# oss0430/SRFRD

Measured on NVIDIA B200. Metric: training seqs/sec; full-catalogue top-10 users/sec, higher is better.
Workload: dtype bf16

## Files before the change

### include/srfrd_b200.h

```cpp
#ifndef SRFRD_B200_H
#define SRFRD_B200_H

#include <stddef.h>
#include <stdint.h>

#ifdef __cplusplus
extern "C" {
#endif

#define SRFRD_ABI_VERSION 10
#if defined(__GNUC__)
#define SRFRD_API __attribute__((visibility("default")))
#else
#define SRFRD_API
#endif

SRFRD_API const char* srfrd_last_error(void);
SRFRD_API int srfrd_abi_version(void);
SRFRD_API int srfrd_device_check(void);

SRFRD_API int srfrd_embed_ln_fwd(const float* item_table, int64_t n_rows, int D, const float* pos_table,
                       const float* aux_table, int64_t n_aux, int F, int mode, const int64_t* seq,
                       const int64_t* aux_ids, int64_t B, int L, float item_scale, const float* ln_w,
                       const float* ln_b, float eps, void* x0_bf16, float* x0_f32, void* q_bf16, float* stats,
                       int ldx, float drop_p, uint64_t drop_seed, uint32_t drop_stream, const float* drop_step,
                       void* stream);

SRFRD_API int srfrd_srfu_labels(const int64_t* fake_ids, int64_t B, int L, int kind, int64_t* labels, void* stream);

SRFRD_API int srfrd_embed_bwd(const void* dx0_bf16, int ldx, const int64_t* seq, const int64_t* aux_ids, int64_t B, int L,
                    int D, int F, int mode, float item_scale, float* d_item, float* d_aux, void* stream);

SRFRD_API int srfrd_layernorm_fwd(const void* x_bf16, int ldx, const float* w, const float* b, float eps, void* y_bf16,
                        float* y_f32, int ldy, float* stats, int64_t T, int H, int64_t row_stride,
                        int64_t row_offset, void* stream);
SRFRD_API int srfrd_layernorm_bwd(const void* dy_bf16, const float* dy_f32, int lddy, const void* x_bf16, int ldx,
                        const float* stats, const float* w, const void* add_bf16, int ldadd,
                        const int64_t* row_ids, void* dx_bf16, int lddx, float* dw, float* db, int64_t T, int H,
                        void* stream);

typedef struct {
  const float* bias;
  const void* residual;
  const void* gate;
  const int64_t* row_ids;
  void* out_bf16;
  float* out_f32;
  int ldr, ldg, ldc;
  int relu;
  float drop_p;
  uint32_t drop_stream;
  uint64_t drop_seed;
  const float* drop_step;
  void* ln_out_bf16;
  const float* ln_w;
  const float* ln_b;
  float* ln_stats;
  int ld_ln;
  float ln_eps;
} srfrd_gemm_epilogue_t;

SRFRD_API int srfrd_gemm_tn(const void* A_bf16, int lda, const void* B_bf16, int ldb, int M, int N, int K,
                  const srfrd_gemm_epilogue_t* ep, void* stream);
SRFRD_API int srfrd_gemm_tn_plan(int M, int N, int K, int has_aux, int bf16_out, int fused_ln, int* out);
SRFRD_API int srfrd_gemm_debug_read(long long* host_dst);
SRFRD_API int srfrd_attn_debug_read(long long* host_dst);

SRFRD_API int srfrd_gemm_wgrad(const void* dY_bf16, int lda, const void* X_bf16, int ldb, int64_t T, int Mo, int No,
                     float* dW, int ldw, float* dbias, void* stream);
SRFRD_API int srfrd_gemm_ref(const void* A, int lda, const void* B, int ldb, float* C, int ldc, int M, int N, int K,
                   int a_mn_major, int b_mn_major, void* stream);

SRFRD_API int srfrd_colsum(const void* X_bf16, int64_t M, int N, int64_t ld, float* out, void* stream);
SRFRD_API int srfrd_add_segments(float* in, int64_t n, int seg_in, int seg_out, float* out, void* stream);

SRFRD_API int srfrd_dropout_apply(const void* x_bf16, int ldx, void* out_bf16, int ldo, int64_t M, int N, float drop_p,
                        uint64_t seed, uint32_t stream_id, const float* drop_step, void* stream);

typedef struct {
  const float* src; int src_ld;
  void* dst; int dst_ld;
  void* dst_t; int dst_t_ld;
  int rows, cols;
  int dst_is_f32;
} srfrd_cast_desc_t;
SRFRD_API int srfrd_cast_weights(const srfrd_cast_desc_t* descs_dev, int n, void* stream);
SRFRD_API int srfrd_f32_to_bf16_split(const float* src, int64_t src_ld, const int64_t* row_index, void* hi, void* lo,
                            int64_t rows, int cols, int dst_ld, void* stream);

SRFRD_API int srfrd_attention_fwd(const void* q, int ldq, const void* k, const void* v, int ldkv, void* o, int ldo,
                        float* stats, int64_t B, int L, int H, int heads, float drop_p, uint64_t seed, uint32_t stream_id,
                        const float* drop_step, void* stream);
SRFRD_API int srfrd_attention_bwd(const void* dout, int lddo, const void* q, int ldq, const void* k, const void* v, int ldkv,
                        const void* o, int ldo, float* stats, void* dq, int lddq, void* dk, void* dv, int lddkv, int64_t B,
                        int L, int H, int heads, float drop_p, uint64_t seed, uint32_t stream_id, const float* drop_step,
                        void* stream);

SRFRD_API int srfrd_score_fwd(const float* h, int ldh, const float* item_table, const float* fake_table, const int64_t* pos,
                    const int64_t* neg, const int64_t* prs, const int64_t* nrs, int64_t T, int D, int F, float* zp,
                    float* zn, void* stream);
SRFRD_API int srfrd_score_bwd(const float* h, int ldh, const float* item_table, const float* fake_table, const int64_t* pos,
                    const int64_t* neg, const int64_t* prs, const int64_t* nrs, const float* dzp, const float* dzn,
                    int64_t T, int D, int F, float* dh, int lddh, float* d_item, float* d_fake, void* stream);
SRFRD_API int srfrd_score_loss_fused(const float* h, int ldh, const float* item_table, const float* fake_table,
                           const int64_t* pos, const int64_t* neg, const int64_t* prs, const int64_t* nrs,
                           const float* w_pos, const float* w_neg, const float* norm, int64_t T, int D, int F,
                           float* zp, float* zn, float* loss_acc, float* dh, int lddh, float* d_item, float* d_fake,
                           void* stream);
SRFRD_API int srfrd_weight_sums(const int64_t* pos, const float* w_pos, const float* w_neg, int64_t T, float* out2,
                      void* stream);
SRFRD_API int srfrd_loss_finalize(float* acc2, const float* norm2, float* loss, void* stream);

SRFRD_API int srfrd_adam_tick(float* state3, float beta1, float beta2, void* stream);
SRFRD_API int srfrd_adam_step(float* p, float* g, float* m, float* v, int64_t n, float lr, float beta1, float beta2, float eps,
                    const float* state3, int zero_grad, void* stream);

SRFRD_API int srfrd_adam_step_fused(float* p, float* g, float* m, float* v, int64_t n, float lr, float beta1, float beta2,
                          float eps, float* state8, int zero_grad, float* acc2, const float* norm2, float* loss,
                          void* stream, const int64_t* l2_seg, int l2_n_seg, const float* l2_coef, const float* l2_reg);

SRFRD_API int srfrd_param_l2_plan(const int64_t* seg_host, int n_seg, int64_t* n_chunks);
SRFRD_API int srfrd_param_l2(const float* p, const int64_t* seg, int n_seg, int64_t n_chunks, float l2, float* coef,
                   float* reg, double* ws, void* stream);

#define SRFRD_TOPK_KMAX 64
SRFRD_API int srfrd_catalogue_topk_plan(int64_t U, int64_t n_rows, int64_t row_lo, int D, int n_split, int* chunks_out,
                                        int k);
SRFRD_API int srfrd_catalogue_topk_kmax(int D, int n_split, int* kmax_out);
SRFRD_API int srfrd_catalogue_topk(const void* feats_bf16, int64_t U, int64_t u_pad, int n_split, const void* table_bf16,
                         int64_t n_rows, int64_t row_lo, int64_t id_base, int D, int ld_feats, int ld_table,
                         int chunks, float* part_scores, int* part_ids, float* packed_out, void* stream, int k);
SRFRD_API int srfrd_merge_topk(const float* scores, const int* ids, int64_t U, int nlists, int k, float* out_scores,
                     int64_t* out_ids, void* stream);
SRFRD_API int srfrd_merge_topk_packed(const float* packed, int64_t U, int nlists, int k, float* out_scores,
                            int64_t* out_ids, void* stream);
SRFRD_API int srfrd_catalogue_rank(const void* feats_bf16, int64_t U, int64_t u_pad, int n_split,
                                   const void* table_bf16, int64_t n_rows, int64_t row_lo, int64_t id_base,
                                   int D, int ld_feats, int ld_table,
                                   const void* target_rows_bf16, int ld_target, const int64_t* target_ids,
                                   float* target_scores, int* rank_out, void* stream);

SRFRD_API int srfrd_catalogue_ce_plan(int Dp, int64_t* smem_bytes, int* ring_stages, int* tmem_cols);
SRFRD_API int srfrd_catalogue_ce_fwd(const void* h_bf16, int ldh, const void* table_bf16, int ldt, int64_t n_items, int Dp,
                                     const int64_t* pos, const float* w_pos, const int* row_tok, const int* rows_dev,
                                     int64_t cap_rows, float* lse, float* loss_acc, void* stream);
SRFRD_API int srfrd_catalogue_ce_bwd(const void* h_bf16, int ldh, const void* table_bf16, int ldt, int64_t n_items, int Dp,
                                     int D, const int64_t* pos, const float* w_pos, const float* norm, const int* row_tok,
                                     const int* rows_dev, int64_t cap_rows, const float* lse, float* dh, int lddh,
                                     float* d_item, int ldd, void* stream);

SRFRD_API int srfrd_sample_batch(const int64_t* offsets, const int* items, const int8_t* labels, const float* p_fake,
                       const int* eligible, int n_eligible, int itemnum, int B, int L, int policy, uint64_t seed,
                       const float* step, int64_t* users, int64_t* seq, int64_t* rsq, int64_t* pos, int64_t* prs,
                       int64_t* neg, int64_t* nrs, float* w_pos, void* stream);

SRFRD_API int srfrd_sample_candidates(const int64_t* offsets, const int* items, const int* users0, const int* target,
                            int64_t U, int itemnum, int C, uint64_t seed, int64_t* cand, void* stream);
SRFRD_API int srfrd_candidate_rank(const float* feats, int ldf, const float* item_table, int64_t n_rows, int D,
                         const int64_t* cand, int64_t U, int C, const float* fake_table, int F,
                         const int64_t* user_label, float* logits, int ldl, int* rank, int* err_flag, void* stream);
SRFRD_API int srfrd_add_user_term(float* logits, int ldl, int64_t U, int I, const float* feats_tail, int ldf,
                        const float* fake_table, const int64_t* label, int F, void* stream);

typedef struct {
  int* rows;
  int* cnt;
  int* seq_first;
  int* tok_row;
  int* row_tok;
  int64_t* row_ids;
  int* row_info;
  int* tile_row0;
  int* last_row;
  int64_t cap;
} srfrd_pack_t;
SRFRD_API int srfrd_pack_plan(const int64_t* seq, const int64_t* keep, int64_t B, int L, const srfrd_pack_t* pk, void* stream);
SRFRD_API int srfrd_set_row_limit(const int* rows_dev);
SRFRD_API int srfrd_embed_ln_fwd_packed(const float* item_table, int64_t n_rows, int D, const float* pos_table,
                              const float* aux_table, int64_t n_aux, int F, int mode, const int64_t* seq,
                              const int64_t* aux_ids, int64_t B, int L, float item_scale, const float* ln_w,
                              const float* ln_b, float eps, void* x0_bf16, void* q_bf16, float* stats, int ldx,
                              float drop_p, uint64_t drop_seed, uint32_t drop_stream, const float* drop_step,
                              const int* row_tok, const int* rows_dev, int64_t cap_rows, void* stream);
SRFRD_API int srfrd_layernorm_fwd_rows(const void* x_bf16, int ldx, const float* w, const float* b, float eps, float* y_f32,
                             int ldy, const int* row_index, int64_t n, int H, void* stream);
SRFRD_API int srfrd_attention_packed_supported(int L, int H, int heads);
SRFRD_API int srfrd_attention_packed_oproj_supported(int L, int H, int heads);
SRFRD_API int srfrd_attention_fwd_packed(const void* q, int ldq, const void* k, const void* v, int ldkv, void* o, int ldo,
                               const srfrd_pack_t* pk, int L, int H, int heads, float drop_p, uint64_t seed,
                               uint32_t stream_id, const float* drop_step, void* stream, const void* wo, int ldw,
                               const float* bo, const void* res, int ldres, const float* ln_w, const float* ln_b,
                               float ln_eps, float* ln_stats, void* r, int ldr, void* y, int ldy);
SRFRD_API int srfrd_attention_bwd_packed(const void* dout, int lddo, const void* q, int ldq, const void* k, const void* v,
                               int ldkv, void* dq, int lddq, void* dk, void* dv, int lddkv, const srfrd_pack_t* pk,
                               int L, int H, int heads, float drop_p, uint64_t seed, uint32_t stream_id,
                               const float* drop_step, void* stream, const void* dr, int lddr, const void* woT, int ldw);
SRFRD_API int srfrd_score_loss_fused_packed(const float* h, int ldh, const float* item_table, const float* fake_table,
                                  const int64_t* pos, const int64_t* neg, const int64_t* prs, const int64_t* nrs,
                                  const float* w_pos, const float* w_neg, const float* norm, int D, int F,
                                  float* loss_acc, float* dh, int lddh, float* d_item, float* d_fake,
                                  const int* row_tok, const int* rows_dev, int64_t cap_rows, void* stream);
SRFRD_API int srfrd_embed_bwd_packed(const void* dx0_bf16, int ldx, const int64_t* seq, const int64_t* aux_ids,
                           const int* row_tok, const int* rows_dev, int64_t cap_rows, int L, int D, int F, int mode,
                           float item_scale, float* d_item, float* d_aux, float* d_pos, void* stream);

typedef struct {
  const float* bias1; const float* bias2;
  const void* gate; int ldg;
  int relu1;
  float drop1_p, drop2_p; uint32_t drop1_stream, drop2_stream; uint64_t drop_seed; const float* drop_step;
  const void* residual; int ldr;
  int residual_is_a;
  const int64_t* row_ids;
  void* mid_out; int ldm;
  void* out; int ldc;
  void* ln_out; int ld_ln; const float* ln_w; const float* ln_b; float* ln_stats; float ln_eps;
} srfrd_mlp2_t;
SRFRD_API int srfrd_mlp2_tn(const void* A_bf16, int lda, const void* W1_bf16, int ldw1, const void* W2_bf16, int ldw2, int M, int N,
                  const srfrd_mlp2_t* ep, void* stream);

SRFRD_API int srfrd_attention_live_items(const int* tok_row, int64_t B, int L, int heads, int* q_lo, int* items, int* n_live,
                               void* stream);
SRFRD_API int srfrd_set_attention_live(const int* q_lo, const int* items, const int* n_live, const int* tok_row);

typedef struct {
  const void* src; int ld_s;
  void* dst; int ld_d;
  int W;
  int mode;
} srfrd_repack_part_t;
SRFRD_API int srfrd_unpack_rows(const srfrd_repack_part_t* parts, int n_parts, const srfrd_pack_t* pk, int64_t B, int L,
                      void* stream);
SRFRD_API int srfrd_pack_rows(const srfrd_repack_part_t* parts, int n_parts, const srfrd_pack_t* pk, int64_t B, int L,
                    void* stream);

SRFRD_API int srfrd_dp_adam_step(float* const* grad_ptrs_dev, float* const* param_ptrs_dev, uint32_t* const* signal_ptrs_dev,
                       int rank, int world, int64_t n, float* m, float* v, float lr, float beta1, float beta2, float eps,
                       float* state8, const float* norm2, uint32_t* local4, void* stream, const int64_t* l2_seg,
                       int l2_n_seg, const float* l2_coef, const float* l2_reg);

#ifdef __cplusplus
}
#endif
#endif
```

### srfrd_b200/_lib.py

```python
from __future__ import annotations

import ctypes as C
import os

_HERE = os.path.dirname(os.path.abspath(__file__))
LIB_PATH = os.environ.get("SRFRD_B200_LIB") or os.path.join(_HERE, "lib", "libsrfrd_b200.so")

vp, i32, i64, f32, u32, u64 = C.c_void_p, C.c_int, C.c_int64, C.c_float, C.c_uint32, C.c_uint64


class GemmEpilogue(C.Structure):
    _fields_ = [("bias", vp), ("residual", vp), ("gate", vp), ("row_ids", vp), ("out_bf16", vp), ("out_f32", vp),
                ("ldr", i32), ("ldg", i32), ("ldc", i32), ("relu", i32), ("drop_p", f32), ("drop_stream", u32),
                ("drop_seed", u64), ("drop_step", vp),
                ("ln_out_bf16", vp), ("ln_w", vp), ("ln_b", vp), ("ln_stats", vp), ("ld_ln", i32), ("ln_eps", f32)]


class CastDesc(C.Structure):
    _fields_ = [("src", vp), ("src_ld", i32), ("dst", vp), ("dst_ld", i32), ("dst_t", vp), ("dst_t_ld", i32),
                ("rows", i32), ("cols", i32), ("dst_is_f32", i32)]


class Mlp2Epilogue(C.Structure):
    _fields_ = [("bias1", vp), ("bias2", vp), ("gate", vp), ("ldg", i32), ("relu1", i32), ("drop1_p", f32), ("drop2_p", f32),
                ("drop1_stream", u32), ("drop2_stream", u32), ("drop_seed", u64), ("drop_step", vp), ("residual", vp), ("ldr", i32),
                ("residual_is_a", i32), ("row_ids", vp), ("mid_out", vp), ("ldm", i32), ("out", vp), ("ldc", i32),
                ("ln_out", vp), ("ld_ln", i32), ("ln_w", vp), ("ln_b", vp), ("ln_stats", vp), ("ln_eps", f32)]


class PackDesc(C.Structure):
    _fields_ = [("rows", vp), ("cnt", vp), ("seq_first", vp), ("tok_row", vp), ("row_tok", vp), ("row_ids", vp),
                ("row_info", vp), ("tile_row0", vp), ("last_row", vp), ("cap", i64)]


class RepackPart(C.Structure):
    _fields_ = [("src", vp), ("ld_s", i32), ("dst", vp), ("ld_d", i32), ("W", i32), ("mode", i32)]


SIGNATURES = {
    "srfrd_abi_version": [],
    "srfrd_device_check": [],
    "srfrd_embed_ln_fwd": [vp, i64, i32, vp, vp, i64, i32, i32, vp, vp, i64, i32, f32, vp, vp, f32, vp, vp, vp, vp, i32,
                           f32, u64, u32, vp, vp],
    "srfrd_srfu_labels": [vp, i64, i32, i32, vp, vp],
    "srfrd_embed_bwd": [vp, i32, vp, vp, i64, i32, i32, i32, i32, f32, vp, vp, vp],
    "srfrd_layernorm_fwd": [vp, i32, vp, vp, f32, vp, vp, i32, vp, i64, i32, i64, i64, vp],
    "srfrd_layernorm_bwd": [vp, vp, i32, vp, i32, vp, vp, vp, i32, vp, vp, i32, vp, vp, i64, i32, vp],
    "srfrd_gemm_tn": [vp, i32, vp, i32, i32, i32, i32, C.POINTER(GemmEpilogue), vp],
    "srfrd_mlp2_tn": [vp, i32, vp, i32, vp, i32, i32, i32, C.POINTER(Mlp2Epilogue), vp],
    "srfrd_gemm_tn_plan": [i32, i32, i32, i32, i32, i32, vp],
    "srfrd_gemm_debug_read": [vp],
    "srfrd_attn_debug_read": [vp],
    "srfrd_gemm_wgrad": [vp, i32, vp, i32, i64, i32, i32, vp, i32, vp, vp],
    "srfrd_gemm_ref": [vp, i32, vp, i32, vp, i32, i32, i32, i32, i32, i32, vp],
    "srfrd_colsum": [vp, i64, i32, i64, vp, vp],
    "srfrd_add_segments": [vp, i64, i32, i32, vp, vp],
    "srfrd_dropout_apply": [vp, i32, vp, i32, i64, i32, f32, u64, u32, vp, vp],
    "srfrd_cast_weights": [vp, i32, vp],
    "srfrd_f32_to_bf16_split": [vp, i64, vp, vp, vp, i64, i32, i32, vp],
    "srfrd_attention_fwd": [vp, i32, vp, vp, i32, vp, i32, vp, i64, i32, i32, i32, f32, u64, u32, vp, vp],
    "srfrd_attention_bwd": [vp, i32, vp, i32, vp, vp, i32, vp, i32, vp, vp, i32, vp, vp, i32, i64, i32, i32, i32, f32, u64,
                            u32, vp, vp],
    "srfrd_score_fwd": [vp, i32, vp, vp, vp, vp, vp, vp, i64, i32, i32, vp, vp, vp],
    "srfrd_score_bwd": [vp, i32, vp, vp, vp, vp, vp, vp, vp, vp, i64, i32, i32, vp, i32, vp, vp, vp],
    "srfrd_score_loss_fused": [vp, i32, vp, vp, vp, vp, vp, vp, vp, vp, vp, i64, i32, i32, vp, vp, vp, vp, i32, vp, vp, vp],
    "srfrd_weight_sums": [vp, vp, vp, i64, vp, vp],
    "srfrd_loss_finalize": [vp, vp, vp, vp],
    "srfrd_adam_tick": [vp, f32, f32, vp],
    "srfrd_adam_step": [vp, vp, vp, vp, i64, f32, f32, f32, f32, vp, i32, vp],
    "srfrd_adam_step_fused": [vp, vp, vp, vp, i64, f32, f32, f32, f32, vp, i32, vp, vp, vp, vp, vp, i32, vp, vp],
    "srfrd_param_l2_plan": [C.POINTER(i64), i32, C.POINTER(i64)],
    "srfrd_param_l2": [vp, vp, i32, i64, f32, vp, vp, vp, vp],
    "srfrd_catalogue_topk_plan": [i64, i64, i64, i32, i32, C.POINTER(i32), i32],
    "srfrd_catalogue_topk_kmax": [i32, i32, C.POINTER(i32)],
    "srfrd_catalogue_topk": [vp, i64, i64, i32, vp, i64, i64, i64, i32, i32, i32, i32, vp, vp, vp, vp, i32],
    "srfrd_merge_topk_packed": [vp, i64, i32, i32, vp, vp, vp],
    "srfrd_catalogue_rank": [vp, i64, i64, i32, vp, i64, i64, i64, i32, i32, i32, vp, i32, vp, vp, vp, vp],
    "srfrd_catalogue_ce_plan": [i32, C.POINTER(i64), C.POINTER(i32), C.POINTER(i32)],
    "srfrd_catalogue_ce_fwd": [vp, i32, vp, i32, i64, i32, vp, vp, vp, vp, i64, vp, vp, vp],
    "srfrd_catalogue_ce_bwd": [vp, i32, vp, i32, i64, i32, i32, vp, vp, vp, vp, vp, i64, vp, vp, i32, vp, i32, vp],
    "srfrd_attention_live_items": [vp, i64, i32, i32, vp, vp, vp, vp],
    "srfrd_set_attention_live": [vp, vp, vp, vp],
    "srfrd_merge_topk": [vp, vp, i64, i32, i32, vp, vp, vp],
    "srfrd_unpack_rows": [C.POINTER(RepackPart), i32, C.POINTER(PackDesc), i64, i32, vp],
    "srfrd_pack_rows": [C.POINTER(RepackPart), i32, C.POINTER(PackDesc), i64, i32, vp],
    "srfrd_dp_adam_step": [vp, vp, vp, i32, i32, i64, vp, vp, f32, f32, f32, f32, vp, vp, vp, vp, vp, i32, vp, vp],
    "srfrd_pack_plan": [vp, vp, i64, i32, C.POINTER(PackDesc), vp],
    "srfrd_set_row_limit": [vp],
    "srfrd_embed_ln_fwd_packed": [vp, i64, i32, vp, vp, i64, i32, i32, vp, vp, i64, i32, f32, vp, vp, f32, vp, vp, vp, i32,
                                  f32, u64, u32, vp, vp, vp, i64, vp],
    "srfrd_layernorm_fwd_rows": [vp, i32, vp, vp, f32, vp, i32, vp, i64, i32, vp],
    "srfrd_attention_packed_supported": [i32, i32, i32],
    "srfrd_attention_packed_oproj_supported": [i32, i32, i32],
    "srfrd_attention_fwd_packed": [vp, i32, vp, vp, i32, vp, i32, C.POINTER(PackDesc), i32, i32, i32, f32, u64, u32, vp, vp,
                                   vp, i32, vp, vp, i32, vp, vp, f32, vp, vp, i32, vp, i32],
    "srfrd_attention_bwd_packed": [vp, i32, vp, i32, vp, vp, i32, vp, i32, vp, vp, i32, C.POINTER(PackDesc), i32, i32, i32,
                                   f32, u64, u32, vp, vp, vp, i32, vp, i32],
    "srfrd_score_loss_fused_packed": [vp, i32, vp, vp, vp, vp, vp, vp, vp, vp, vp, i32, i32, vp, vp, i32, vp, vp, vp, vp,
                                      i64, vp],
    "srfrd_embed_bwd_packed": [vp, i32, vp, vp, vp, vp, i64, i32, i32, i32, i32, f32, vp, vp, vp, vp],
    "srfrd_sample_candidates": [vp, vp, vp, vp, i64, i32, i32, u64, vp, vp],
    "srfrd_candidate_rank": [vp, i32, vp, i64, i32, vp, i64, i32, vp, i32, vp, vp, i32, vp, vp, vp],
    "srfrd_add_user_term": [vp, i32, i64, i32, vp, i32, vp, vp, i32, vp],
    "srfrd_sample_batch": [vp, vp, vp, vp, vp, i32, i32, i32, i32, i32, u64, vp, vp, vp, vp, vp, vp, vp, vp, vp, vp],
}

_lib = None
_device_ok = False
launch_count = 0


def load() -> C.CDLL:
    global _lib
    if _lib is not None:
        return _lib
    if not os.path.exists(LIB_PATH):
        raise RuntimeError(
            f"srfrd_b200: {LIB_PATH} is not built. Run `make -C srfrd_b200/csrc` (needs nvcc, sm_100a). "
            "There is no CPU fallback.")
    lib = C.CDLL(LIB_PATH)
    lib.srfrd_last_error.restype = C.c_char_p
    lib.srfrd_last_error.argtypes = []
    for name, argtypes in SIGNATURES.items():
        fn = getattr(lib, name)
        fn.argtypes = argtypes
        fn.restype = C.c_int
    if lib.srfrd_abi_version() != 10:
        raise RuntimeError("srfrd_b200: ABI version mismatch between _lib.py and the built library")
    _lib = lib
    return lib


def require_device() -> None:
    global _device_ok
    if _device_ok:
        return
    lib = load()
    if lib.srfrd_device_check() != 0:
        raise RuntimeError("srfrd_b200: " + lib.srfrd_last_error().decode())
    _device_ok = True


_profile = None


def set_profile(records) -> None:
    global _profile
    _profile = records


def call(name: str, *args) -> None:
    global launch_count
    lib = _lib or load()
    if _profile is not None:
        import torch
        e0, e1 = torch.cuda.Event(enable_timing=True), torch.cuda.Event(enable_timing=True)
        e0.record()
        rc = getattr(lib, name)(*args)
        e1.record()
        _profile.append((name, args, e0, e1))
    else:
        rc = getattr(lib, name)(*args)
    if rc != 0:
        raise RuntimeError(f"{name}: {lib.srfrd_last_error().decode()}")
    launch_count += 1
```

### srfrd_b200/csrc/pack.cu

```cuda
#include "common.cuh"
#include "srfrd_b200.h"

namespace srfrd {

static constexpr int PACK_TILE = 128;
static constexpr int SCAN_THREADS = 1024;

__global__ void __launch_bounds__(256) pack_count_kernel(const int64_t* seq, const int64_t* keep, int64_t B, int L, int* cnt) {
  const int lane = threadIdx.x & 31;
  const int64_t b = (int64_t)blockIdx.x * (blockDim.x >> 5) + (threadIdx.x >> 5);
  if (b >= B) return;
  int n = 0;
  for (int l0 = 0; l0 < L; l0 += 32) {
    const int l = l0 + lane;
    bool k = false;
    if (l < L) k = (__ldg(seq + b * L + l) != 0) || (keep && __ldg(keep + b * L + l) != 0);
    n += __popc(__ballot_sync(0xffffffffu, k));
  }
  if (lane == 0) cnt[b] = n;
}

__device__ __forceinline__ int pack_bound(const int* first, int B, int Tp, int i) { return i <= B ? first[min(i, B)] + 0 : Tp + (i - B); }

__global__ void __launch_bounds__(SCAN_THREADS) pack_scan_kernel(srfrd_pack_t pk, int64_t B, int plan_tiles) {
  extern __shared__ int sm[];
  __shared__ int wsum[32];
  __shared__ int s_total;
  const int tid = threadIdx.x, lane = tid & 31, warp = tid >> 5;
  int* first = sm;
  const int per = (int)((B + SCAN_THREADS - 1) / SCAN_THREADS);
  const int64_t b0 = (int64_t)tid * per, b1 = min(B, b0 + per);
  int local = 0;
  for (int64_t b = b0; b < b1; ++b) local += pk.cnt[b] + 1;
  int incl = local;
#pragma unroll
  for (int o = 1; o < 32; o <<= 1) { const int v = __shfl_up_sync(0xffffffffu, incl, o); if (lane >= o) incl += v; }
  if (lane == 31) wsum[warp] = incl;
  __syncthreads();
  if (warp == 0) {
    int v = wsum[lane];
#pragma unroll
    for (int o = 1; o < 32; o <<= 1) { const int u = __shfl_up_sync(0xffffffffu, v, o); if (lane >= o) v += u; }
    wsum[lane] = v;
    if (lane == 31) s_total = v;
  }
  __syncthreads();
  int run = incl - local + (warp ? wsum[warp - 1] : 0);
  for (int64_t b = b0; b < b1; ++b) { first[b] = run; pk.seq_first[b] = run; run += pk.cnt[b] + 1; }
  const int Tp = s_total;
  const int M = (Tp + PACK_TILE - 1) / PACK_TILE * PACK_TILE;
  if (tid == 0) { first[B] = Tp; pk.seq_first[B] = Tp; pk.rows[0] = M; pk.rows[1] = Tp; }
  __syncthreads();
  for (int r = Tp + tid; r < M; r += SCAN_THREADS) {
    pk.row_tok[r] = -1;
    pk.row_ids[r] = 0;
    reinterpret_cast<int4*>(pk.row_info)[r] = make_int4(r, r + 1, __float_as_int(1.f), 0);
  }
  if (!plan_tiles) {
    if (tid == 0) { pk.rows[2] = 0; pk.rows[3] = 0; pk.tile_row0[0] = M; }
    return;
  }
  const int NB = (int)B + (M - Tp);
  int* nxt = sm + B + 1;
  for (int i = tid; i < NB; i += SCAN_THREADS) {
    const int lim = pack_bound(first, (int)B, Tp, i) + PACK_TILE;
    int lo = i + 1, hi = NB;
    while (lo < hi) {
      const int mid = (lo + hi + 1) >> 1;
      if (pack_bound(first, (int)B, Tp, mid) <= lim) lo = mid; else hi = mid - 1;
    }
    nxt[i] = lo;
  }
  __syncthreads();
  __shared__ int s_ntiles;
  if (tid == 0) {
    int k = 0;
    for (int i = 0; i < NB;) { const int j = nxt[i]; nxt[k++] = i; i = j; }
    s_ntiles = k;
    pk.rows[2] = k;
    pk.rows[3] = 0;
  }
  __syncthreads();
  const int nt = s_ntiles;
  for (int k = tid; k < nt; k += SCAN_THREADS) pk.tile_row0[k] = pack_bound(first, (int)B, Tp, nxt[k]);
  if (tid == 0) pk.tile_row0[nt] = M;
}

__global__ void __launch_bounds__(256) pack_fill_kernel(const int64_t* seq, const int64_t* keep, int64_t B, int L, srfrd_pack_t pk) {
  const int lane = threadIdx.x & 31;
  const int64_t b = (int64_t)blockIdx.x * (blockDim.x >> 5) + (threadIdx.x >> 5);
  if (b >= B) return;
  const int row0 = pk.seq_first[b], end = pk.seq_first[b + 1];
  int4* info = reinterpret_cast<int4*>(pk.row_info);
  if (lane == 0) {
    pk.row_tok[row0] = -1;
    pk.row_ids[row0] = 0;
    info[row0] = make_int4(row0, end, __float_as_int(1.f), 0);
  }
  int base = 0;
  int last = row0;
  for (int l0 = 0; l0 < L; l0 += 32) {
    const int l = l0 + lane;
    int64_t id = 0;
    bool k = false;
    if (l < L) {
      id = __ldg(seq + b * L + l);
      k = (id != 0) || (keep && __ldg(keep + b * L + l) != 0);
    }
    const unsigned m = __ballot_sync(0xffffffffu, k);
    const int before = base + __popc(m & ((1u << lane) - 1u));
    const int row = row0 + 1 + before;
    if (l < L) {
      pk.tok_row[b * L + l] = k ? row : -1;
      if (k) {
        pk.row_tok[row] = (int)(b * L + l);
        pk.row_ids[row] = id;
        info[row] = make_int4(row0, end, __float_as_int((float)(l - before)), l);
        if (l == L - 1) last = row;
      }
    }
    base += __popc(m);
  }
  last = __shfl_sync(0xffffffffu, last, (L - 1) & 31);
  if (lane == 0) pk.last_row[b] = last;
}

}

using namespace srfrd;

extern "C" int srfrd_pack_plan(const int64_t* seq, const int64_t* keep, int64_t B, int L, const srfrd_pack_t* pk_host,
                               void* stream_) {
  cudaStream_t stream = (cudaStream_t)stream_;
  SRFRD_REQUIRE(seq && pk_host, "pack_plan: null pointer");
  const srfrd_pack_t pk = *pk_host;
  SRFRD_REQUIRE(pk.rows && pk.cnt && pk.seq_first && pk.tok_row && pk.row_tok && pk.row_ids && pk.row_info && pk.tile_row0 &&
                pk.last_row, "pack_plan: null output");
  SRFRD_REQUIRE(B >= 1 && L >= 1 && L <= 4096, "pack_plan: bad shape (B=%lld L=%d)", (long long)B, L);
  SRFRD_REQUIRE(B <= 16384, "pack_plan: at most 16384 sequences per call (B=%lld)", (long long)B);
  const int64_t need = (B * (L + 1) + PACK_TILE - 1) / PACK_TILE * PACK_TILE;
  SRFRD_REQUIRE(pk.cap >= need, "pack_plan: capacity %lld rows < %lld", (long long)pk.cap, (long long)need);
  SRFRD_REQUIRE(((uintptr_t)pk.row_info & 15) == 0, "pack_plan: row_info must be 16-byte aligned");
  pack_count_kernel<<<(unsigned)((B + 7) / 8), 256, 0, stream>>>(seq, keep, B, L, pk.cnt);
  SRFRD_LAUNCH_CHECK();
  const size_t smem = (size_t)(2 * B + 2 + PACK_TILE + 2) * sizeof(int);
  static bool attr = false;
  if (!attr) {
    SRFRD_CUDA(cudaFuncSetAttribute(pack_scan_kernel, cudaFuncAttributeMaxDynamicSharedMemorySize, 160 * 1024));
    attr = true;
  }
  pack_scan_kernel<<<1, SCAN_THREADS, smem, stream>>>(pk, B, L + 1 <= PACK_TILE ? 1 : 0);
  SRFRD_LAUNCH_CHECK();
  pack_fill_kernel<<<(unsigned)((B + 7) / 8), 256, 0, stream>>>(seq, keep, B, L, pk);
  SRFRD_LAUNCH_CHECK();
  return 0;
}
```

### srfrd_b200/csrc/rowwise.cu

```cuda
#include <stdlib.h>

#include "common.cuh"
#include "srfrd_b200.h"

namespace srfrd {

static constexpr int MAXW = 512;

template <int LPR>
__device__ __forceinline__ float group_sum(float v) {
#pragma unroll
  for (int o = LPR / 2; o > 0; o >>= 1) v += __shfl_xor_sync(0xffffffffu, v, o);
  return v;
}

__device__ __forceinline__ void unpack8(const uint4& u, float* f) {
  const uint32_t w[4] = {u.x, u.y, u.z, u.w};
#pragma unroll
  for (int i = 0; i < 4; ++i) {
    const float2 t = __bfloat1622float2(*reinterpret_cast<const __nv_bfloat162*>(&w[i]));
    f[2 * i] = t.x; f[2 * i + 1] = t.y;
  }
}
__device__ __forceinline__ uint4 pack8(const float* f) {
  return make_uint4(pack_bf16x2(f[0], f[1]), pack_bf16x2(f[2], f[3]), pack_bf16x2(f[4], f[5]), pack_bf16x2(f[6], f[7]));
}
__device__ __forceinline__ void load8_f32(const float* p, float* f) {
  const float4 a = __ldg(reinterpret_cast<const float4*>(p)), b = __ldg(reinterpret_cast<const float4*>(p) + 1);
  f[0] = a.x; f[1] = a.y; f[2] = a.z; f[3] = a.w; f[4] = b.x; f[5] = b.y; f[6] = b.z; f[7] = b.w;
}
__device__ __forceinline__ void load8_f32_stream(const float* p, float* f) {
  float4 a, b;
  asm volatile("ld.global.nc.L1::no_allocate.L2::256B.v4.f32 {%0,%1,%2,%3}, [%4];"
               : "=f"(a.x), "=f"(a.y), "=f"(a.z), "=f"(a.w) : "l"(p));
  asm volatile("ld.global.nc.L1::no_allocate.L2::256B.v4.f32 {%0,%1,%2,%3}, [%4];"
               : "=f"(b.x), "=f"(b.y), "=f"(b.z), "=f"(b.w) : "l"(p + 4));
  f[0] = a.x; f[1] = a.y; f[2] = a.z; f[3] = a.w; f[4] = b.x; f[5] = b.y; f[6] = b.z; f[7] = b.w;
}
__device__ __forceinline__ void store8_f32(float* p, const float* f) {
  reinterpret_cast<float4*>(p)[0] = make_float4(f[0], f[1], f[2], f[3]);
  reinterpret_cast<float4*>(p)[1] = make_float4(f[4], f[5], f[6], f[7]);
}

struct EmbedParams {
  const float* item_table;
  const float* pos_table;
  const float* aux_table;
  const int64_t* seq;
  const int64_t* aux_ids;
  const int* row_tok;
  const int* rows_dev;
  int64_t T;
  int L, D, F, mode;
  float item_scale;
  const float* ln_w;
  const float* ln_b;
  float eps;
  bf16* x0;
  float* x0_f32;
  bf16* q;
  float* stats;
  int ldx;
  uint64_t drop_seed; uint32_t drop_thresh, drop_stream; float drop_scale; const float* drop_step;
};

template <int LPR, int CH, bool VEC>
__global__ void __launch_bounds__(256, 4) embed_ln_kernel(EmbedParams p) {
  pdl_prologue_done();
  if (p.drop_thresh) p.drop_seed = mix_seed(p.drop_seed, p.drop_step);
  constexpr int RPW = 32 / LPR;
  const int lane = threadIdx.x & 31, sub = lane % LPR, grp = lane / LPR;
  const int H = p.D + (p.mode == 1 ? p.F : 0);
  const int Hc = (H + 7) & ~7;
  const int64_t warp = (int64_t)blockIdx.x * (blockDim.x >> 5) + (threadIdx.x >> 5);
  const int64_t nwarps = (int64_t)gridDim.x * (blockDim.x >> 5);
  for (int64_t t0 = warp * RPW; t0 < p.T; t0 += nwarps * RPW) {
    const int64_t t = t0 + grp;
    const bool row_ok = t < p.T;
    int64_t id = 0, aid = 0;
    int l = 0;
    if (row_ok) {
      l = (int)(t % p.L);
      id = __ldg(p.seq + t);
      if (p.mode == 1) aid = p.aux_ids ? __ldg(p.aux_ids + t) : 0;
      if (p.mode == 2) aid = __ldg(p.aux_ids + t / p.L);
    }
    const bool valid = row_ok && id != 0;
    float v[CH][8];
    float sum = 0.f;
#pragma unroll
    for (int ch = 0; ch < CH; ++ch) {
      const int c = (ch * LPR + sub) * 8;
#pragma unroll
      for (int j = 0; j < 8; ++j) v[ch][j] = 0.f;
      if (!VEC) {
        if (valid && c < Hc) {
#pragma unroll
          for (int j = 0; j < 8; ++j) {
            const int col = c + j;
            float x = 0.f;
            if (col < p.D) {
              x = __ldg(p.item_table + id * p.D + col);
              if (p.item_scale != 1.f) x = __fmul_rn(x, p.item_scale);
              x = __fadd_rn(x, __ldg(p.pos_table + (int64_t)l * p.D + col));
              if (p.mode == 2) x = __fadd_rn(x, __ldg(p.aux_table + aid * p.D + col));
            } else if (col < H) {
              x = __ldg(p.aux_table + aid * p.F + (col - p.D));
            }
            if (p.drop_thresh && col < H)
              x = dropout_keep(p.drop_seed, p.drop_stream, (uint64_t)t * H + col, p.drop_thresh) ? x * p.drop_scale : 0.f;
            v[ch][j] = x;
          }
        }
      } else if (valid && c < H) {
        if (c < p.D) {
          float e[8], pp[8];
          load8_f32_stream(p.item_table + id * p.D + c, e);
          load8_f32(p.pos_table + (int64_t)l * p.D + c, pp);
#pragma unroll
          for (int j = 0; j < 8; ++j) {
            float x = e[j];
            if (p.item_scale != 1.f) x = __fmul_rn(x, p.item_scale);
            v[ch][j] = __fadd_rn(x, pp[j]);
          }
          if (p.mode == 2) {
            float u[8];
            load8_f32(p.aux_table + aid * p.D + c, u);
#pragma unroll
            for (int j = 0; j < 8; ++j) v[ch][j] = __fadd_rn(v[ch][j], u[j]);
          }
        } else {
          load8_f32(p.aux_table + aid * p.F + (c - p.D), v[ch]);
        }
        if (p.drop_thresh) {
#pragma unroll
          for (int j = 0; j < 8; ++j)
            v[ch][j] = dropout_keep(p.drop_seed, p.drop_stream, (uint64_t)t * H + c + j, p.drop_thresh)
                           ? v[ch][j] * p.drop_scale : 0.f;
        }
      }
#pragma unroll
      for (int j = 0; j < 8; ++j) sum += v[ch][j];
    }
    float mean = 0.f, rstd = 0.f;
    if (p.ln_w) {
      mean = group_sum<LPR>(sum) / H;
      float sq = 0.f;
#pragma unroll
      for (int ch = 0; ch < CH; ++ch) {
        const int c = (ch * LPR + sub) * 8;
        if (c < Hc) {
#pragma unroll
          for (int j = 0; j < 8; ++j) { const float d = v[ch][j] - mean; sq += (VEC || c + j < H) ? d * d : 0.f; }
        }
      }
      rstd = rsqrtf(group_sum<LPR>(sq) / H + p.eps);
    }
    if (!row_ok) continue;
#pragma unroll
    for (int ch = 0; ch < CH; ++ch) {
      const int c = (ch * LPR + sub) * 8;
      if (c >= Hc) continue;
      if (p.x0_f32) {
        if (VEC) store8_f32(p.x0_f32 + t * H + c, v[ch]);
        else {
#pragma unroll
          for (int j = 0; j < 8; ++j) if (c + j < H) p.x0_f32[t * H + c + j] = v[ch][j];
        }
      }
      if (p.x0) *reinterpret_cast<uint4*>(p.x0 + t * p.ldx + c) = pack8(v[ch]);
      if (p.ln_w) {
        float w[8], b[8], y[8];
        if (VEC) { load8_f32(p.ln_w + c, w); load8_f32(p.ln_b + c, b); }
        else {
#pragma unroll
          for (int j = 0; j < 8; ++j) { w[j] = c + j < H ? __ldg(p.ln_w + c + j) : 0.f; b[j] = c + j < H ? __ldg(p.ln_b + c + j) : 0.f; }
        }
#pragma unroll
        for (int j = 0; j < 8; ++j) y[j] = (VEC || c + j < H) ? (v[ch][j] - mean) * rstd * w[j] + b[j] : 0.f;
        *reinterpret_cast<uint4*>(p.q + t * p.ldx + c) = pack8(y);
      }
    }
    if (p.ln_w && p.stats && sub == 0) *reinterpret_cast<float2*>(p.stats + 2 * t) = make_float2(mean, rstd);
  }
}

template <int LPR, int CH, int MODE, bool DROP>
__global__ void __launch_bounds__(256, 4) embed_ln_vec_kernel(EmbedParams p) {
  pdl_prologue_done();
  if (DROP) p.drop_seed = mix_seed(p.drop_seed, p.drop_step);
  constexpr int RPW = 32 / LPR;
  const int lane = threadIdx.x & 31, sub = lane % LPR, grp = lane / LPR;
  const int H = p.D + (MODE == 1 ? p.F : 0);
  const float invH = 1.f / (float)H;
  const int64_t warp = (int64_t)blockIdx.x * (blockDim.x >> 5) + (threadIdx.x >> 5);
  const int64_t stride = (int64_t)gridDim.x * (blockDim.x >> 5) * RPW;
  const int lstep = (int)(stride % p.L);
  int64_t t = warp * RPW + grp;
  int l = (int)(t % p.L);
  const bool has_ln = p.ln_w != nullptr;
  if (p.rows_dev) p.T = min(p.T, (int64_t)__ldg(p.rows_dev));
  for (; t - grp < p.T; t += stride, l = (l + lstep >= p.L) ? l + lstep - p.L : l + lstep) {
    const bool row_ok = t < p.T;
    int64_t id = 0, aid = 0;
    if (p.row_tok) {
      const int src = row_ok ? __ldg(p.row_tok + t) : -1;
      if (src >= 0) {
        l = src % p.L;
        id = __ldg(p.seq + src);
        if (MODE == 1) aid = p.aux_ids ? __ldg(p.aux_ids + src) : 0;
        if (MODE == 2) aid = __ldg(p.aux_ids + src / p.L);
      }
    } else if (row_ok) {
      id = __ldg(p.seq + t);
      if (MODE == 1) aid = p.aux_ids ? __ldg(p.aux_ids + t) : 0;
      if (MODE == 2) aid = __ldg(p.aux_ids + t / p.L);
    }
    const bool valid = row_ok && id != 0;
    const float* erow = p.item_table + id * p.D;
    const float* prow = p.pos_table + (int64_t)l * p.D;
    const float* arow = p.aux_table + aid * (MODE == 1 ? p.F : p.D);
    float v[CH][8];
    float e[CH][8];
#pragma unroll
    for (int ch = 0; ch < CH; ++ch) {
      const int c = (ch * LPR + sub) * 8;
#pragma unroll
      for (int j = 0; j < 8; ++j) e[ch][j] = 0.f;
      if (valid && c < H) {
        if (MODE != 1 || c < p.D) load8_f32_stream(erow + c, e[ch]);
        else load8_f32(arow + (c - p.D), e[ch]);
      }
    }
    float sum = 0.f;
#pragma unroll
    for (int ch = 0; ch < CH; ++ch) {
      const int c = (ch * LPR + sub) * 8;
#pragma unroll
      for (int j = 0; j < 8; ++j) v[ch][j] = e[ch][j];
      if (valid && c < p.D) {
        float pp[8];
        load8_f32(prow + c, pp);
#pragma unroll
        for (int j = 0; j < 8; ++j) {
          float x = e[ch][j];
          if (p.item_scale != 1.f) x = __fmul_rn(x, p.item_scale);
          v[ch][j] = __fadd_rn(x, pp[j]);
        }
        if (MODE == 2) {
          float u[8];
          load8_f32(arow + c, u);
#pragma unroll
          for (int j = 0; j < 8; ++j) v[ch][j] = __fadd_rn(v[ch][j], u[j]);
        }
      }
      if (DROP) {
        if (valid && c < H) {
#pragma unroll
          for (int j = 0; j < 8; ++j)
            v[ch][j] = dropout_keep(p.drop_seed, p.drop_stream, (uint64_t)t * H + c + j, p.drop_thresh)
                           ? v[ch][j] * p.drop_scale : 0.f;
        }
      }
      sum += ((v[ch][0] + v[ch][1]) + (v[ch][2] + v[ch][3])) + ((v[ch][4] + v[ch][5]) + (v[ch][6] + v[ch][7]));
    }
    float a = 0.f, nb = 0.f, mean = 0.f;
    if (has_ln) {
      mean = group_sum<LPR>(sum) * invH;
      float sq = 0.f;
#pragma unroll
      for (int ch = 0; ch < CH; ++ch) {
        if ((ch * LPR + sub) * 8 < H) {
          float d[8];
#pragma unroll
          for (int j = 0; j < 8; ++j) d[j] = v[ch][j] - mean;
          sq += ((d[0] * d[0] + d[1] * d[1]) + (d[2] * d[2] + d[3] * d[3])) + ((d[4] * d[4] + d[5] * d[5]) + (d[6] * d[6] + d[7] * d[7]));
        }
      }
      a = rsqrtf(group_sum<LPR>(sq) * invH + p.eps);
      nb = -mean * a;
    }
    if (!row_ok) continue;
#pragma unroll
    for (int ch = 0; ch < CH; ++ch) {
      const int c = (ch * LPR + sub) * 8;
      if (c >= H) continue;
      if (p.x0_f32) store8_f32(p.x0_f32 + t * H + c, v[ch]);
      if (p.x0) *reinterpret_cast<uint4*>(p.x0 + t * p.ldx + c) = pack8(v[ch]);
      if (has_ln) {
        float w[8], b[8], y[8];
        load8_f32(p.ln_w + c, w);
        load8_f32(p.ln_b + c, b);
#pragma unroll
        for (int j = 0; j < 8; ++j) y[j] = fmaf(fmaf(v[ch][j], a, nb), w[j], b[j]);
        *reinterpret_cast<uint4*>(p.q + t * p.ldx + c) = pack8(y);
      }
    }
    if (has_ln && p.stats && sub == 0) *reinterpret_cast<float2*>(p.stats + 2 * t) = make_float2(mean, a);
  }
}

struct LnFwdParams {
  const bf16* x; int ldx;
  const float* w; const float* b; float eps;
  bf16* y_bf16; float* y_f32; int ldy;
  float* stats;
  int64_t T; int H;
  int64_t row_stride;
  int64_t row_offset;
  const int* row_index;
  const int* rows_dev;
};

template <int LPR, int CH, bool RAGGED>
__global__ void __launch_bounds__(256) ln_fwd_kernel(LnFwdParams p) {
  constexpr int RPW = 32 / LPR, UN = 2;
  const int lane = threadIdx.x & 31, sub = lane % LPR, grp = lane / LPR;
  const int Hc = (p.H + 7) & ~7;
  constexpr bool ragged = RAGGED;
  pdl_prologue_done();
  if (p.rows_dev) p.T = min(p.T, (int64_t)__ldg(p.rows_dev));
  const int64_t warp = (int64_t)blockIdx.x * (blockDim.x >> 5) + (threadIdx.x >> 5);
  const int64_t nwarps = (int64_t)gridDim.x * (blockDim.x >> 5);
  for (int64_t t0 = warp * RPW * UN; t0 < p.T; t0 += nwarps * RPW * UN) {
    uint4 raw[UN][CH];
#pragma unroll
    for (int u = 0; u < UN; ++u) {
      const int64_t t = t0 + u * RPW + grp;
#pragma unroll
      for (int ch = 0; ch < CH; ++ch) {
        const int c = (ch * LPR + sub) * 8;
        raw[u][ch] = make_uint4(0, 0, 0, 0);
        if (t < p.T && c < Hc)
          raw[u][ch] = __ldg(reinterpret_cast<const uint4*>(
              p.x + (p.row_index ? (int64_t)__ldg(p.row_index + t) : t * p.row_stride + p.row_offset) * p.ldx + c));
      }
    }
#pragma unroll
    for (int u = 0; u < UN; ++u) {
      const int64_t t = t0 + u * RPW + grp;
      float v[CH][8];
      float sum = 0.f;
#pragma unroll
      for (int ch = 0; ch < CH; ++ch) {
        unpack8(raw[u][ch], v[ch]);
        const int c = (ch * LPR + sub) * 8;
#pragma unroll
        for (int j = 0; j < 8; ++j) {
          if (ragged && c + j >= p.H) v[ch][j] = 0.f;
          sum += v[ch][j];
        }
      }
      const float mean = group_sum<LPR>(sum) / p.H;
      float sq = 0.f;
#pragma unroll
      for (int ch = 0; ch < CH; ++ch) {
        const int c = (ch * LPR + sub) * 8;
        if (c < Hc) {
#pragma unroll
          for (int j = 0; j < 8; ++j) { const float d = v[ch][j] - mean; sq += (!ragged || c + j < p.H) ? d * d : 0.f; }
        }
      }
      const float rstd = rsqrtf(group_sum<LPR>(sq) / p.H + p.eps);
      if (t >= p.T) continue;
#pragma unroll
      for (int ch = 0; ch < CH; ++ch) {
        const int c = (ch * LPR + sub) * 8;
        if (c >= Hc) continue;
        float y[8], w[8], b[8];
        if (!ragged) { load8_f32(p.w + c, w); load8_f32(p.b + c, b); }
        else {
#pragma unroll
          for (int j = 0; j < 8; ++j) { w[j] = c + j < p.H ? __ldg(p.w + c + j) : 0.f; b[j] = c + j < p.H ? __ldg(p.b + c + j) : 0.f; }
        }
#pragma unroll
        for (int j = 0; j < 8; ++j) y[j] = (!ragged || c + j < p.H) ? (v[ch][j] - mean) * rstd * w[j] + b[j] : 0.f;
        if (p.y_bf16) *reinterpret_cast<uint4*>(p.y_bf16 + t * p.ldy + c) = pack8(y);
        if (p.y_f32) store8_f32(p.y_f32 + t * p.ldy + c, y);
      }
      if (p.stats && sub == 0) *reinterpret_cast<float2*>(p.stats + 2 * t) = make_float2(mean, rstd);
    }
  }
}

struct LnBwdParams {
  const bf16* dy_bf16; const float* dy_f32; int lddy;
  const bf16* x; int ldx;
  const float* stats;
  const float* w;
  const bf16* add; int ldadd;
  const int64_t* row_ids;
  bf16* dx; int lddx;
  float* dw; float* db;
  int64_t T; int H;
  const int* rows_dev;
};

template <int LPR, int CH, bool F32DY, bool RAGGED>
__global__ void __launch_bounds__(256, 2) ln_bwd_kernel(LnBwdParams p) {
  __shared__ float sdw[MAXW], sdb[MAXW];
  __shared__ __align__(16) float sw[MAXW];
  constexpr int RPW = 32 / LPR;
  const int lane = threadIdx.x & 31, sub = lane % LPR, grp = lane / LPR;
  const int Hc = (p.H + 7) & ~7;
  constexpr bool ragged = RAGGED;
  const int64_t warp = (int64_t)blockIdx.x * (blockDim.x >> 5) + (threadIdx.x >> 5);
  const int64_t nwarps = (int64_t)gridDim.x * (blockDim.x >> 5);
  pdl_prologue_done();
  if (p.rows_dev) p.T = min(p.T, (int64_t)__ldg(p.rows_dev));
  for (int i = threadIdx.x; i < MAXW; i += blockDim.x) { sdw[i] = sdb[i] = 0.f; sw[i] = i < p.H ? __ldg(p.w + i) : 0.f; }
  __syncthreads();
  float adw[CH][8], adb[CH][8];
#pragma unroll
  for (int ch = 0; ch < CH; ++ch)
#pragma unroll
    for (int j = 0; j < 8; ++j) adw[ch][j] = adb[ch][j] = 0.f;
  const float invH = 1.f / p.H;
  for (int64_t t0 = warp * RPW; t0 < p.T; t0 += nwarps * RPW) {
    const int64_t t = t0 + grp;
    const bool ok = t < p.T;
    uint4 xr[CH], ar[CH], dr[CH];
    float df[F32DY ? CH : 1][8];
    const float2 st = ok ? __ldg(reinterpret_cast<const float2*>(p.stats + 2 * t)) : make_float2(0.f, 0.f);
    const float msk = (ok && p.row_ids) ? ((__ldg(p.row_ids + t) != 0) ? 1.f : 0.f) : 1.f;
#pragma unroll
    for (int ch = 0; ch < CH; ++ch) {
      const int c = (ch * LPR + sub) * 8;
      xr[ch] = ar[ch] = dr[ch] = make_uint4(0, 0, 0, 0);
      if (F32DY) {
#pragma unroll
        for (int j = 0; j < 8; ++j) df[ch][j] = 0.f;
      }
      if (ok && c < Hc) {
        if (F32DY) load8_f32(p.dy_f32 + t * p.lddy + c, df[ch]);
        else dr[ch] = __ldg(reinterpret_cast<const uint4*>(p.dy_bf16 + t * p.lddy + c));
        xr[ch] = __ldg(reinterpret_cast<const uint4*>(p.x + t * p.ldx + c));
        if (p.add) ar[ch] = __ldg(reinterpret_cast<const uint4*>(p.add + t * p.ldadd + c));
      }
    }
    const float mean = st.x, rstd = st.y;
    float sg = 0.f, sgx = 0.f;
#pragma unroll
    for (int ch = 0; ch < CH; ++ch) {
      const int c = (ch * LPR + sub) * 8;
      const bool cok = c < Hc && ok;
      float xv[8], dv[8];
      unpack8(xr[ch], xv);
      if (F32DY) {
#pragma unroll
        for (int j = 0; j < 8; ++j) dv[j] = df[ch][j];
      } else {
        unpack8(dr[ch], dv);
      }
      const float4 w0 = *reinterpret_cast<const float4*>(sw + (cok ? c : 0)), w1 = *reinterpret_cast<const float4*>(sw + (cok ? c : 0) + 4);
      const float wv[8] = {w0.x, w0.y, w0.z, w0.w, w1.x, w1.y, w1.z, w1.w};
#pragma unroll
      for (int j = 0; j < 8; ++j) {
        const float xh = (cok && (!ragged || c + j < p.H)) ? (xv[j] - mean) * rstd : 0.f;
        if (ragged && c + j >= p.H) dv[j] = 0.f;
        const float g = dv[j] * wv[j];
        adw[ch][j] = fmaf(dv[j], xh, adw[ch][j]);
        adb[ch][j] += dv[j];
        sg += g;
        sgx = fmaf(g, xh, sgx);
      }
    }
    sg = group_sum<LPR>(sg) * invH;
    sgx = group_sum<LPR>(sgx) * invH;
    if (!ok) continue;
#pragma unroll
    for (int ch = 0; ch < CH; ++ch) {
      const int c = (ch * LPR + sub) * 8;
      if (c >= Hc) continue;
      float xv[8], dv[8], av[8], o[8];
      unpack8(xr[ch], xv);
      unpack8(ar[ch], av);
      if (F32DY) {
#pragma unroll
        for (int j = 0; j < 8; ++j) dv[j] = df[ch][j];
      } else {
        unpack8(dr[ch], dv);
      }
      const float4 w0 = *reinterpret_cast<const float4*>(sw + c), w1 = *reinterpret_cast<const float4*>(sw + c + 4);
      const float wv[8] = {w0.x, w0.y, w0.z, w0.w, w1.x, w1.y, w1.z, w1.w};
#pragma unroll
      for (int j = 0; j < 8; ++j) {
        const float xh = (xv[j] - mean) * rstd;
        o[j] = (rstd * (dv[j] * wv[j] - sg - xh * sgx) + av[j]) * msk;
        if (ragged && c + j >= p.H) o[j] = 0.f;
      }
      *reinterpret_cast<uint4*>(p.dx + t * p.lddx + c) = pack8(o);
    }
  }
#pragma unroll
  for (int ch = 0; ch < CH; ++ch) {
#pragma unroll
    for (int j = 0; j < 8; ++j) {
#pragma unroll
      for (int o = LPR; o < 32; o <<= 1) {
        adw[ch][j] += __shfl_xor_sync(0xffffffffu, adw[ch][j], o);
        adb[ch][j] += __shfl_xor_sync(0xffffffffu, adb[ch][j], o);
      }
    }
    const int c = (ch * LPR + sub) * 8;
    if (grp == 0 && c < Hc) {
#pragma unroll
      for (int j = 0; j < 8; ++j) { atomicAdd(&sdw[c + j], adw[ch][j]); atomicAdd(&sdb[c + j], adb[ch][j]); }
    }
  }
  __syncthreads();
  for (int i = threadIdx.x; i < p.H; i += blockDim.x) { red_add_f32(p.dw + i, sdw[i]); red_add_f32(p.db + i, sdb[i]); }
}

template <int LPR, int CH>
__global__ void __launch_bounds__(256, 4) ln_fwd_vec_kernel(LnFwdParams p) {
  constexpr int RPW = 32 / LPR, LAST = CH - 1;
  const int lane = threadIdx.x & 31, sub = lane % LPR, grp = lane / LPR;
  pdl_prologue_done();
  const float invH = 1.f / (float)p.H;
  const bool last_ok = (LAST * LPR + sub) * 8 < p.H;
  int col[CH];
#pragma unroll
  for (int ch = 0; ch < CH; ++ch) col[ch] = (ch * LPR + sub) * 8;
  if (!last_ok) col[LAST] = 0;
  const int64_t stride = (int64_t)gridDim.x * (blockDim.x >> 5) * RPW;
  if (p.rows_dev) p.T = min(p.T, (int64_t)__ldg(p.rows_dev));
  for (int64_t t = ((int64_t)blockIdx.x * (blockDim.x >> 5) + (threadIdx.x >> 5)) * RPW + grp; t - grp < p.T; t += stride) {
    const bool ok = t < p.T;
    const int64_t tt = ok ? t : p.T - 1;
    const bf16* xrow = p.x + (p.row_index ? (int64_t)__ldg(p.row_index + tt) : tt * p.row_stride + p.row_offset) * p.ldx;
    uint4 raw[CH];
#pragma unroll
    for (int ch = 0; ch < CH; ++ch) raw[ch] = __ldg(reinterpret_cast<const uint4*>(xrow + col[ch]));
    if (!last_ok) raw[LAST] = make_uint4(0, 0, 0, 0);
    float v[CH][8];
    float sum = 0.f;
#pragma unroll
    for (int ch = 0; ch < CH; ++ch) {
      unpack8(raw[ch], v[ch]);
      sum += ((v[ch][0] + v[ch][1]) + (v[ch][2] + v[ch][3])) + ((v[ch][4] + v[ch][5]) + (v[ch][6] + v[ch][7]));
    }
    const float mean = group_sum<LPR>(sum) * invH;
    float sq = 0.f;
#pragma unroll
    for (int ch = 0; ch < CH; ++ch) {
      float d[8];
#pragma unroll
      for (int j = 0; j < 8; ++j) d[j] = v[ch][j] - mean;
      const float s8 = ((d[0] * d[0] + d[1] * d[1]) + (d[2] * d[2] + d[3] * d[3])) + ((d[4] * d[4] + d[5] * d[5]) + (d[6] * d[6] + d[7] * d[7]));
      sq += (ch == LAST && !last_ok) ? 0.f : s8;
    }
    const float a = rsqrtf(group_sum<LPR>(sq) * invH + p.eps), nb = -mean * a;
#pragma unroll
    for (int ch = 0; ch < CH; ++ch) {
      float y[8], w[8], b[8];
      load8_f32(p.w + col[ch], w);
      load8_f32(p.b + col[ch], b);
#pragma unroll
      for (int j = 0; j < 8; ++j) y[j] = fmaf(fmaf(v[ch][j], a, nb), w[j], b[j]);
      const bool st = ok && (ch != LAST || last_ok);
      if (p.y_bf16 && st) *reinterpret_cast<uint4*>(p.y_bf16 + t * p.ldy + col[ch]) = pack8(y);
      if (p.y_f32 && st) store8_f32(p.y_f32 + t * p.ldy + col[ch], y);
    }
    if (p.stats && sub == 0 && ok) *reinterpret_cast<float2*>(p.stats + 2 * t) = make_float2(mean, a);
  }
}

template <int LPR, int CH, bool F32DY, bool HAS_ADD, int TPB, int BPS>
__global__ void __launch_bounds__(TPB, BPS) ln_bwd_vec_kernel(LnBwdParams p) {
  __shared__ float sdw[MAXW], sdb[MAXW];
  __shared__ __align__(16) float sw[MAXW];
  constexpr int RPW = 32 / LPR, LAST = CH - 1;
  const int lane = threadIdx.x & 31, sub = lane % LPR, grp = lane / LPR;
  pdl_prologue_done();
  if (p.rows_dev) p.T = min(p.T, (int64_t)__ldg(p.rows_dev));
  for (int i = threadIdx.x; i < MAXW; i += blockDim.x) { sdw[i] = sdb[i] = 0.f; sw[i] = i < p.H ? __ldg(p.w + i) : 0.f; }
  __syncthreads();
  float adw[CH][8], adb[CH][8];
#pragma unroll
  for (int ch = 0; ch < CH; ++ch)
#pragma unroll
    for (int j = 0; j < 8; ++j) adw[ch][j] = adb[ch][j] = 0.f;
  const float invH = 1.f / (float)p.H;
  const bool last_ok = (LAST * LPR + sub) * 8 < p.H;
  int col[CH];
#pragma unroll
  for (int ch = 0; ch < CH; ++ch) col[ch] = (ch * LPR + sub) * 8;
  if (!last_ok) col[LAST] = 0;
  const int64_t stride = (int64_t)gridDim.x * (blockDim.x >> 5) * RPW;
  for (int64_t t = ((int64_t)blockIdx.x * (blockDim.x >> 5) + (threadIdx.x >> 5)) * RPW + grp; t - grp < p.T; t += stride) {
    const bool ok = t < p.T;
    const int64_t tt = ok ? t : p.T - 1;
    uint4 xr[CH], ar[HAS_ADD ? CH : 1], dr[F32DY ? 1 : CH];
    float df[F32DY ? CH : 1][8];
    const float2 st = __ldg(reinterpret_cast<const float2*>(p.stats + 2 * tt));
    const bool keep = p.row_ids ? (__ldg(p.row_ids + tt) != 0) : true;
#pragma unroll
    for (int ch = 0; ch < CH; ++ch) {
      const bool cok = ok && (ch != LAST || last_ok);
      if (F32DY) {
        load8_f32(p.dy_f32 + tt * p.lddy + col[ch], df[ch]);
        if (!cok) {
#pragma unroll
          for (int j = 0; j < 8; ++j) df[ch][j] = 0.f;
        }
      } else {
        dr[ch] = __ldg(reinterpret_cast<const uint4*>(p.dy_bf16 + tt * p.lddy + col[ch]));
        if (!cok) dr[ch] = make_uint4(0, 0, 0, 0);
      }
      xr[ch] = __ldg(reinterpret_cast<const uint4*>(p.x + tt * p.ldx + col[ch]));
      if (HAS_ADD) ar[ch] = __ldg(reinterpret_cast<const uint4*>(p.add + tt * p.ldadd + col[ch]));
    }
    const float rstd = st.y, nb = -st.x * st.y;
    float sg = 0.f, sgx = 0.f;
#pragma unroll
    for (int ch = 0; ch < CH; ++ch) {
      float xv[8], dv[8];
      unpack8(xr[ch], xv);
      if (F32DY) {
#pragma unroll
        for (int j = 0; j < 8; ++j) dv[j] = df[ch][j];
      } else {
        unpack8(dr[ch], dv);
      }
      const float4 w0 = *reinterpret_cast<const float4*>(sw + col[ch]), w1 = *reinterpret_cast<const float4*>(sw + col[ch] + 4);
      const float wv[8] = {w0.x, w0.y, w0.z, w0.w, w1.x, w1.y, w1.z, w1.w};
#pragma unroll
      for (int j = 0; j < 8; ++j) {
        const float xh = fmaf(xv[j], rstd, nb);
        const float g = dv[j] * wv[j];
        adw[ch][j] = fmaf(dv[j], xh, adw[ch][j]);
        adb[ch][j] += dv[j];
        sg += g;
        sgx = fmaf(g, xh, sgx);
      }
    }
    sg = group_sum<LPR>(sg) * invH;
    sgx = group_sum<LPR>(sgx) * invH;
#pragma unroll
    for (int ch = 0; ch < CH; ++ch) {
      float xv[8], dv[8], av[8], o[8];
      unpack8(xr[ch], xv);
      if (HAS_ADD) unpack8(ar[ch], av);
      if (F32DY) {
#pragma unroll
        for (int j = 0; j < 8; ++j) dv[j] = df[ch][j];
      } else {
        unpack8(dr[ch], dv);
      }
      const float4 w0 = *reinterpret_cast<const float4*>(sw + col[ch]), w1 = *reinterpret_cast<const float4*>(sw + col[ch] + 4);
      const float wv[8] = {w0.x, w0.y, w0.z, w0.w, w1.x, w1.y, w1.z, w1.w};
#pragma unroll
      for (int j = 0; j < 8; ++j) {
        const float xh = fmaf(xv[j], rstd, nb);
        const float u = fmaf(-sgx, xh, fmaf(dv[j], wv[j], -sg));
        o[j] = HAS_ADD ? fmaf(rstd, u, av[j]) : rstd * u;
      }
      uint4 pk = pack8(o);
      if (!keep) pk = make_uint4(0, 0, 0, 0);
      if (ok && (ch != LAST || last_ok)) *reinterpret_cast<uint4*>(p.dx + t * p.lddx + col[ch]) = pk;
    }
  }
#pragma unroll
  for (int ch = 0; ch < CH; ++ch) {
#pragma unroll
    for (int j = 0; j < 8; ++j) {
#pragma unroll
      for (int o = LPR; o < 32; o <<= 1) {
        adw[ch][j] += __shfl_xor_sync(0xffffffffu, adw[ch][j], o);
        adb[ch][j] += __shfl_xor_sync(0xffffffffu, adb[ch][j], o);
      }
    }
    if (grp == 0 && (ch != LAST || last_ok)) {
#pragma unroll
      for (int j = 0; j < 8; ++j) { atomicAdd(&sdw[col[ch] + j], adw[ch][j]); atomicAdd(&sdb[col[ch] + j], adb[ch][j]); }
    }
  }
  __syncthreads();
  for (int i = threadIdx.x; i < p.H; i += blockDim.x) { red_add_f32(p.dw + i, sdw[i]); red_add_f32(p.db + i, sdb[i]); }
}

#define SRFRD_ROW_DISPATCH_BWD(H, CALL)                  \
  do {                                                   \
    if ((H) <= 64) { CALL(8, 1); }                       \
    else if ((H) <= 128) { CALL(16, 1); }                \
    else if ((H) <= 256) { CALL(32, 1); }                \
    else { CALL(32, 2); }                                \
  } while (0)
#define SRFRD_ROW_DISPATCH(H, CALL)                      \
  do {                                                   \
    if ((H) <= 32) { CALL(4, 1); }                       \
    else if ((H) <= 64) { CALL(8, 1); }                  \
    else if ((H) <= 96) { CALL(4, 3); }                  \
    else if ((H) <= 128) { CALL(16, 1); }                \
    else if ((H) <= 192) { CALL(8, 3); }                 \
    else if ((H) <= 256) { CALL(32, 1); }                \
    else if ((H) <= 384) { CALL(16, 3); }                \
    else { CALL(32, 2); }                                \
  } while (0)

__global__ void __launch_bounds__(256) colsum_kernel(const bf16* X, int64_t M, int N, int64_t ld, float* out,
                                                     int rows_per_block) {
  extern __shared__ float sm[];
  pdl_prologue_done();
  const int TX = blockDim.x, TY = blockDim.y;
  const int64_t r0 = (int64_t)blockIdx.x * rows_per_block;
  const int64_t r1 = min(M, r0 + rows_per_block);
  for (int c0 = blockIdx.y * TX * 2; c0 < N; c0 += gridDim.y * TX * 2) {
    const int c = c0 + threadIdx.x * 2;
    float a0 = 0.f, a1 = 0.f;
    if (c < N) {
      for (int64_t r = r0 + threadIdx.y; r < r1; r += TY) {
        const __nv_bfloat162 v = *reinterpret_cast<const __nv_bfloat162*>(X + r * ld + c);
        a0 += __low2float(v);
        a1 += __high2float(v);
      }
    }
    sm[(threadIdx.y * TX + threadIdx.x) * 2] = a0;
    sm[(threadIdx.y * TX + threadIdx.x) * 2 + 1] = a1;
    __syncthreads();
    if (threadIdx.y == 0 && c < N) {
      for (int y = 1; y < TY; ++y) { a0 += sm[(y * TX + threadIdx.x) * 2]; a1 += sm[(y * TX + threadIdx.x) * 2 + 1]; }
      red_add_f32(out + c, a0);
      red_add_f32(out + c + 1, a1);
    }
    __syncthreads();
  }
}

__global__ void cast_weights_kernel(const srfrd_cast_desc_t* descs, int n) {
  pdl_prologue_done();
  const srfrd_cast_desc_t d = descs[blockIdx.x];
  const int total = d.rows * d.cols;
  for (int i = blockIdx.y * blockDim.x + threadIdx.x; i < total; i += gridDim.y * blockDim.x) {
    const int r = i / d.cols, c = i % d.cols;
    if (d.dst_is_f32) {
      reinterpret_cast<float*>(d.dst)[(size_t)r * d.dst_ld + c] = d.src[(size_t)r * d.src_ld + c];
      continue;
    }
    const bf16 v = f2bf(d.src[(size_t)r * d.src_ld + c]);
    if (d.dst) reinterpret_cast<bf16*>(d.dst)[(size_t)r * d.dst_ld + c] = v;
    if (d.dst_t) reinterpret_cast<bf16*>(d.dst_t)[(size_t)c * d.dst_t_ld + r] = v;
  }
}

__global__ void srfu_labels_kernel(const int64_t* fake_ids, int64_t B, int L, int kind, int64_t* labels) {
  const int lane = threadIdx.x & 31;
  const int64_t b = (int64_t)blockIdx.x * (blockDim.x >> 5) + (threadIdx.x >> 5);
  if (b >= B) return;
  int nf = 0, nr = 0;
  for (int l = lane; l < L; l += 32) {
    const int64_t f = fake_ids[b * L + l];
    nf += f == 1;
    nr += f == 2;
  }
  for (int o = 16; o > 0; o >>= 1) { nf += __shfl_xor_sync(0xffffffffu, nf, o); nr += __shfl_xor_sync(0xffffffffu, nr, o); }
  if (lane == 0) {
    int64_t lab;
    if (kind == 0) lab = nf < nr ? 1 : 2;
    else if (kind == 3) lab = nf > nr ? 2 : 1;
    else if (kind == 1) lab = nf;
    else {
      const float r = __fmul_rn(__fdiv_rn((float)nf, (float)(nf + nr)), 10.f);
      lab = (nf + nr) == 0 ? 0 : (int64_t)floorf(r);
    }
    labels[b] = lab;
  }
}

__global__ void f32_to_bf16_rows_kernel(const float* src, int64_t src_ld, const int64_t* row_index, bf16* hi, bf16* lo,
                                        int64_t rows, int cols, int dst_ld) {
  const int64_t i = (int64_t)blockIdx.x * blockDim.x + threadIdx.x;
  if (i >= rows * cols) return;
  const int64_t r = i / cols; const int c = (int)(i % cols);
  const int64_t sr = row_index ? row_index[r] : r;
  const float v = src[sr * src_ld + c];
  const bf16 h = f2bf(v);
  hi[r * dst_ld + c] = h;
  if (lo) lo[r * dst_ld + c] = f2bf(v - bf2f(h));
}

__global__ void dropout_apply_kernel(const bf16* x, int ldx, bf16* out, int ldo, int64_t M, int N, uint64_t seed,
                                     uint32_t thresh, uint32_t stream_id, float scale, const float* step,
                                     const int* rows_dev) {
  pdl_prologue_done();
  if (rows_dev) M = min(M, (int64_t)__ldg(rows_dev));
  seed = mix_seed(seed, step);
  const int64_t n2 = M * (N / 2);
  for (int64_t i = (int64_t)blockIdx.x * blockDim.x + threadIdx.x; i < n2; i += (int64_t)gridDim.x * blockDim.x) {
    const int64_t r = i / (N / 2); const int c = (int)(i % (N / 2)) * 2;
    const float2 v = __bfloat1622float2(*reinterpret_cast<const __nv_bfloat162*>(x + r * ldx + c));
    const float a = dropout_keep(seed, stream_id, (uint64_t)r * N + c, thresh) ? v.x * scale : 0.f;
    const float b = dropout_keep(seed, stream_id, (uint64_t)r * N + c + 1, thresh) ? v.y * scale : 0.f;
    *reinterpret_cast<uint32_t*>(out + r * ldo + c) = pack_bf16x2(a, b);
  }
}

static int grid_for_rows(int64_t T, int rows_per_block, int max_blocks_per_sm) {
  int64_t blocks = (T + rows_per_block - 1) / rows_per_block;
  const int64_t cap = (int64_t)num_sms() * max_blocks_per_sm;
  return (int)(blocks < cap ? (blocks > 0 ? blocks : 1) : cap);
}

}

using namespace srfrd;

static int embed_ln_fwd_impl(const float* item_table, int64_t n_rows, int D, const float* pos_table,
                             const float* aux_table, int64_t n_aux, int F, int mode, const int64_t* seq,
                             const int64_t* aux_ids, int64_t B, int L, float item_scale, const float* ln_w,
                             const float* ln_b, float eps, void* x0_bf16, float* x0_f32, void* q_bf16,
                             float* stats, int ldx, float drop_p, uint64_t drop_seed, uint32_t drop_stream,
                             const float* drop_step, const int* row_tok, const int* rows_dev, int64_t cap_rows,
                             void* stream) {
  SRFRD_REQUIRE(item_table && pos_table && seq, "embed_ln_fwd: null input");
  SRFRD_REQUIRE(drop_p >= 0.f && drop_p < 1.f, "embed_ln_fwd: dropout p must be in [0, 1)");
  SRFRD_REQUIRE(mode >= 0 && mode <= 2, "embed_ln_fwd: mode must be 0 (none), 1 (concat fake) or 2 (add user label)");
  SRFRD_REQUIRE(mode == 0 || aux_table, "embed_ln_fwd: aux_table required for mode %d", mode);
  SRFRD_REQUIRE(mode != 2 || aux_ids, "embed_ln_fwd: per-sequence labels required for mode 2");
  const int H = D + (mode == 1 ? F : 0);
  SRFRD_REQUIRE(H <= MAXW, "embed_ln_fwd: width %d > %d unsupported", H, MAXW);
  const bool vec = D % 8 == 0 && H % 8 == 0;
  SRFRD_REQUIRE(!ln_w || (ln_b && q_bf16), "embed_ln_fwd: LN needs weight, bias and an output");
  SRFRD_REQUIRE((!x0_bf16 && !q_bf16) || (ldx >= ((H + 7) & ~7) && ldx % 8 == 0), "embed_ln_fwd: bad ldx %d", ldx);
  (void)n_rows; (void)n_aux;
  if (B * L == 0) return 0;
  SRFRD_REQUIRE(!row_tok || (vec && rows_dev && cap_rows > 0 && !x0_f32),
                "embed_ln_fwd_packed: needs widths that are multiples of 8, the device row count and a capacity");
  EmbedParams p;
  p.item_table = item_table; p.pos_table = pos_table; p.aux_table = aux_table; p.seq = seq; p.aux_ids = aux_ids;
  p.row_tok = row_tok; p.rows_dev = rows_dev;
  p.T = row_tok ? cap_rows : B * L; p.L = L; p.D = D; p.F = F; p.mode = mode; p.item_scale = item_scale;
  p.ln_w = ln_w; p.ln_b = ln_b; p.eps = eps; p.x0 = (bf16*)x0_bf16; p.x0_f32 = x0_f32; p.q = (bf16*)q_bf16;
  p.stats = stats; p.ldx = ldx;
  p.drop_seed = drop_seed; p.drop_stream = drop_stream; p.drop_step = drop_step;
  p.drop_thresh = drop_p > 0.f ? (uint32_t)((double)drop_p * 4294967296.0) : 0;
  p.drop_scale = drop_p > 0.f ? 1.f / (1.f - drop_p) : 1.f;
#define CALL(LPR, CH)                                                                                       \
  do {                                                                                                      \
    const int grid = grid_for_rows(p.T, 8 * (32 / LPR), 8);                                                 \
    if (vec) {                                                                                              \
      auto* kern = !p.drop_thresh ? (p.mode == 0 ? embed_ln_vec_kernel<LPR, CH, 0, false>                   \
                                    : p.mode == 1 ? embed_ln_vec_kernel<LPR, CH, 1, false>                  \
                                                  : embed_ln_vec_kernel<LPR, CH, 2, false>)                 \
                                  : (p.mode == 0 ? embed_ln_vec_kernel<LPR, CH, 0, true>                    \
                                    : p.mode == 1 ? embed_ln_vec_kernel<LPR, CH, 1, true>                   \
                                                  : embed_ln_vec_kernel<LPR, CH, 2, true>);                 \
      SRFRD_CUDA(launch_pdl(kern, dim3(grid), dim3(256), 0, (cudaStream_t)stream, p));                      \
    }                                                                                                       \
    else SRFRD_CUDA(launch_pdl(embed_ln_kernel<LPR, CH, false>, dim3(grid), dim3(256), 0, (cudaStream_t)stream, p));    \
  } while (0)
  SRFRD_ROW_DISPATCH(H, CALL);
#undef CALL
  SRFRD_LAUNCH_CHECK();
  return 0;
}

extern "C" int srfrd_embed_ln_fwd(const float* item_table, int64_t n_rows, int D, const float* pos_table,
                                  const float* aux_table, int64_t n_aux, int F, int mode, const int64_t* seq,
                                  const int64_t* aux_ids, int64_t B, int L, float item_scale, const float* ln_w,
                                  const float* ln_b, float eps, void* x0_bf16, float* x0_f32, void* q_bf16,
                                  float* stats, int ldx, float drop_p, uint64_t drop_seed, uint32_t drop_stream,
                                  const float* drop_step, void* stream) {
  return embed_ln_fwd_impl(item_table, n_rows, D, pos_table, aux_table, n_aux, F, mode, seq, aux_ids, B, L, item_scale, ln_w,
                           ln_b, eps, x0_bf16, x0_f32, q_bf16, stats, ldx, drop_p, drop_seed, drop_stream, drop_step, nullptr,
                           nullptr, 0, stream);
}

extern "C" int srfrd_embed_ln_fwd_packed(const float* item_table, int64_t n_rows, int D, const float* pos_table,
                                         const float* aux_table, int64_t n_aux, int F, int mode, const int64_t* seq,
                                         const int64_t* aux_ids, int64_t B, int L, float item_scale, const float* ln_w,
                                         const float* ln_b, float eps, void* x0_bf16, void* q_bf16, float* stats, int ldx,
                                         float drop_p, uint64_t drop_seed, uint32_t drop_stream, const float* drop_step,
                                         const int* row_tok, const int* rows_dev, int64_t cap_rows, void* stream) {
  SRFRD_REQUIRE(row_tok && rows_dev, "embed_ln_fwd_packed: null row map");
  return embed_ln_fwd_impl(item_table, n_rows, D, pos_table, aux_table, n_aux, F, mode, seq, aux_ids, B, L, item_scale, ln_w,
                           ln_b, eps, x0_bf16, nullptr, q_bf16, stats, ldx, drop_p, drop_seed, drop_stream, drop_step, row_tok,
                           rows_dev, cap_rows, stream);
}

static int layernorm_fwd_impl(const void* x, int ldx, const float* w, const float* b, float eps, void* y_bf16,
                              float* y_f32, int ldy, float* stats, int64_t T, int H, int64_t row_stride,
                              int64_t row_offset, const int* row_index, const int* rows_dev, void* stream) {
  SRFRD_REQUIRE(x && w && b && (y_bf16 || y_f32), "layernorm_fwd: null pointer");
  SRFRD_REQUIRE(H <= MAXW && ldx % 8 == 0 && ldy % 8 == 0 && ldx >= ((H + 7) & ~7) && ldy >= ((H + 7) & ~7),
                "layernorm_fwd: width %d / ld (%d, %d) unsupported (rows are padded to a multiple of 8 columns)", H, ldx, ldy);
  if (T == 0) return 0;
  LnFwdParams p;
  p.x = (const bf16*)x; p.ldx = ldx; p.w = w; p.b = b; p.eps = eps; p.y_bf16 = (bf16*)y_bf16; p.y_f32 = y_f32;
  p.ldy = ldy; p.stats = stats; p.T = T; p.H = H; p.row_stride = row_stride; p.row_offset = row_offset;
  p.row_index = row_index; p.rows_dev = rows_dev;
#define CALL(LPR, CH)                                                                                                   \
  do {                                                                                                                  \
    const dim3 grid(grid_for_rows(T, 16 * (32 / LPR), 8));                                                              \
    if (H % 8) SRFRD_CUDA(launch_pdl(ln_fwd_kernel<LPR, CH, true>, grid, dim3(256), 0, (cudaStream_t)stream, p));       \
    else SRFRD_CUDA(launch_pdl(ln_fwd_vec_kernel<LPR, CH>, dim3(grid_for_rows(T, 8 * (32 / LPR), 4)), dim3(256), 0,     \
                               (cudaStream_t)stream, p));                                                               \
  } while (0)
  SRFRD_ROW_DISPATCH(H, CALL);
#undef CALL
  SRFRD_LAUNCH_CHECK();
  return 0;
}

extern "C" int srfrd_layernorm_fwd(const void* x, int ldx, const float* w, const float* b, float eps, void* y_bf16,
                                   float* y_f32, int ldy, float* stats, int64_t T, int H, int64_t row_stride,
                                   int64_t row_offset, void* stream) {
  return layernorm_fwd_impl(x, ldx, w, b, eps, y_bf16, y_f32, ldy, stats, T, H, row_stride, row_offset, nullptr, row_limit(),
                            stream);
}

extern "C" int srfrd_layernorm_fwd_rows(const void* x, int ldx, const float* w, const float* b, float eps, float* y_f32,
                                        int ldy, const int* row_index, int64_t n, int H, void* stream) {
  SRFRD_REQUIRE(row_index, "layernorm_fwd_rows: null row index");
  return layernorm_fwd_impl(x, ldx, w, b, eps, nullptr, y_f32, ldy, nullptr, n, H, 1, 0, row_index, nullptr, stream);
}

extern "C" int srfrd_layernorm_bwd(const void* dy_bf16, const float* dy_f32, int lddy, const void* x, int ldx,
                                   const float* stats, const float* w, const void* add, int ldadd,
                                   const int64_t* row_ids, void* dx, int lddx, float* dw, float* db, int64_t T, int H,
                                   void* stream) {
  SRFRD_REQUIRE((dy_bf16 || dy_f32) && x && stats && w && dx && dw && db, "layernorm_bwd: null pointer");
  const int Hc8 = (H + 7) & ~7;
  SRFRD_REQUIRE(H <= MAXW - 8 && ldx % 8 == 0 && lddx % 8 == 0 && lddy % 8 == 0 && (!add || ldadd % 8 == 0) &&
                    ldx >= Hc8 && lddx >= Hc8 && lddy >= Hc8 && (!add || ldadd >= Hc8),
                "layernorm_bwd: width %d / ld unsupported (rows are padded to a multiple of 8 columns)", H);
  if (T == 0) return 0;
  LnBwdParams p;
  p.dy_bf16 = (const bf16*)dy_bf16; p.dy_f32 = dy_f32; p.lddy = lddy; p.x = (const bf16*)x; p.ldx = ldx;
  p.stats = stats; p.w = w; p.add = (const bf16*)add; p.ldadd = ldadd; p.row_ids = row_ids; p.dx = (bf16*)dx;
  p.lddx = lddx; p.dw = dw; p.db = db; p.T = T; p.H = H; p.rows_dev = row_limit();
#define CALL(LPR, CH)                                                                                             \
  do {                                                                                                            \
    const int grid = grid_for_rows(T, 8 * (32 / LPR) * 8, 2);                                                     \
    if (dy_f32 && (H % 8)) SRFRD_CUDA(launch_pdl(ln_bwd_kernel<LPR, CH, true, true>, dim3(grid), dim3(256), 0, (cudaStream_t)stream, p));        \
    else if (H % 8) SRFRD_CUDA(launch_pdl(ln_bwd_kernel<LPR, CH, false, true>, dim3(grid), dim3(256), 0, (cudaStream_t)stream, p));        \
    else {                                                                                                        \
        \
      const int g3 = grid_for_rows(T, 4 * (32 / LPR) * 8, 3);                                                     \
      if (dy_f32 && add) SRFRD_CUDA(launch_pdl(ln_bwd_vec_kernel<LPR, CH, true, true, 128, 3>, dim3(g3), dim3(128), 0, (cudaStream_t)stream, p));   \
      else if (dy_f32) SRFRD_CUDA(launch_pdl(ln_bwd_vec_kernel<LPR, CH, true, false, 128, 3>, dim3(g3), dim3(128), 0, (cudaStream_t)stream, p));  \
      else if (add) SRFRD_CUDA(launch_pdl(ln_bwd_vec_kernel<LPR, CH, false, true, 128, 3>, dim3(g3), dim3(128), 0, (cudaStream_t)stream, p));     \
      else SRFRD_CUDA(launch_pdl(ln_bwd_vec_kernel<LPR, CH, false, false, 128, 3>, dim3(g3), dim3(128), 0, (cudaStream_t)stream, p));             \
    }                                                                                                             \
  } while (0)
  SRFRD_ROW_DISPATCH(H, CALL);
#undef CALL
  SRFRD_LAUNCH_CHECK();
  return 0;
}

extern "C" int srfrd_colsum(const void* X, int64_t M, int N, int64_t ld, float* out, void* stream) {
  SRFRD_REQUIRE(X && out, "colsum: null pointer");
  SRFRD_REQUIRE(N % 2 == 0 && ld % 2 == 0, "colsum: N and ld must be even");
  if (M == 0 || N == 0) return 0;
  int tx = 32;
  while (tx * 2 < N && tx < 128) tx *= 2;
  const int ty = 256 / tx;
  const int gy = (N + tx * 2 - 1) / (tx * 2);
  int64_t gx = (int64_t)num_sms() * 8 / gy;
  if (gx < 1) gx = 1;
  int64_t rows_per_block = (M + gx - 1) / gx;
  if (rows_per_block < ty * 4) rows_per_block = ty * 4;
  gx = (M + rows_per_block - 1) / rows_per_block;
  dim3 grid((unsigned)gx, (unsigned)gy), block(tx, ty);
  SRFRD_CUDA(launch_pdl(colsum_kernel, grid, block, 256 * 2 * sizeof(float), (cudaStream_t)stream, (const bf16*)X, M, N, ld, out,
                        (int)rows_per_block));
  SRFRD_LAUNCH_CHECK();
  return 0;
}

extern "C" int srfrd_cast_weights(const srfrd_cast_desc_t* descs_dev, int n, void* stream) {
  SRFRD_REQUIRE(descs_dev || n == 0, "cast_weights: null table");
  if (n == 0) return 0;
  SRFRD_CUDA(launch_pdl(cast_weights_kernel, dim3(n, 8), dim3(256), 0, (cudaStream_t)stream, descs_dev, n));
  SRFRD_LAUNCH_CHECK();
  return 0;
}

extern "C" int srfrd_srfu_labels(const int64_t* fake_ids, int64_t B, int L, int kind, int64_t* labels, void* stream) {
  SRFRD_REQUIRE(fake_ids && labels, "srfu_labels: null pointer");
  SRFRD_REQUIRE(kind >= 0 && kind <= 3, "srfu_labels: kind must be 0 (B), 1 (F), 2 (R) or 3 (SRFRN.predict)");
  if (B == 0) return 0;
  srfu_labels_kernel<<<(unsigned)((B + 7) / 8), 256, 0, (cudaStream_t)stream>>>(fake_ids, B, L, kind, labels);
  SRFRD_LAUNCH_CHECK();
  return 0;
}

extern "C" int srfrd_f32_to_bf16_split(const float* src, int64_t src_ld, const int64_t* row_index, void* hi, void* lo,
                                       int64_t rows, int cols, int dst_ld, void* stream) {
  SRFRD_REQUIRE(src && hi, "f32_to_bf16_split: null pointer");
  if (rows * cols == 0) return 0;
  const int64_t n = rows * cols;
  f32_to_bf16_rows_kernel<<<(unsigned)((n + 255) / 256), 256, 0, (cudaStream_t)stream>>>(
      src, src_ld, row_index, (bf16*)hi, (bf16*)lo, rows, cols, dst_ld);
  SRFRD_LAUNCH_CHECK();
  return 0;
}

extern "C" int srfrd_dropout_apply(const void* x, int ldx, void* out, int ldo, int64_t M, int N, float drop_p,
                                   uint64_t seed, uint32_t stream_id, const float* drop_step, void* stream) {
  SRFRD_REQUIRE(x && out, "dropout_apply: null pointer");
  SRFRD_REQUIRE(N % 2 == 0 && ldx % 2 == 0 && ldo % 2 == 0, "dropout_apply: widths must be even");
  SRFRD_REQUIRE(drop_p > 0.f && drop_p < 1.f, "dropout_apply: p must be in (0, 1)");
  if (M == 0) return 0;
  int64_t blocks = (M * (N / 2) + 255) / 256;
  if (blocks > num_sms() * 16) blocks = num_sms() * 16;
  SRFRD_CUDA(launch_pdl(dropout_apply_kernel, dim3((unsigned)blocks), dim3(256), 0, (cudaStream_t)stream, (const bf16*)x, ldx,
                        (bf16*)out, ldo, M, N, seed, (uint32_t)((double)drop_p * 4294967296.0), stream_id,
                        1.f / (1.f - drop_p), drop_step, row_limit()));
  SRFRD_LAUNCH_CHECK();
  return 0;
}
```

### srfrd_b200/engine.py

```python
from __future__ import annotations

import math
import os
from contextlib import contextmanager, nullcontext
from dataclasses import dataclass
from typing import Dict, List, Optional, Tuple

import torch

from . import ops

bf16 = torch.bfloat16
LN_EPS = 1e-8

KINDS = ("SRFR", "SRFRN", "SRFU_B", "SRFU_F", "SRFU_R", "SASRec")


@dataclass
class ModelSpec:
    kind: str
    item_number: int
    max_len: int
    D: int
    F: int = 0
    n_labels: int = 0
    num_blocks: int = 2
    num_heads: int = 1
    dropout: float = 0.0

    def __post_init__(self):
        if self.kind not in KINDS:
            raise ValueError(f"unknown model kind {self.kind}")
        if self.H % self.num_heads:
            raise ValueError("hidden size must be divisible by num_heads")
        if (self.H // self.num_heads) % 2:
            raise ValueError(f"srfrd_b200: head width {self.H // self.num_heads} must be even (bf16 pairs)")

    @property
    def H(self) -> int:
        return self.D + self.F if self.kind in ("SRFR", "SRFRN") else self.D

    @property
    def Dout(self) -> int:
        return self.H if self.kind == "SRFRN" else self.D

    @property
    def Hp(self) -> int:
        return (self.H + 15) // 16 * 16

    @property
    def Dp(self) -> int:
        return (self.D + 15) // 16 * 16

    @property
    def Doutp(self) -> int:
        return self.Hp if self.kind == "SRFRN" else self.Dp

    @property
    def padded(self) -> bool:
        return self.Hp != self.H or self.Dp != self.D

    @property
    def mode(self) -> int:
        return 1 if self.kind in ("SRFR", "SRFRN") else (2 if self.kind.startswith("SRFU") else 0)

    @property
    def item_scale(self) -> float:
        return float(self.D ** 0.5) if self.kind == "SASRec" else 1.0

    @property
    def item_key(self) -> str:
        return "item_emb.weight" if self.kind == "SASRec" else "embedding_layer.item_embed.weight"

    @property
    def pos_key(self) -> str:
        return "pos_emb.weight" if self.kind == "SASRec" else "embedding_layer.pos_embed.weight"

    @property
    def aux_key(self) -> Optional[str]:
        if self.mode == 1:
            return "embedding_layer.fake_embed.weight"
        if self.mode == 2:
            return "embedding_layer.user_label_embed.weight"
        return None

    def param_shapes(self) -> List[Tuple[str, Tuple[int, ...]]]:
        H, D, L, N = self.H, self.D, self.max_len, self.item_number
        out: List[Tuple[str, Tuple[int, ...]]] = []
        if self.kind == "SASRec":
            out += [("item_emb.weight", (N + 1, D)), ("pos_emb.weight", (L, D))]
        elif self.mode == 1:
            out += [("embedding_layer.item_embed.weight", (N + 1, D)),
                    ("embedding_layer.fake_embed.weight", (3, self.F)),
                    ("embedding_layer.pos_embed.weight", (L, D))]
        else:
            out += [("embedding_layer.item_embed.weight", (N + 1, D)),
                    ("embedding_layer.user_label_embed.weight", (self.n_labels, D)),
                    ("embedding_layer.pos_embed.weight", (L, D))]
        for i in range(self.num_blocks):
            out += [(f"attention_layernorms.{i}.weight", (H,)), (f"attention_layernorms.{i}.bias", (H,))]
        for i in range(self.num_blocks):
            out += [(f"attention_layers.{i}.in_proj_weight", (3 * H, H)), (f"attention_layers.{i}.in_proj_bias", (3 * H,)),
                    (f"attention_layers.{i}.out_proj.weight", (H, H)), (f"attention_layers.{i}.out_proj.bias", (H,))]
        for i in range(self.num_blocks):
            out += [(f"forward_layernorms.{i}.weight", (H,)), (f"forward_layernorms.{i}.bias", (H,))]
        for i in range(self.num_blocks):
            out += [(f"forward_layers.{i}.conv1.weight", (H, H, 1)), (f"forward_layers.{i}.conv1.bias", (H,)),
                    (f"forward_layers.{i}.conv2.weight", (H, H, 1)), (f"forward_layers.{i}.conv2.bias", (H,))]
        if self.kind == "SRFR":
            out += [("last_conv.weight", (D, H, 1)), ("last_conv.bias", (D,))]
        out += [("last_layernorm.weight", (self.Dout,)), ("last_layernorm.bias", (self.Dout,))]
        return out


class FlatParams:

    def __init__(self, spec: ModelSpec, device, alloc=None):
        self.spec = spec
        self.offsets: Dict[str, Tuple[int, Tuple[int, ...]]] = {}
        off = 0
        for name, shape in spec.param_shapes():
            n = int(math.prod(shape))
            self.offsets[name] = (off, shape)
            off += (n + 3) // 4 * 4
        self.numel = off
        zeros = (lambda n: alloc(n).zero_()) if alloc is not None else (lambda n: torch.zeros(n, dtype=torch.float32, device=device))
        self.data_ext = zeros(off + 4)
        self.data = self.data_ext[:off]
        self.data_tail = self.data_ext[off:]
        self.grad_bucket = zeros(off + 4)
        self.grad = self.grad_bucket[:off]
        self.grad_tail = self.grad_bucket[off:]

    def segments(self) -> List[Tuple[int, int]]:
        return [(off, int(math.prod(shape))) for off, shape in self.offsets.values()]

    def view(self, name: str, grad: bool = False) -> torch.Tensor:
        off, shape = self.offsets[name]
        buf = self.grad if grad else self.data
        return buf[off:off + int(math.prod(shape))].view(shape)

    def mat(self, name: str, grad: bool = False) -> torch.Tensor:
        v = self.view(name, grad)
        return v.view(v.shape[0], -1)


@dataclass
class _Saved:
    seq: torch.Tensor
    aux_ids: Optional[torch.Tensor]
    B: int
    L: int
    T: int
    row_ids: torch.Tensor
    plan: Optional[ops.PackedPlan]
    hyb: Optional[Dict[str, torch.Tensor]]
    live: Optional[ops.LiveTiles]
    p_drop: float
    seed: int
    step: Optional[torch.Tensor]
    fuse_ln: bool
    oproj: int
    mlp2: bool
    version: int

    def __getitem__(self, key: str):
        return getattr(self, key)


class HotPath:

    def __init__(self, spec: ModelSpec, params: FlatParams):
        self.spec, self.P = spec, params
        self.device = params.data.device
        self._ws_tokens = 0
        self._ws: Dict[str, torch.Tensor] = {}
        self.ws_generation = 0
        self.fwd_version = 0
        self.host_drop_counter = 0
        self._build_shadows()
        self.step_state = torch.zeros(8, dtype=torch.float32, device=self.device)
        self.side = torch.cuda.Stream(device=self.device)
        self.side2 = torch.cuda.Stream(device=self.device)
        self.overlap = os.environ.get("SRFRD_OVERLAP", "1") != "0"
        self.drop_seed = 0x5EED5EED
        self.saved: Optional[_Saved] = None
        self._plans: Dict[Tuple[int, int], ops.PackedPlan] = {}
        self._lives: Dict[Tuple[int, int], ops.LiveTiles] = {}
        self.packed_default = os.environ.get("SRFRD_PACKED", "1") != "0"
        self.fuse_ffn = os.environ.get("SRFRD_FUSE_FFN", "1") != "0"
        self.fuse_ln = os.environ.get("SRFRD_FUSE_LN", "1") != "0"
        self.hybrid = os.environ.get("SRFRD_HYBRID", "1") != "0"
        self.live_tiles = os.environ.get("SRFRD_LIVE_TILES", "1") != "0"

    def _build_shadows(self):
        s, P, dev = self.spec, self.P, self.device
        H, D, Hp, Dp = s.H, s.D, s.Hp, s.Dp
        self.sh: Dict[str, torch.Tensor] = {}
        self.vsh: Dict[str, torch.Tensor] = {}
        entries = []
        zb = lambda r, c: torch.zeros(r, c, dtype=bf16, device=dev)

        def vec(name, src, n_pad, dst_off=0, dst=None):
            if not s.padded:
                return
            if dst is None:
                dst = self.vsh.setdefault(name, torch.zeros(n_pad, dtype=torch.float32, device=dev))
            entries.append((src.view(1, -1), dst[dst_off:dst_off + src.numel()].view(1, -1), None))

        for i in range(s.num_blocks):
            win = P.mat(f"attention_layers.{i}.in_proj_weight")
            bin_ = P.view(f"attention_layers.{i}.in_proj_bias")
            self.sh[f"wq{i}"] = zb(Hp, Hp)
            self.sh[f"wkv{i}"] = zb(2 * Hp, Hp)
            self.sh[f"wqT{i}"] = zb(Hp, Hp)
            self.sh[f"wkvT{i}"] = zb(Hp, 2 * Hp)
            entries.append((win[:H], self.sh[f"wq{i}"][:H, :H], self.sh[f"wqT{i}"][:H, :H]))
            entries.append((win[H:2 * H], self.sh[f"wkv{i}"][:H, :H], self.sh[f"wkvT{i}"][:H, :H]))
            entries.append((win[2 * H:], self.sh[f"wkv{i}"][Hp:Hp + H, :H], self.sh[f"wkvT{i}"][:H, Hp:Hp + H]))
            vec(f"bq{i}", bin_[:H], Hp)
            vec(f"bkv{i}", bin_[H:2 * H], 2 * Hp)
            vec(f"bkv{i}", bin_[2 * H:], 2 * Hp, dst_off=Hp)
            for tag, key in (("wo", f"attention_layers.{i}.out_proj"), ("w1", f"forward_layers.{i}.conv1"),
                             ("w2", f"forward_layers.{i}.conv2")):
                self.sh[f"{tag}{i}"] = zb(Hp, Hp)
                self.sh[f"{tag}T{i}"] = zb(Hp, Hp)
                entries.append((P.mat(key + ".weight"), self.sh[f"{tag}{i}"][:H, :H], self.sh[f"{tag}T{i}"][:H, :H]))
                vec(f"b{tag[1]}{i}", P.view(key + ".bias"), Hp)
        if s.kind == "SRFR":
            self.sh["wc"] = zb(Dp, Hp)
            self.sh["wcT"] = zb(Hp, Dp)
            entries.append((P.mat("last_conv.weight"), self.sh["wc"][:D, :H], self.sh["wcT"][:H, :D]))
            vec("bc", P.view("last_conv.bias"), Dp)
        self._cast_entries = entries
        self._cast_table, self._cast_n = ops.make_cast_table(entries, dev)
        self.shadows_version = -1

    def enable_ce_table(self) -> torch.Tensor:
        if "ce_table" not in self.sh:
            s = self.spec
            E = self.P.view(s.item_key)
            self.sh["ce_table"] = torch.zeros(E.shape[0], s.Dp, dtype=bf16, device=self.device)
            for r0 in range(0, E.shape[0], 4096):
                self._cast_entries.append((E[r0:r0 + 4096], self.sh["ce_table"][r0:r0 + 4096, :s.D], None))
            self._cast_table, self._cast_n = ops.make_cast_table(self._cast_entries, self.device)
            self.refresh_shadows()
        return self.sh["ce_table"]

    def bias(self, tag: str, i: Optional[int] = None) -> torch.Tensor:
        s, P = self.spec, self.P
        if s.padded:
            return self.vsh[tag if i is None else f"{tag}{i}"]
        if tag == "bq":
            return P.view(f"attention_layers.{i}.in_proj_bias")[:s.H]
        if tag == "bkv":
            return P.view(f"attention_layers.{i}.in_proj_bias")[s.H:]
        if tag == "bc":
            return P.view("last_conv.bias")
        key = {"bo": f"attention_layers.{i}.out_proj.bias", "b1": f"forward_layers.{i}.conv1.bias",
               "b2": f"forward_layers.{i}.conv2.bias"}[tag]
        return P.view(key)

    def refresh_shadows(self):
        ops.cast_weights(self._cast_table, self._cast_n)

    @contextmanager
    def _branch(self, second: bool = False):
        if not self.overlap:
            yield
            return
        main = torch.cuda.current_stream()
        st = self.side2 if second else self.side
        st.wait_stream(main)
        with torch.cuda.stream(st):
            yield

    def _join(self, second: bool = False):
        if self.overlap:
            torch.cuda.current_stream().wait_stream(self.side2 if second else self.side)

    def _workspace(self, T: int, L: int) -> Dict[str, torch.Tensor]:
        if T <= self._ws_tokens:
            return self._ws
        s, dev = self.spec, self.device
        Lmax = max(L, s.max_len)
        H, nb = s.Hp, s.num_blocks
        ws: Dict[str, torch.Tensor] = {}

        def act(name, w=H, dtype=bf16):
            ws[name] = torch.zeros(T, w, dtype=dtype, device=dev)

        for i in range(nb + 1):
            act(f"x{i}")
        for i in range(nb):
            for n in ("Q", "q", "o", "r", "y", "h1"):
                act(f"{n}{i}")
            act(f"kv{i}", 2 * H)
            act(f"st1_{i}", 2, torch.float32)
            act(f"st2_{i}", 2, torch.float32)
            if Lmax > 128:
                ws[f"ast{i}"] = torch.zeros(T * s.num_heads, 4, dtype=torch.float32, device=dev)
        if s.kind == "SRFR":
            act("c", s.Dp)
        act("stF", 2, torch.float32)
        act("hfin", s.Doutp, torch.float32)
        act("dh", s.Doutp, torch.float32)
        for n in ("gA", "gC", "gD", "gX"):
            act(n)
        for i in range(nb):
            for n in ("gda1_", "gdr_", "gdq_"):
                act(f"{n}{i}")
            act(f"gdz_{i}")
            act(f"gdkv_{i}", 2 * H)
        if s.kind == "SRFR":
            act("gc", s.Dp)
        if s.dropout > 0:
            for i in range(nb):
                act(f"gE_{i}")
        ws["pos_tmp"] = torch.zeros(Lmax * H, dtype=torch.float32, device=dev)
        self._ws, self._ws_tokens = ws, T
        self.ws_generation += 1
        return ws

    def packed_ok(self, B: int, L: int) -> bool:
        return self.packed_mode(B, L) is not None

    def packed_mode(self, B: int, L: int) -> Optional[str]:
        s = self.spec
        if s.padded or s.H % 16 or s.D % 8 or B > 16384 or B < 1:
            return None
        if ops.attention_packed_supported(L, s.H, s.num_heads):
            return "tile"
        if self.hybrid and L <= 4096:
            return "hybrid"
        return None

    def _hybrid_ws(self, Td: int) -> Dict[str, torch.Tensor]:
        hw = getattr(self, "_hws", None)
        if hw is not None and hw["_rows"] >= Td:
            return hw
        s, dev = self.spec, self.device
        Hp = s.Hp
        hw = {"_rows": Td}
        z = lambda w: torch.zeros(Td, w, dtype=bf16, device=dev)
        for i in range(s.num_blocks):
            hw[f"qd{i}"], hw[f"kvd{i}"], hw[f"od{i}"] = z(Hp), z(2 * Hp), z(Hp)
        hw["dod"], hw["dqd"], hw["dkvd"] = z(Hp), z(Hp), z(2 * Hp)
        self._hws = hw
        self.ws_generation += 1
        return hw

    def _cached(self, cache: dict, key, make):
        if key not in cache:
            if len(cache) >= 4:
                cache.clear()
                self.ws_generation += 1
            cache[key] = make()
        return cache[key]

    def _aux_ids(self, fake_ids: Optional[torch.Tensor], B: int, L: int) -> Optional[torch.Tensor]:
        s = self.spec
        if s.mode == 1:
            return None if fake_ids is None else fake_ids.contiguous()
        if s.mode != 2:
            return None
        aux_ids = torch.empty(B, dtype=torch.int64, device=self.device)
        ops.srfu_labels(fake_ids.contiguous(), {"SRFU_B": 0, "SRFU_F": 1, "SRFU_R": 2}[s.kind], aux_ids)
        need = {"SRFU_B": 3, "SRFU_F": L + 1, "SRFU_R": 11}[s.kind]
        if s.n_labels < need and B > 0 and int(aux_ids.max()) >= s.n_labels:
            raise IndexError(f"index out of range in self: {s.kind} user label {int(aux_ids.max())} needs "
                             f"number_of_labels >= {need}, got {s.n_labels}")
        return aux_ids

    def forward(self, seq: torch.Tensor, fake_ids: Optional[torch.Tensor], training: bool,
                last_only: bool = False, save: Optional[bool] = None, packed: bool = False,
                keep: Optional[torch.Tensor] = None) -> torch.Tensor:
        s, P = self.spec, self.P
        B, L = seq.shape
        if L > s.max_len:
            raise RuntimeError(f"sequence length {L} exceeds max_len {s.max_len} (pos_embed rows, SRFR_model.py:12)")
        H, Hp, nb = s.H, s.Hp, s.num_blocks
        plan = self._cached(self._plans, (B, L), lambda: ops.PackedPlan(B, L, self.device)) if packed else None
        T = plan.cap if packed else B * L
        ws = self._workspace(T, L)
        self.fwd_version += 1
        p_drop = s.dropout if training else 0.0
        step = self.step_state[3:4] if p_drop > 0 else None
        seed = (self.drop_seed + self.host_drop_counter * 0x9E3779B97F4A7C15) & 0xFFFFFFFFFFFFFFFF
        seq = seq.contiguous()
        aux_ids = self._aux_ids(fake_ids, B, L)
        hyb = live = None
        if packed:
            plan.build(seq, None if keep is None else keep.contiguous())
            if self.packed_mode(B, L) == "hybrid":
                hyb = self._hybrid_ws(B * L)
                if self.live_tiles:
                    live = self._cached(self._lives, (B, L), lambda: ops.LiveTiles(B, L, s.num_heads, self.device))
                    live.build(plan)
        fuse_ln = H == Hp and Hp <= 128 and self.fuse_ln
        oproj = 0
        if packed and hyb is None and s.num_heads == 1 and fuse_ln:
            oproj = ops.attention_packed_oproj_supported(L, H, s.num_heads)
        sv = _Saved(seq=seq, aux_ids=aux_ids, B=B, L=L, T=T, row_ids=plan.row_ids if packed else seq.view(-1), plan=plan,
                    hyb=hyb, live=live, p_drop=p_drop, seed=seed, step=step, fuse_ln=fuse_ln, oproj=oproj,
                    mlp2=packed and self.fuse_ffn and Hp <= 128, version=self.fwd_version)
        x = [ws[f"x{i}"][:T] for i in range(nb + 1)]
        with ops.row_limit(plan.rows) if packed else nullcontext():
            emb = (P.view(s.item_key), P.view(s.pos_key), P.view(s.aux_key) if s.aux_key else None, s.mode, seq, aux_ids,
                   s.item_scale, P.view("attention_layernorms.0.weight"), P.view("attention_layernorms.0.bias"), LN_EPS)
            emb_drop = dict(drop_p=p_drop if s.kind == "SASRec" else 0.0, drop_seed=seed, drop_stream=1, drop_step=step)
            if packed:
                ops.embed_ln_fwd_packed(*emb, x[0], ws["Q0"][:T], ws["st1_0"][:T], plan, **emb_drop)
            else:
                ops.embed_ln_fwd(*emb, x0_bf16=x[0], q_bf16=ws["Q0"][:T], stats=ws["st1_0"][:T], **emb_drop)
            for i in range(nb):
                Q, q, kv, o, r, y, h1 = (ws[f"{n}{i}"][:T] for n in ("Q", "q", "kv", "o", "r", "y", "h1"))
                with self._branch():
                    ops.gemm_tn(x[i], self.sh[f"wkv{i}"], out_bf16=kv, bias=self.bias("bkv", i))
                if i > 0 and not fuse_ln:
                    ops.layernorm_fwd(x[i], P.view(f"attention_layernorms.{i}.weight"), P.view(f"attention_layernorms.{i}.bias"),
                                      LN_EPS, y_bf16=Q, stats=ws[f"st1_{i}"][:T], H=H)
                ops.gemm_tn(Q, self.sh[f"wq{i}"], out_bf16=q, bias=self.bias("bq", i))
                self._join()
                ln2 = dict(ln_w=P.view(f"forward_layernorms.{i}.weight"), ln_b=P.view(f"forward_layernorms.{i}.bias"),
                           ln_eps=LN_EPS, ln_stats=ws[f"st2_{i}"][:T])
                fold = dict(wo=self.sh[f"wo{i}"], bias=self.bias("bo", i), residual=Q, r=r, y=y, **ln2) if oproj & 1 else {}
                self._attention_fwd(sv, i, q, kv, o, ws.get(f"ast{i}"), fold)
                if oproj & 1:
                    pass
                elif fuse_ln:
                    ops.gemm_tn(o, self.sh[f"wo{i}"], out_bf16=r, bias=self.bias("bo", i), residual=Q, ln_out=y, **ln2)
                else:
                    ops.gemm_tn(o, self.sh[f"wo{i}"], out_bf16=r, bias=self.bias("bo", i), residual=Q)
                    ops.layernorm_fwd(r, ln2["ln_w"], ln2["ln_b"], LN_EPS, y_bf16=y, stats=ln2["ln_stats"], H=H)
                nxt = {}
                if fuse_ln and i + 1 < nb:
                    nxt = dict(ln_out=ws[f"Q{i + 1}"][:T], ln_w=P.view(f"attention_layernorms.{i + 1}.weight"),
                               ln_b=P.view(f"attention_layernorms.{i + 1}.bias"), ln_eps=LN_EPS,
                               ln_stats=ws[f"st1_{i + 1}"][:T])
                if sv.mlp2:
                    ops.mlp2_tn(y, self.sh[f"w1{i}"], self.sh[f"w2{i}"], h1, x[i + 1], bias1=self.bias("b1", i),
                                bias2=self.bias("b2", i), relu1=True, drop1_p=p_drop, drop2_p=p_drop, drop1_stream=11 + 4 * i,
                                drop2_stream=12 + 4 * i, drop_seed=seed, drop_step=step, residual_is_a=True,
                                row_ids=sv.row_ids, **nxt)
                else:
                    ops.gemm_tn(y, self.sh[f"w1{i}"], out_bf16=h1, bias=self.bias("b1", i), relu=True,
                                drop_p=p_drop, drop_seed=seed, drop_stream=11 + 4 * i, drop_step=step)
                    ops.gemm_tn(h1, self.sh[f"w2{i}"], out_bf16=x[i + 1], bias=self.bias("b2", i), residual=y,
                                row_ids=sv.row_ids, drop_p=p_drop, drop_seed=seed, drop_stream=12 + 4 * i, drop_step=step,
                                **nxt)
            fin_in = x[nb]
            if s.kind == "SRFR":
                ops.gemm_tn(x[nb], self.sh["wc"], out_bf16=ws["c"][:T], bias=self.bias("bc"))
                fin_in = ws["c"][:T]
            if not last_only:
                ops.layernorm_fwd(fin_in, P.view("last_layernorm.weight"), P.view("last_layernorm.bias"), LN_EPS,
                                  y_f32=ws["hfin"][:T], stats=ws["stF"][:T], H=s.Dout)
        if last_only:
            out = ws["hfin"][:B]
            if packed:
                ops.layernorm_fwd_rows(fin_in, P.view("last_layernorm.weight"), P.view("last_layernorm.bias"), LN_EPS, out,
                                       plan.last_row, B, s.Dout)
            else:
                ops.layernorm_fwd(fin_in, P.view("last_layernorm.weight"), P.view("last_layernorm.bias"), LN_EPS, y_f32=out,
                                  T=B, H=s.Dout, row_stride=L, row_offset=L - 1)
            return out[:, :s.Dout]
        if training if save is None else save:
            self.saved = sv
        return ws["hfin"][:T] if packed else ws["hfin"][:T].view(B, L, s.Doutp)[..., :s.Dout]

    def _attention_fwd(self, sv: "_Saved", i: int, q, kv, o, stats, fold: dict) -> None:
        s, Hp = self.spec, self.spec.Hp
        drop = (sv.p_drop, sv.seed, 10 + 4 * i, sv.step)
        if sv.plan is not None and sv.hyb is None:
            ops.attention_fwd_packed(q, kv[:, :Hp], kv[:, Hp:], o, sv.plan, sv.L, s.H, s.num_heads, *drop, **fold)
            return
        qd, kvd, od = q, kv, o
        if sv.hyb is not None:
            Td = sv.B * sv.L
            qd, kvd, od = sv.hyb[f"qd{i}"][:Td], sv.hyb[f"kvd{i}"][:Td], sv.hyb[f"od{i}"][:Td]
            ops.unpack_rows([(q, qd, Hp, 0), (kv, kvd, 2 * Hp, 0)], sv.plan)
        with sv.live.active() if sv.live is not None else nullcontext():
            ops.attention_fwd(qd, kvd[:, :Hp], kvd[:, Hp:], od, sv.B, sv.L, s.H, s.num_heads, *drop, stats=stats)
        if sv.hyb is not None:
            ops.pack_rows([(od, o, Hp, 0)], sv.plan)

    def check_saved(self, version: Optional[int] = None) -> "_Saved":
        sv = self.saved
        if sv is None and version is None:
            raise RuntimeError("backward() without a training forward()")
        if sv is None or sv.version != self.fwd_version or (version is not None and version != sv.version):
            raise RuntimeError("srfrd_b200: backward() of a stale forward -- another forward() (training, validation or "
                               "predict) ran on this model after the one being back-propagated and overwrote the shared "
                               "activation workspace; run backward() before the next forward()")
        return sv

    def backward(self, dh: torch.Tensor, version: Optional[int] = None) -> None:
        s, P = self.spec, self.P
        sv = self.check_saved(version)
        T, H, Hp, nb = sv.T, s.H, s.Hp, s.num_blocks
        ws = self._ws
        row_ids = sv.row_ids
        p_drop, seed, step = sv.p_drop, sv.seed, sv.step
        gA, gC, gD, gX = (ws[n][:T] for n in ("gA", "gC", "gD", "gX"))
        G = lambda name: P.view(name, grad=True)
        GM = lambda name: P.mat(name, grad=True)
        x = [ws[f"x{i}"][:T] for i in range(nb + 1)]
        dz_top = ws[f"gdz_{nb - 1}"][:T]
        with ops.row_limit(sv.plan.rows) if sv.plan is not None else nullcontext():
            if s.kind == "SRFR":
                gc = ws["gc"][:T]
                ops.layernorm_bwd(dh, ws["c"][:T], ws["stF"][:T], P.view("last_layernorm.weight"), gc,
                                  G("last_layernorm.weight"), G("last_layernorm.bias"), H=s.D)
                with self._branch():
                    ops.gemm_wgrad(gc, x[nb], GM("last_conv.weight"), G("last_conv.bias"), Mo=s.D, No=H)
                ops.gemm_tn(gc, self.sh["wcT"], out_bf16=dz_top, row_ids=row_ids)
            else:
                ops.layernorm_bwd(dh, x[nb], ws["stF"][:T], P.view("last_layernorm.weight"), dz_top,
                                  G("last_layernorm.weight"), G("last_layernorm.bias"), row_ids=row_ids, H=s.Dout)

            for i in reversed(range(nb)):
                Q, q, kv, o, r, y, h1 = (ws[f"{n}{i}"][:T] for n in ("Q", "q", "kv", "o", "r", "y", "h1"))
                dz, da1, dr, dq, dkv = (ws[f"{n}{i}"][:T] for n in ("gdz_", "gda1_", "gdr_", "gdq_", "gdkv_"))
                dx_out = ws[f"gdz_{i - 1}"][:T] if i > 0 else gA
                dz2 = dz
                if p_drop > 0:
                    dz2 = ws[f"gE_{i}"][:T]
                    ops.dropout_apply(dz, dz2, Hp, p_drop, seed, 12 + 4 * i, step)
                with self._branch():
                    ops.gemm_wgrad(dz2, h1, GM(f"forward_layers.{i}.conv2.weight"), G(f"forward_layers.{i}.conv2.bias"),
                                   Mo=H, No=H)
                if sv.mlp2:
                    ops.mlp2_tn(dz2, self.sh[f"w2T{i}"], self.sh[f"w1T{i}"], da1, gC, gate=h1, drop1_p=p_drop,
                                drop1_stream=11 + 4 * i, drop_seed=seed, drop_step=step, residual=dz)
                else:
                    ops.gemm_tn(dz2, self.sh[f"w2T{i}"], out_bf16=da1, gate=h1, drop_p=p_drop, drop_seed=seed,
                                drop_stream=11 + 4 * i, drop_step=step)
                with self._branch():
                    ops.gemm_wgrad(da1, y, GM(f"forward_layers.{i}.conv1.weight"), G(f"forward_layers.{i}.conv1.bias"),
                                   Mo=H, No=H)
                if not sv.mlp2:
                    ops.gemm_tn(da1, self.sh[f"w1T{i}"], out_bf16=gC, residual=dz)
                ops.layernorm_bwd(gC, r, ws[f"st2_{i}"][:T], P.view(f"forward_layernorms.{i}.weight"), dr,
                                  G(f"forward_layernorms.{i}.weight"), G(f"forward_layernorms.{i}.bias"), H=H)
                with self._branch():
                    ops.gemm_wgrad(dr, o, GM(f"attention_layers.{i}.out_proj.weight"),
                                   G(f"attention_layers.{i}.out_proj.bias"), Mo=H, No=H)
                if not sv.oproj & 2:
                    ops.gemm_tn(dr, self.sh[f"woT{i}"], out_bf16=gC)
                self._attention_bwd(sv, i, gC, q, kv, o, dq, dkv, dr, ws.get(f"ast{i}"))
                gin = GM(f"attention_layers.{i}.in_proj_weight")
                gbin = G(f"attention_layers.{i}.in_proj_bias")
                with self._branch():
                    ops.gemm_wgrad(dq, Q, gin[:H], gbin[:H], Mo=H, No=H)
                    if Hp == H:
                        ops.gemm_wgrad(dkv, x[i], gin[H:], gbin[H:], Mo=2 * H, No=H)
                    else:
                        ops.gemm_wgrad(dkv[:, :Hp], x[i], gin[H:2 * H], gbin[H:2 * H], Mo=H, No=H)
                        ops.gemm_wgrad(dkv[:, Hp:], x[i], gin[2 * H:], gbin[2 * H:], Mo=H, No=H)
                with self._branch(second=True):
                    ops.gemm_tn(dkv, self.sh[f"wkvT{i}"], out_bf16=gX)
                ops.gemm_tn(dq, self.sh[f"wqT{i}"], out_bf16=gD, residual=dr)
                self._join(second=True)
                ops.layernorm_bwd(gD, x[i], ws[f"st1_{i}"][:T], P.view(f"attention_layernorms.{i}.weight"), dx_out,
                                  G(f"attention_layernorms.{i}.weight"), G(f"attention_layernorms.{i}.bias"),
                                  add=gX, row_ids=row_ids, H=H)
            dx0 = gA
            if s.kind == "SASRec" and p_drop > 0:
                ops.dropout_apply(gA, gC, H, p_drop, seed, 1, step)
                dx0 = gC

        aux_grad = G(s.aux_key) if s.aux_key else None
        F = s.F if s.mode == 1 else 0
        if sv.plan is not None:
            ops.embed_bwd_packed(dx0, sv.seq, sv.aux_ids, sv.plan, s.D, F, s.mode, s.item_scale, G(s.item_key), aux_grad,
                                 G(s.pos_key))
        else:
            ops.embed_bwd(dx0, sv.seq, sv.aux_ids, s.D, F, s.mode, s.item_scale, G(s.item_key), aux_grad)
            LH = sv.L * Hp
            pos_tmp = ws["pos_tmp"][:LH]
            ops.colsum(dx0, pos_tmp, M=sv.B, N=LH, ld=LH)
            ops.add_segments(pos_tmp, LH, Hp, s.D, G(s.pos_key))
        self._join()
        self.saved = None

    def _attention_bwd(self, sv: "_Saved", i: int, do, q, kv, o, dq, dkv, dr, stats) -> None:
        s, Hp = self.spec, self.spec.Hp
        drop = (sv.p_drop, sv.seed, 10 + 4 * i, sv.step)
        if sv.plan is not None and sv.hyb is None:
            fold = dict(dr=dr, woT=self.sh[f"woT{i}"]) if sv.oproj & 2 else {}
            ops.attention_bwd_packed(None if fold else do, q, kv[:, :Hp], kv[:, Hp:], dq, dkv[:, :Hp], dkv[:, Hp:], sv.plan,
                                     sv.L, s.H, s.num_heads, *drop, **fold)
            return
        dqd, dkvd = dq, dkv
        if sv.hyb is not None:
            Td, hyb = sv.B * sv.L, sv.hyb
            q, kv, o = hyb[f"qd{i}"][:Td], hyb[f"kvd{i}"][:Td], hyb[f"od{i}"][:Td]
            dod, dqd, dkvd = hyb["dod"][:Td], hyb["dqd"][:Td], hyb["dkvd"][:Td]
            ops.unpack_rows([(do, dod, Hp, 1)], sv.plan)
            do = dod
        with sv.live.active() if sv.live is not None else nullcontext():
            ops.attention_bwd(do, q, kv[:, :Hp], kv[:, Hp:], dqd, dkvd[:, :Hp], dkvd[:, Hp:], sv.B, sv.L, s.H, s.num_heads,
                              *drop, o=o, stats=stats)
        if sv.hyb is not None:
            ops.pack_rows([(dqd, dq, Hp, 0), (dkvd, dkv, 2 * Hp, 1)], sv.plan)

    def fake_table(self) -> Optional[torch.Tensor]:
        return self.P.view("embedding_layer.fake_embed.weight") if self.spec.kind == "SRFRN" else None

    def fake_table_grad(self) -> Optional[torch.Tensor]:
        return self.P.view("embedding_layer.fake_embed.weight", grad=True) if self.spec.kind == "SRFRN" else None
```

### srfrd_b200/ops.py

```python
from __future__ import annotations

import ctypes as C
from typing import Optional

import torch

from . import _lib
from contextlib import contextmanager

from ._lib import CastDesc, GemmEpilogue, Mlp2Epilogue, PackDesc, RepackPart, call

bf16 = torch.bfloat16


def _p(t: Optional[torch.Tensor]):
    return None if t is None else t.data_ptr()


def _stream():
    return torch.cuda.current_stream().cuda_stream


def _chk(t: torch.Tensor, dtype, name: str):
    if not t.is_cuda:
        raise RuntimeError(f"srfrd_b200: {name} must be a CUDA tensor (there is no CPU fallback)")
    if t.dtype != dtype:
        raise RuntimeError(f"srfrd_b200: {name} must be {dtype}, got {t.dtype}")
    if t.stride(-1) != 1:
        raise RuntimeError(f"srfrd_b200: {name} must be contiguous in its last dimension")


def embed_ln_fwd(item_table, pos_table, aux_table, mode, seq, aux_ids, item_scale, ln_w, ln_b, eps,
                 x0_bf16=None, x0_f32=None, q_bf16=None, stats=None, drop_p=0.0, drop_seed=0, drop_stream=0,
                 drop_step=None):
    _lib.require_device()
    B, L = seq.shape
    D = item_table.shape[1]
    F = aux_table.shape[1] if (aux_table is not None and mode == 1) else 0
    _chk(item_table, torch.float32, "item_table"); _chk(seq, torch.int64, "seq")
    ldx = (x0_bf16 if x0_bf16 is not None else q_bf16).stride(0) if (x0_bf16 is not None or q_bf16 is not None) else D + F
    call("srfrd_embed_ln_fwd", _p(item_table), item_table.shape[0], D, _p(pos_table), _p(aux_table),
         0 if aux_table is None else aux_table.shape[0], F, mode, _p(seq), _p(aux_ids), B, L, float(item_scale),
         _p(ln_w), _p(ln_b), float(eps), _p(x0_bf16), _p(x0_f32), _p(q_bf16), _p(stats), ldx, float(drop_p),
         int(drop_seed), int(drop_stream), _p(drop_step), _stream())


def srfu_labels(fake_ids, kind: int, labels):
    _lib.require_device()
    B, L = fake_ids.shape
    call("srfrd_srfu_labels", _p(fake_ids), B, L, kind, _p(labels), _stream())


def embed_bwd(dx0, seq, aux_ids, D, F, mode, item_scale, d_item, d_aux):
    B, L = seq.shape
    call("srfrd_embed_bwd", _p(dx0), dx0.stride(0), _p(seq), _p(aux_ids), B, L, D, F, mode, float(item_scale),
         _p(d_item), _p(d_aux), _stream())


def layernorm_fwd(x, w, b, eps, y_bf16=None, y_f32=None, stats=None, T=None, H=None, row_stride=1, row_offset=0):
    _lib.require_device()
    T = x.shape[0] if T is None else T
    H = x.shape[1] if H is None else H
    y = y_bf16 if y_bf16 is not None else y_f32
    call("srfrd_layernorm_fwd", _p(x), x.stride(0), _p(w), _p(b), float(eps), _p(y_bf16), _p(y_f32), y.stride(0),
         _p(stats), T, H, row_stride, row_offset, _stream())


def layernorm_bwd(dy, x, stats, w, dx, dw, db, add=None, row_ids=None, H=None):
    T = x.shape[0]
    H = x.shape[1] if H is None else H
    dyb = dy if dy.dtype == bf16 else None
    dyf = dy if dy.dtype == torch.float32 else None
    call("srfrd_layernorm_bwd", _p(dyb), _p(dyf), dy.stride(0), _p(x), x.stride(0), _p(stats), _p(w), _p(add),
         0 if add is None else add.stride(0), _p(row_ids), _p(dx), dx.stride(0), _p(dw), _p(db), T, H, _stream())


def gemm_tn(A, B, out_bf16=None, out_f32=None, bias=None, residual=None, gate=None, row_ids=None, relu=False,
            drop_p=0.0, drop_seed=0, drop_stream=0, drop_step=None, M=None, ln_out=None, ln_w=None, ln_b=None, ln_eps=0.0,
            ln_stats=None):
    _lib.require_device()
    M = A.shape[0] if M is None else M
    K = A.shape[1]
    N = B.shape[0]
    out = out_bf16 if out_bf16 is not None else out_f32
    ep = GemmEpilogue(_p(bias), _p(residual), _p(gate), _p(row_ids), _p(out_bf16), _p(out_f32),
                      0 if residual is None else residual.stride(0), 0 if gate is None else gate.stride(0),
                      out.stride(0), int(relu), float(drop_p), int(drop_stream), int(drop_seed), _p(drop_step),
                      _p(ln_out), _p(ln_w), _p(ln_b), _p(ln_stats), 0 if ln_out is None else ln_out.stride(0), float(ln_eps))
    call("srfrd_gemm_tn", _p(A), A.stride(0), _p(B), B.stride(0), M, N, K, C.byref(ep), _stream())


def gemm_wgrad(dY, X, dW, dbias=None, Mo=None, No=None):
    T = dY.shape[0]
    Mo = dY.shape[1] if Mo is None else Mo
    No = X.shape[1] if No is None else No
    call("srfrd_gemm_wgrad", _p(dY), dY.stride(0), _p(X), X.stride(0), T, Mo, No, _p(dW), dW.stride(0), _p(dbias),
         _stream())


def gemm_ref(A, B, Cout, a_mn_major=False, b_mn_major=False):
    _lib.require_device()
    M, N = Cout.shape
    K = A.shape[0] if a_mn_major else A.shape[1]
    call("srfrd_gemm_ref", _p(A), A.stride(0), _p(B), B.stride(0), _p(Cout), Cout.stride(0), M, N, K,
         int(a_mn_major), int(b_mn_major), _stream())


def colsum(X, out, M=None, N=None, ld=None):
    M = X.shape[0] if M is None else M
    N = X.shape[1] if N is None else N
    ld = X.stride(0) if ld is None else ld
    call("srfrd_colsum", _p(X), M, N, ld, _p(out), _stream())


def add_segments(src, n, seg_in, seg_out, out):
    call("srfrd_add_segments", _p(src), n, seg_in, seg_out, _p(out), _stream())


def dropout_apply(x, out, N, drop_p, seed, stream_id, drop_step=None):
    call("srfrd_dropout_apply", _p(x), x.stride(0), _p(out), out.stride(0), x.shape[0], N, float(drop_p), int(seed),
         int(stream_id), _p(drop_step), _stream())


def cast_weights(descs_dev, n):
    call("srfrd_cast_weights", _p(descs_dev), n, _stream())


def make_cast_table(entries, device):
    arr = (CastDesc * len(entries))()
    for i, (src, dst, dst_t) in enumerate(entries):
        is_f32 = int(dst is not None and dst.dtype == torch.float32)
        arr[i] = CastDesc(src.data_ptr(), src.stride(0), _p(dst), 0 if dst is None else dst.stride(0), _p(dst_t),
                          0 if dst_t is None else dst_t.stride(0), src.shape[0], src.shape[1], is_f32)
    raw = bytes(arr)
    host = torch.frombuffer(bytearray(raw), dtype=torch.uint8)
    return host.to(device), len(entries)


def f32_to_bf16_split(src, hi, lo=None, row_index=None):
    _lib.require_device()
    rows = src.shape[0] if row_index is None else row_index.numel()
    cols = src.shape[1]
    call("srfrd_f32_to_bf16_split", _p(src), src.stride(0), _p(row_index), _p(hi), _p(lo), rows, cols, hi.stride(0),
         _stream())


def attention_fwd(q, k, v, o, B, L, H, heads, drop_p=0.0, seed=0, stream_id=0, drop_step=None, stats=None):
    _lib.require_device()
    call("srfrd_attention_fwd", _p(q), q.stride(0), _p(k), _p(v), k.stride(0), _p(o), o.stride(0), _p(stats), B, L, H, heads,
         float(drop_p), int(seed), int(stream_id), _p(drop_step), _stream())


def attention_bwd(dout, q, k, v, dq, dk, dv, B, L, H, heads, drop_p=0.0, seed=0, stream_id=0, drop_step=None, o=None,
                  stats=None):
    call("srfrd_attention_bwd", _p(dout), dout.stride(0), _p(q), q.stride(0), _p(k), _p(v), k.stride(0), _p(o),
         0 if o is None else o.stride(0), _p(stats), _p(dq), dq.stride(0), _p(dk), _p(dv), dk.stride(0), B, L, H, heads,
         float(drop_p), int(seed), int(stream_id), _p(drop_step), _stream())


def score_fwd(h, item_table, fake_table, pos, neg, prs, nrs, zp, zn):
    _lib.require_device()
    T = pos.numel()
    D = item_table.shape[1]
    F = 0 if fake_table is None else fake_table.shape[1]
    call("srfrd_score_fwd", _p(h), h.stride(0), _p(item_table), _p(fake_table), _p(pos), _p(neg), _p(prs), _p(nrs), T,
         D, F, _p(zp), _p(zn), _stream())


def score_bwd(h, item_table, fake_table, pos, neg, prs, nrs, dzp, dzn, dh, d_item, d_fake):
    T = pos.numel()
    D = item_table.shape[1]
    F = 0 if fake_table is None else fake_table.shape[1]
    call("srfrd_score_bwd", _p(h), h.stride(0), _p(item_table), _p(fake_table), _p(pos), _p(neg), _p(prs), _p(nrs),
         _p(dzp), _p(dzn), T, D, F, _p(dh), dh.stride(0), _p(d_item), _p(d_fake), _stream())


def score_loss_fused(h, item_table, fake_table, pos, neg, prs, nrs, w_pos, w_neg, norm, loss_acc, dh, d_item, d_fake,
                     zp=None, zn=None):
    T = pos.numel()
    D = item_table.shape[1]
    F = 0 if fake_table is None else fake_table.shape[1]
    call("srfrd_score_loss_fused", _p(h), h.stride(0), _p(item_table), _p(fake_table), _p(pos), _p(neg), _p(prs),
         _p(nrs), _p(w_pos), _p(w_neg), _p(norm), T, D, F, _p(zp), _p(zn), _p(loss_acc), _p(dh),
         0 if dh is None else dh.stride(0), _p(d_item), _p(d_fake), _stream())


def weight_sums(pos, w_pos, w_neg, out2):
    _lib.require_device()
    call("srfrd_weight_sums", _p(pos), _p(w_pos), _p(w_neg), pos.numel(), _p(out2), _stream())


def loss_finalize(acc2, norm2, loss):
    call("srfrd_loss_finalize", _p(acc2), _p(norm2), _p(loss), _stream())


def adam_tick(state3, beta1, beta2):
    call("srfrd_adam_tick", _p(state3), float(beta1), float(beta2), _stream())


def adam_step(p, g, m, v, lr, beta1, beta2, eps, state3, zero_grad=True):
    _lib.require_device()
    call("srfrd_adam_step", _p(p), _p(g), _p(m), _p(v), p.numel(), float(lr), float(beta1), float(beta2), float(eps),
         _p(state3), int(zero_grad), _stream())


def adam_step_fused(p, g, m, v, lr, beta1, beta2, eps, state8, zero_grad=True, acc2=None, norm2=None, loss=None,
                    l2: Optional["ParamL2"] = None):
    _lib.require_device()
    call("srfrd_adam_step_fused", _p(p), _p(g), _p(m), _p(v), p.numel(), float(lr), float(beta1), float(beta2), float(eps),
         _p(state8), int(zero_grad), _p(acc2), _p(norm2), _p(loss), _stream(), *_l2_args(l2))


class ParamL2:

    def __init__(self, segments, l2: float, device):
        host = (C.c_int64 * (2 * len(segments)))(*[int(x) for s in segments for x in s])
        n_chunks = C.c_int64(0)
        call("srfrd_param_l2_plan", host, len(segments), C.byref(n_chunks))
        self.n_seg, self.n_chunks, self.l2 = len(segments), int(n_chunks.value), float(l2)
        self.seg = torch.tensor([int(x) for s in segments for x in s], dtype=torch.int64).to(device)
        self.coef = torch.zeros(self.n_seg, dtype=torch.float32, device=device)
        self.reg = torch.zeros(1, dtype=torch.float32, device=device)
        self.ws = torch.zeros(self.n_chunks + 1, dtype=torch.float64, device=device)

    def launch(self, p: torch.Tensor):
        _lib.require_device()
        _chk(p, torch.float32, "p")
        call("srfrd_param_l2", _p(p), _p(self.seg), self.n_seg, self.n_chunks, self.l2, _p(self.coef), _p(self.reg),
             _p(self.ws), _stream())


def _l2_args(l2: Optional[ParamL2]):
    return (None, 0, None, None) if l2 is None else (_p(l2.seg), l2.n_seg, _p(l2.coef), _p(l2.reg))


def catalogue_topk_plan(U, n_rows, row_lo, D, n_split, k=10) -> int:
    out = C.c_int(0)
    call("srfrd_catalogue_topk_plan", U, n_rows, row_lo, D, n_split, C.byref(out), int(k))
    return out.value


def catalogue_topk_kmax(D, n_split) -> int:
    out = C.c_int(0)
    call("srfrd_catalogue_topk_kmax", D, n_split, C.byref(out))
    return out.value


def catalogue_topk(feats, U, u_pad, n_split, table, row_lo, id_base, chunks, part_scores, part_ids, packed=None, k=10):
    _lib.require_device()
    D = table.shape[1]
    call("srfrd_catalogue_topk", _p(feats), U, u_pad, n_split, _p(table), table.shape[0], row_lo, id_base, D,
         feats.stride(0), table.stride(0), chunks, _p(part_scores), _p(part_ids), _p(packed), _stream(), int(k))


def catalogue_rank(feats, U, u_pad, n_split, table, row_lo, id_base, target_rows, target_ids, rank_out,
                   target_scores=None):
    _lib.require_device()
    D = table.shape[1]
    call("srfrd_catalogue_rank", _p(feats), U, u_pad, n_split, _p(table), table.shape[0], row_lo, id_base, D,
         feats.stride(0), table.stride(0), _p(target_rows), target_rows.stride(0), _p(target_ids), _p(target_scores),
         _p(rank_out), _stream())


def merge_topk_packed(packed, U, nlists, k, out_scores, out_ids):
    _lib.require_device()
    call("srfrd_merge_topk_packed", _p(packed), U, nlists, k, _p(out_scores), _p(out_ids), _stream())


def merge_topk(scores, ids, U, nlists, k, out_scores, out_ids):
    _lib.require_device()
    call("srfrd_merge_topk", _p(scores), _p(ids), U, nlists, k, _p(out_scores), _p(out_ids), _stream())


def sample_batch(offsets, items, labels, p_fake, eligible, itemnum, B, L, policy, seed, step, out, w_pos=None):
    _lib.require_device()
    call("srfrd_sample_batch", _p(offsets), _p(items), _p(labels), _p(p_fake), _p(eligible), eligible.numel(), int(itemnum),
         B, L, int(policy), int(seed), _p(step), _p(out.get("users")), _p(out["seq"]), _p(out["rsq"]), _p(out["pos"]),
         _p(out["prs"]), _p(out["neg"]), _p(out["nrs"]), _p(w_pos), _stream())


def sample_candidates(offsets, items, users0, target, itemnum, C, seed, cand):
    _lib.require_device()
    call("srfrd_sample_candidates", _p(offsets), _p(items), _p(users0), _p(target), users0.numel(), int(itemnum), int(C),
         int(seed), _p(cand), _stream())


def candidate_rank(feats, item_table, cand, D, fake_table=None, user_label=None, logits=None, rank=None, err_flag=None):
    _lib.require_device()
    _chk(feats, torch.float32, "feats"); _chk(item_table, torch.float32, "item_table"); _chk(cand, torch.int64, "cand")
    U, Cn = cand.shape
    F = 0 if fake_table is None else fake_table.shape[1]
    call("srfrd_candidate_rank", _p(feats), feats.stride(0), _p(item_table), item_table.shape[0], int(D), _p(cand), U, Cn,
         _p(fake_table), F, _p(user_label), _p(logits), 0 if logits is None else logits.stride(0), _p(rank), _p(err_flag),
         _stream())


def add_user_term(logits, feats_tail, fake_table, label):
    _lib.require_device()
    U, I = logits.shape
    call("srfrd_add_user_term", _p(logits), logits.stride(0), U, I, _p(feats_tail), feats_tail.stride(0), _p(fake_table),
         _p(label), fake_table.shape[1], _stream())


class PackedPlan:

    def __init__(self, B: int, L: int, device):
        self.B, self.L = B, L
        self.cap = (B * (L + 1) + 127) // 128 * 128
        i32 = lambda n: torch.zeros(n, dtype=torch.int32, device=device)
        self.rows, self.cnt, self.seq_first = i32(4), i32(B), i32(B + 1)
        self.tok_row, self.row_tok = i32(B * L), i32(self.cap)
        self.row_ids = torch.zeros(self.cap, dtype=torch.int64, device=device)
        self.row_info = i32(4 * self.cap)
        self.tile_row0, self.last_row = i32(B + 130), i32(B)
        self.desc = PackDesc(_p(self.rows), _p(self.cnt), _p(self.seq_first), _p(self.tok_row), _p(self.row_tok),
                             _p(self.row_ids), _p(self.row_info), _p(self.tile_row0), _p(self.last_row), self.cap)

    def build(self, seq, keep=None):
        _lib.require_device()
        B, L = seq.shape
        assert (B, L) == (self.B, self.L)
        _chk(seq, torch.int64, "seq")
        call("srfrd_pack_plan", _p(seq), _p(keep), B, L, C.byref(self.desc), _stream())


@contextmanager
def row_limit(rows_dev):
    call("srfrd_set_row_limit", _p(rows_dev))
    try:
        yield
    finally:
        call("srfrd_set_row_limit", None)


class LiveTiles:

    def __init__(self, B: int, L: int, heads: int, device):
        nq = (L + 127) // 128
        self.B, self.L, self.heads = B, L, heads
        self.q_lo = torch.zeros(B, dtype=torch.int32, device=device)
        self.items = torch.zeros(B * heads * nq, dtype=torch.int32, device=device)
        self.n_live = torch.zeros(1, dtype=torch.int32, device=device)

    def build(self, plan: "PackedPlan"):
        _lib.require_device()
        assert (plan.B, plan.L) == (self.B, self.L)
        self.tok_row = plan.tok_row
        call("srfrd_attention_live_items", _p(plan.tok_row), self.B, self.L, self.heads, _p(self.q_lo), _p(self.items),
             _p(self.n_live), _stream())

    @contextmanager
    def active(self):
        call("srfrd_set_attention_live", _p(self.q_lo), _p(self.items), _p(self.n_live), _p(self.tok_row))
        try:
            yield
        finally:
            call("srfrd_set_attention_live", None, None, None, None)


def attention_packed_supported(L: int, H: int, heads: int) -> bool:
    return bool(_lib.load().srfrd_attention_packed_supported(int(L), int(H), int(heads)))


def embed_ln_fwd_packed(item_table, pos_table, aux_table, mode, seq, aux_ids, item_scale, ln_w, ln_b, eps, x0_bf16, q_bf16,
                        stats, plan: PackedPlan, drop_p=0.0, drop_seed=0, drop_stream=0, drop_step=None):
    _lib.require_device()
    B, L = seq.shape
    D = item_table.shape[1]
    F = aux_table.shape[1] if (aux_table is not None and mode == 1) else 0
    call("srfrd_embed_ln_fwd_packed", _p(item_table), item_table.shape[0], D, _p(pos_table), _p(aux_table),
         0 if aux_table is None else aux_table.shape[0], F, mode, _p(seq), _p(aux_ids), B, L, float(item_scale), _p(ln_w),
         _p(ln_b), float(eps), _p(x0_bf16), _p(q_bf16), _p(stats), x0_bf16.stride(0), float(drop_p), int(drop_seed),
         int(drop_stream), _p(drop_step), _p(plan.row_tok), _p(plan.rows), plan.cap, _stream())


def layernorm_fwd_rows(x, w, b, eps, y_f32, row_index, n, H):
    _lib.require_device()
    call("srfrd_layernorm_fwd_rows", _p(x), x.stride(0), _p(w), _p(b), float(eps), _p(y_f32), y_f32.stride(0), _p(row_index),
         n, H, _stream())


def attention_packed_oproj_supported(L: int, H: int, heads: int) -> int:
    return int(_lib.load().srfrd_attention_packed_oproj_supported(int(L), int(H), int(heads)))


def attention_fwd_packed(q, k, v, o, plan: PackedPlan, L, H, heads, drop_p=0.0, seed=0, stream_id=0, drop_step=None,
                         wo=None, bias=None, residual=None, r=None, y=None, ln_w=None, ln_b=None, ln_eps=0.0, ln_stats=None):
    _lib.require_device()
    st = lambda t: 0 if t is None else t.stride(0)
    call("srfrd_attention_fwd_packed", _p(q), q.stride(0), _p(k), _p(v), k.stride(0), _p(o), o.stride(0), C.byref(plan.desc),
         L, H, heads, float(drop_p), int(seed), int(stream_id), _p(drop_step), _stream(), _p(wo), st(wo), _p(bias),
         _p(residual), st(residual), _p(ln_w), _p(ln_b), float(ln_eps), _p(ln_stats), _p(r), st(r), _p(y), st(y))


def attention_bwd_packed(dout, q, k, v, dq, dk, dv, plan: PackedPlan, L, H, heads, drop_p=0.0, seed=0, stream_id=0,
                         drop_step=None, dr=None, woT=None):
    st = lambda t: 0 if t is None else t.stride(0)
    call("srfrd_attention_bwd_packed", _p(dout), st(dout), _p(q), q.stride(0), _p(k), _p(v), k.stride(0), _p(dq),
         dq.stride(0), _p(dk), _p(dv), dk.stride(0), C.byref(plan.desc), L, H, heads, float(drop_p), int(seed),
         int(stream_id), _p(drop_step), _stream(), _p(dr), st(dr), _p(woT), st(woT))


def score_loss_fused_packed(h, item_table, fake_table, pos, neg, prs, nrs, w_pos, w_neg, norm, loss_acc, dh, d_item, d_fake,
                            plan: PackedPlan):
    D = item_table.shape[1]
    F = 0 if fake_table is None else fake_table.shape[1]
    call("srfrd_score_loss_fused_packed", _p(h), h.stride(0), _p(item_table), _p(fake_table), _p(pos), _p(neg), _p(prs),
         _p(nrs), _p(w_pos), _p(w_neg), _p(norm), D, F, _p(loss_acc), _p(dh), dh.stride(0), _p(d_item), _p(d_fake),
         _p(plan.row_tok), _p(plan.rows), plan.cap, _stream())


def embed_bwd_packed(dx0, seq, aux_ids, plan: PackedPlan, D, F, mode, item_scale, d_item, d_aux, d_pos):
    B, L = seq.shape
    call("srfrd_embed_bwd_packed", _p(dx0), dx0.stride(0), _p(seq), _p(aux_ids), _p(plan.row_tok), _p(plan.rows), plan.cap,
         L, D, F, mode, float(item_scale), _p(d_item), _p(d_aux), _p(d_pos), _stream())


def dp_adam_step(grad_ptrs_dev: int, param_ptrs_dev: int, signal_ptrs_dev: int, rank, world, n, m, v, lr, beta1, beta2, eps,
                 state8, norm2, local4, l2: Optional[ParamL2] = None):
    _lib.require_device()
    call("srfrd_dp_adam_step", grad_ptrs_dev, param_ptrs_dev, signal_ptrs_dev, int(rank), int(world), int(n), _p(m), _p(v),
         float(lr), float(beta1), float(beta2), float(eps), _p(state8), _p(norm2), _p(local4), _stream(), *_l2_args(l2))


def _parts(parts):
    arr = (RepackPart * len(parts))()
    for i, (src, dst, W, mode) in enumerate(parts):
        arr[i] = RepackPart(_p(src), src.stride(0), _p(dst), dst.stride(0), int(W), int(mode))
    return arr


def unpack_rows(parts, plan: PackedPlan):
    _lib.require_device()
    arr = _parts(parts)
    call("srfrd_unpack_rows", arr, len(parts), C.byref(plan.desc), plan.B, plan.L, _stream())


def pack_rows(parts, plan: PackedPlan):
    _lib.require_device()
    arr = _parts(parts)
    call("srfrd_pack_rows", arr, len(parts), C.byref(plan.desc), plan.B, plan.L, _stream())


def mlp2_tn(A, W1, W2, mid_out, out, bias1=None, bias2=None, gate=None, relu1=False, drop1_p=0.0, drop2_p=0.0, drop1_stream=0,
            drop2_stream=0, drop_seed=0, drop_step=None, residual=None, residual_is_a=False, row_ids=None, ln_out=None,
            ln_w=None, ln_b=None, ln_stats=None, ln_eps=0.0, M=None):
    _lib.require_device()
    M = A.shape[0] if M is None else M
    N = W1.shape[0]
    ep = Mlp2Epilogue(_p(bias1), _p(bias2), _p(gate), 0 if gate is None else gate.stride(0), int(relu1), float(drop1_p),
                      float(drop2_p), int(drop1_stream), int(drop2_stream), int(drop_seed), _p(drop_step), _p(residual),
                      0 if residual is None else residual.stride(0), int(residual_is_a), _p(row_ids), _p(mid_out),
                      mid_out.stride(0), _p(out), out.stride(0), _p(ln_out), 0 if ln_out is None else ln_out.stride(0),
                      _p(ln_w), _p(ln_b), _p(ln_stats), float(ln_eps))
    call("srfrd_mlp2_tn", _p(A), A.stride(0), _p(W1), W1.stride(0), _p(W2), W2.stride(0), M, N, C.byref(ep), _stream())


def catalogue_ce_plan(Dp: int):
    smem, stages, tmem = C.c_int64(0), C.c_int(0), C.c_int(0)
    call("srfrd_catalogue_ce_plan", int(Dp), C.byref(smem), C.byref(stages), C.byref(tmem))
    return int(smem.value), int(stages.value), int(tmem.value)


def _ce_rows(h, plan):
    return (None, None, h.shape[0]) if plan is None else (plan.row_tok, plan.rows, plan.cap)


def catalogue_ce_fwd(h, table, pos, w_pos, lse, loss_acc, plan: Optional[PackedPlan] = None):
    _lib.require_device()
    _chk(h, bf16, "h"); _chk(table, bf16, "table"); _chk(pos, torch.int64, "pos")
    row_tok, rows, cap = _ce_rows(h, plan)
    call("srfrd_catalogue_ce_fwd", _p(h), h.stride(0), _p(table), table.stride(0), table.shape[0] - 1, table.shape[1],
         _p(pos), _p(w_pos), _p(row_tok), _p(rows), cap, _p(lse), _p(loss_acc), _stream())


def catalogue_ce_bwd(h, table, pos, w_pos, norm, lse, dh, d_item, D, plan: Optional[PackedPlan] = None):
    _lib.require_device()
    _chk(h, bf16, "h"); _chk(table, bf16, "table"); _chk(pos, torch.int64, "pos")
    row_tok, rows, cap = _ce_rows(h, plan)
    call("srfrd_catalogue_ce_bwd", _p(h), h.stride(0), _p(table), table.stride(0), table.shape[0] - 1, table.shape[1],
         int(D), _p(pos), _p(w_pos), _p(norm), _p(row_tok), _p(rows), cap, _p(lse), _p(dh),
         0 if dh is None else dh.stride(0), _p(d_item), 0 if d_item is None else d_item.stride(0), _stream())
```

Baseline: 9.834 million.

## Split pack planning and fuse row fill with embedding LayerNorm

Pack planning is split into three steps. The first computes offsets with a multi-block count plus last-block scan, replacing the single-block 1024-thread scan. The second fills the packed rows and computes the embedding and LayerNorm for those rows in the same kernel. The third builds the attention tile plan on a side stream that is joined before the first attention. This removes separate kernel launches and a global round trip, and takes the serial scan off the critical path, at the cost of more complex code and atomic last-block coordination.

```diff
diff --git a/include/srfrd_b200.h b/include/srfrd_b200.h
--- a/include/srfrd_b200.h
+++ b/include/srfrd_b200.h
@@ -8,7 +8,7 @@
 extern "C" {
 #endif
 
-#define SRFRD_ABI_VERSION 10
+#define SRFRD_ABI_VERSION 11
 #if defined(__GNUC__)
 #define SRFRD_API __attribute__((visibility("default")))
 #else
@@ -175,6 +175,15 @@
   int64_t cap;
 } srfrd_pack_t;
 SRFRD_API int srfrd_pack_plan(const int64_t* seq, const int64_t* keep, int64_t B, int L, const srfrd_pack_t* pk, void* stream);
+SRFRD_API int srfrd_pack_offsets(const int64_t* seq, const int64_t* keep, int64_t B, int L, const srfrd_pack_t* pk,
+                                 void* stream);
+SRFRD_API int srfrd_pack_embed_ln_fwd(const int64_t* seq, const int64_t* keep, int64_t B, int L, const srfrd_pack_t* pk,
+                                      const float* item_table, int64_t n_rows, int D, const float* pos_table,
+                                      const float* aux_table, int64_t n_aux, int F, int mode, const int64_t* aux_ids,
+                                      float item_scale, const float* ln_w, const float* ln_b, float eps, void* x0_bf16,
+                                      void* q_bf16, float* stats, int ldx, float drop_p, uint64_t drop_seed,
+                                      uint32_t drop_stream, const float* drop_step, void* stream);
+SRFRD_API int srfrd_pack_tiles(int64_t B, int L, const srfrd_pack_t* pk, void* stream);
 SRFRD_API int srfrd_set_row_limit(const int* rows_dev);
 SRFRD_API int srfrd_embed_ln_fwd_packed(const float* item_table, int64_t n_rows, int D, const float* pos_table,
                               const float* aux_table, int64_t n_aux, int F, int mode, const int64_t* seq,
diff --git a/srfrd_b200/_lib.py b/srfrd_b200/_lib.py
--- a/srfrd_b200/_lib.py
+++ b/srfrd_b200/_lib.py
@@ -86,6 +86,10 @@
     "srfrd_pack_rows": [C.POINTER(RepackPart), i32, C.POINTER(PackDesc), i64, i32, vp],
     "srfrd_dp_adam_step": [vp, vp, vp, i32, i32, i64, vp, vp, f32, f32, f32, f32, vp, vp, vp, vp, vp, i32, vp, vp],
     "srfrd_pack_plan": [vp, vp, i64, i32, C.POINTER(PackDesc), vp],
+    "srfrd_pack_offsets": [vp, vp, i64, i32, C.POINTER(PackDesc), vp],
+    "srfrd_pack_embed_ln_fwd": [vp, vp, i64, i32, C.POINTER(PackDesc), vp, i64, i32, vp, vp, i64, i32, i32, vp, f32, vp, vp,
+                                f32, vp, vp, vp, i32, f32, u64, u32, vp, vp],
+    "srfrd_pack_tiles": [i64, i32, C.POINTER(PackDesc), vp],
     "srfrd_set_row_limit": [vp],
     "srfrd_embed_ln_fwd_packed": [vp, i64, i32, vp, vp, i64, i32, i32, vp, vp, i64, i32, f32, vp, vp, f32, vp, vp, vp, i32,
                                   f32, u64, u32, vp, vp, vp, i64, vp],
@@ -125,7 +129,7 @@
         fn = getattr(lib, name)
         fn.argtypes = argtypes
         fn.restype = C.c_int
-    if lib.srfrd_abi_version() != 10:
+    if lib.srfrd_abi_version() != 11:
         raise RuntimeError("srfrd_b200: ABI version mismatch between _lib.py and the built library")
     _lib = lib
     return lib
diff --git a/srfrd_b200/csrc/embed_row.cuh b/srfrd_b200/csrc/embed_row.cuh
--- /dev/null
+++ b/srfrd_b200/csrc/embed_row.cuh
@@ -0,0 +1,173 @@
+#pragma once
+#include "common.cuh"
+
+namespace srfrd {
+
+static constexpr int MAXW = 512;
+
+template <int LPR>
+__device__ __forceinline__ float group_sum(float v) {
+#pragma unroll
+  for (int o = LPR / 2; o > 0; o >>= 1) v += __shfl_xor_sync(0xffffffffu, v, o);
+  return v;
+}
+
+__device__ __forceinline__ void unpack8(const uint4& u, float* f) {
+  const uint32_t w[4] = {u.x, u.y, u.z, u.w};
+#pragma unroll
+  for (int i = 0; i < 4; ++i) {
+    const float2 t = __bfloat1622float2(*reinterpret_cast<const __nv_bfloat162*>(&w[i]));
+    f[2 * i] = t.x; f[2 * i + 1] = t.y;
+  }
+}
+__device__ __forceinline__ uint4 pack8(const float* f) {
+  return make_uint4(pack_bf16x2(f[0], f[1]), pack_bf16x2(f[2], f[3]), pack_bf16x2(f[4], f[5]), pack_bf16x2(f[6], f[7]));
+}
+__device__ __forceinline__ void load8_f32(const float* p, float* f) {
+  const float4 a = __ldg(reinterpret_cast<const float4*>(p)), b = __ldg(reinterpret_cast<const float4*>(p) + 1);
+  f[0] = a.x; f[1] = a.y; f[2] = a.z; f[3] = a.w; f[4] = b.x; f[5] = b.y; f[6] = b.z; f[7] = b.w;
+}
+__device__ __forceinline__ void load8_f32_stream(const float* p, float* f) {
+  float4 a, b;
+  asm volatile("ld.global.nc.L1::no_allocate.L2::256B.v4.f32 {%0,%1,%2,%3}, [%4];"
+               : "=f"(a.x), "=f"(a.y), "=f"(a.z), "=f"(a.w) : "l"(p));
+  asm volatile("ld.global.nc.L1::no_allocate.L2::256B.v4.f32 {%0,%1,%2,%3}, [%4];"
+               : "=f"(b.x), "=f"(b.y), "=f"(b.z), "=f"(b.w) : "l"(p + 4));
+  f[0] = a.x; f[1] = a.y; f[2] = a.z; f[3] = a.w; f[4] = b.x; f[5] = b.y; f[6] = b.z; f[7] = b.w;
+}
+__device__ __forceinline__ void store8_f32(float* p, const float* f) {
+  reinterpret_cast<float4*>(p)[0] = make_float4(f[0], f[1], f[2], f[3]);
+  reinterpret_cast<float4*>(p)[1] = make_float4(f[4], f[5], f[6], f[7]);
+}
+
+struct EmbedParams {
+  const float* item_table;
+  const float* pos_table;
+  const float* aux_table;
+  const int64_t* seq;
+  const int64_t* aux_ids;
+  const int* row_tok;
+  const int* rows_dev;
+  int64_t T;
+  int L, D, F, mode;
+  float item_scale;
+  const float* ln_w;
+  const float* ln_b;
+  float eps;
+  bf16* x0;
+  float* x0_f32;
+  bf16* q;
+  float* stats;
+  int ldx;
+  uint64_t drop_seed; uint32_t drop_thresh, drop_stream; float drop_scale; const float* drop_step;
+};
+
+template <int LPR, int CH, int MODE, bool DROP>
+__device__ __forceinline__ void embed_ln_row(const EmbedParams& p, int64_t t, bool row_ok, int64_t id, int64_t aid, int l,
+                                             int sub) {
+  const int H = p.D + (MODE == 1 ? p.F : 0);
+  const float invH = 1.f / (float)H;
+  const bool has_ln = p.ln_w != nullptr;
+  const bool valid = row_ok && id != 0;
+  const float* erow = p.item_table + id * p.D;
+  const float* prow = p.pos_table + (int64_t)l * p.D;
+  const float* arow = p.aux_table + aid * (MODE == 1 ? p.F : p.D);
+  float v[CH][8];
+  float e[CH][8];
+#pragma unroll
+  for (int ch = 0; ch < CH; ++ch) {
+    const int c = (ch * LPR + sub) * 8;
+#pragma unroll
+    for (int j = 0; j < 8; ++j) e[ch][j] = 0.f;
+    if (valid && c < H) {
+      if (MODE != 1 || c < p.D) load8_f32_stream(erow + c, e[ch]);
+      else load8_f32(arow + (c - p.D), e[ch]);
+    }
+  }
+  float sum = 0.f;
+#pragma unroll
+  for (int ch = 0; ch < CH; ++ch) {
+    const int c = (ch * LPR + sub) * 8;
+#pragma unroll
+    for (int j = 0; j < 8; ++j) v[ch][j] = e[ch][j];
+    if (valid && c < p.D) {
+      float pp[8];
+      load8_f32(prow + c, pp);
+#pragma unroll
+      for (int j = 0; j < 8; ++j) {
+        float x = e[ch][j];
+        if (p.item_scale != 1.f) x = __fmul_rn(x, p.item_scale);
+        v[ch][j] = __fadd_rn(x, pp[j]);
+      }
+      if (MODE == 2) {
+        float u[8];
+        load8_f32(arow + c, u);
+#pragma unroll
+        for (int j = 0; j < 8; ++j) v[ch][j] = __fadd_rn(v[ch][j], u[j]);
+      }
+    }
+    if (DROP) {
+      if (valid && c < H) {
+#pragma unroll
+        for (int j = 0; j < 8; ++j)
+          v[ch][j] = dropout_keep(p.drop_seed, p.drop_stream, (uint64_t)t * H + c + j, p.drop_thresh)
+                         ? v[ch][j] * p.drop_scale : 0.f;
+      }
+    }
+    sum += ((v[ch][0] + v[ch][1]) + (v[ch][2] + v[ch][3])) + ((v[ch][4] + v[ch][5]) + (v[ch][6] + v[ch][7]));
+  }
+  float a = 0.f, nb = 0.f, mean = 0.f;
+  if (has_ln) {
+    mean = group_sum<LPR>(sum) * invH;
+    float sq = 0.f;
+#pragma unroll
+    for (int ch = 0; ch < CH; ++ch) {
+      if ((ch * LPR + sub) * 8 < H) {
+        float d[8];
+#pragma unroll
+        for (int j = 0; j < 8; ++j) d[j] = v[ch][j] - mean;
+        sq += ((d[0] * d[0] + d[1] * d[1]) + (d[2] * d[2] + d[3] * d[3])) + ((d[4] * d[4] + d[5] * d[5]) + (d[6] * d[6] + d[7] * d[7]));
+      }
+    }
+    a = rsqrtf(group_sum<LPR>(sq) * invH + p.eps);
+    nb = -mean * a;
+  }
+  if (!row_ok) return;
+#pragma unroll
+  for (int ch = 0; ch < CH; ++ch) {
+    const int c = (ch * LPR + sub) * 8;
+    if (c >= H) continue;
+    if (p.x0_f32) store8_f32(p.x0_f32 + t * H + c, v[ch]);
+    if (p.x0) *reinterpret_cast<uint4*>(p.x0 + t * p.ldx + c) = pack8(v[ch]);
+    if (has_ln) {
+      float w[8], b[8], y[8];
+      load8_f32(p.ln_w + c, w);
+      load8_f32(p.ln_b + c, b);
+#pragma unroll
+      for (int j = 0; j < 8; ++j) y[j] = fmaf(fmaf(v[ch][j], a, nb), w[j], b[j]);
+      *reinterpret_cast<uint4*>(p.q + t * p.ldx + c) = pack8(y);
+    }
+  }
+  if (has_ln && p.stats && sub == 0) *reinterpret_cast<float2*>(p.stats + 2 * t) = make_float2(mean, a);
+}
+
+#define SRFRD_ROW_DISPATCH(H, CALL)                      \
+  do {                                                   \
+    if ((H) <= 32) { CALL(4, 1); }                       \
+    else if ((H) <= 64) { CALL(8, 1); }                  \
+    else if ((H) <= 96) { CALL(4, 3); }                  \
+    else if ((H) <= 128) { CALL(16, 1); }                \
+    else if ((H) <= 192) { CALL(8, 3); }                 \
+    else if ((H) <= 256) { CALL(32, 1); }                \
+    else if ((H) <= 384) { CALL(16, 3); }                \
+    else { CALL(32, 2); }                                \
+  } while (0)
+
+
+int embed_params(EmbedParams& p, bool& vec, const float* item_table, int D, const float* pos_table, const float* aux_table,
+                 int F, int mode, const int64_t* seq, const int64_t* aux_ids, int64_t B, int L, float item_scale,
+                 const float* ln_w, const float* ln_b, float eps, void* x0_bf16, float* x0_f32, void* q_bf16, float* stats,
+                 int ldx, float drop_p, uint64_t drop_seed, uint32_t drop_stream, const float* drop_step, const int* row_tok,
+                 const int* rows_dev, int64_t cap_rows);
+
+}
diff --git a/srfrd_b200/csrc/pack.cu b/srfrd_b200/csrc/pack.cu
--- a/srfrd_b200/csrc/pack.cu
+++ b/srfrd_b200/csrc/pack.cu
@@ -1,15 +1,15 @@
 #include "common.cuh"
+#include "embed_row.cuh"
 #include "srfrd_b200.h"
 
 namespace srfrd {
 
 static constexpr int PACK_TILE = 128;
-static constexpr int SCAN_THREADS = 1024;
-
-__global__ void __launch_bounds__(256) pack_count_kernel(const int64_t* seq, const int64_t* keep, int64_t B, int L, int* cnt) {
-  const int lane = threadIdx.x & 31;
-  const int64_t b = (int64_t)blockIdx.x * (blockDim.x >> 5) + (threadIdx.x >> 5);
-  if (b >= B) return;
+static constexpr int PACK_SEQS = 8;
+static constexpr int PACK_THREADS = 32 * PACK_SEQS;
+static constexpr int TILE_THREADS = 128;
+
+__device__ __forceinline__ int pack_count(const int64_t* seq, const int64_t* keep, int64_t b, int L, int lane) {
   int n = 0;
   for (int l0 = 0; l0 < L; l0 += 32) {
     const int l = l0 + lane;
@@ -17,123 +17,210 @@
     if (l < L) k = (__ldg(seq + b * L + l) != 0) || (keep && __ldg(keep + b * L + l) != 0);
     n += __popc(__ballot_sync(0xffffffffu, k));
   }
-  if (lane == 0) cnt[b] = n;
-}
-
-__device__ __forceinline__ int pack_bound(const int* first, int B, int Tp, int i) { return i <= B ? first[min(i, B)] + 0 : Tp + (i - B); }
-
-__global__ void __launch_bounds__(SCAN_THREADS) pack_scan_kernel(srfrd_pack_t pk, int64_t B, int plan_tiles) {
-  extern __shared__ int sm[];
-  __shared__ int wsum[32];
-  __shared__ int s_total;
+  return n;
+}
+
+__global__ void __launch_bounds__(PACK_THREADS) pack_offsets_kernel(const int64_t* seq, const int64_t* keep, int64_t B, int L,
+                                                                   int plan_tiles, srfrd_pack_t pk) {
+  __shared__ int s_rows[PACK_SEQS];
+  __shared__ bool s_last;
+  pdl_prologue_done();
   const int tid = threadIdx.x, lane = tid & 31, warp = tid >> 5;
-  int* first = sm;
-  const int per = (int)((B + SCAN_THREADS - 1) / SCAN_THREADS);
-  const int64_t b0 = (int64_t)tid * per, b1 = min(B, b0 + per);
+  const int64_t b0 = (int64_t)blockIdx.x * PACK_SEQS, b = b0 + warp;
+  int n = 0;
+  if (b < B) {
+    n = pack_count(seq, keep, b, L, lane);
+    if (lane == 0) pk.cnt[b] = n;
+  }
+  if (lane == 0) s_rows[warp] = b < B ? n + 1 : 0;
+  __syncthreads();
+  if (tid == 0) {
+    int tot = 0;
+    for (int w = 0; w < PACK_SEQS; ++w) tot += s_rows[w];
+    pk.seq_first[b0] = tot;
+    __threadfence();
+    s_last = atomicAdd(pk.rows + 3, 1) == (int)gridDim.x - 1;
+  }
+  __syncthreads();
+  if (!s_last) return;
+  __threadfence();
+  const int nblk = (int)gridDim.x;
+  const int per = (nblk + PACK_THREADS - 1) / PACK_THREADS;
+  const int j0 = min(nblk, tid * per), j1 = min(nblk, j0 + per);
   int local = 0;
-  for (int64_t b = b0; b < b1; ++b) local += pk.cnt[b] + 1;
+  for (int j = j0; j < j1; ++j) local += __ldcg(pk.seq_first + (int64_t)j * PACK_SEQS);
   int incl = local;
 #pragma unroll
   for (int o = 1; o < 32; o <<= 1) { const int v = __shfl_up_sync(0xffffffffu, incl, o); if (lane >= o) incl += v; }
-  if (lane == 31) wsum[warp] = incl;
-  __syncthreads();
-  if (warp == 0) {
-    int v = wsum[lane];
-#pragma unroll
-    for (int o = 1; o < 32; o <<= 1) { const int u = __shfl_up_sync(0xffffffffu, v, o); if (lane >= o) v += u; }
-    wsum[lane] = v;
-    if (lane == 31) s_total = v;
-  }
-  __syncthreads();
-  int run = incl - local + (warp ? wsum[warp - 1] : 0);
-  for (int64_t b = b0; b < b1; ++b) { first[b] = run; pk.seq_first[b] = run; run += pk.cnt[b] + 1; }
-  const int Tp = s_total;
+  if (lane == 31) s_rows[warp] = incl;
+  __syncthreads();
+  int run = incl - local, Tp = 0;
+  for (int w = 0; w < PACK_SEQS; ++w) { if (w < warp) run += s_rows[w]; Tp += s_rows[w]; }
+  for (int j = j0; j < j1; ++j) {
+    const int v = __ldcg(pk.seq_first + (int64_t)j * PACK_SEQS);
+    pk.seq_first[(int64_t)j * PACK_SEQS] = run;
+    run += v;
+  }
   const int M = (Tp + PACK_TILE - 1) / PACK_TILE * PACK_TILE;
-  if (tid == 0) { first[B] = Tp; pk.seq_first[B] = Tp; pk.rows[0] = M; pk.rows[1] = Tp; }
-  __syncthreads();
-  for (int r = Tp + tid; r < M; r += SCAN_THREADS) {
+  if (tid == 0) {
+    pk.seq_first[B] = Tp;
+    pk.rows[0] = M;
+    pk.rows[1] = Tp;
+    pk.rows[3] = 0;
+    if (!plan_tiles) { pk.rows[2] = 0; pk.tile_row0[0] = M; }
+  }
+  for (int r = Tp + tid; r < M; r += PACK_THREADS) {
     pk.row_tok[r] = -1;
     pk.row_ids[r] = 0;
     reinterpret_cast<int4*>(pk.row_info)[r] = make_int4(r, r + 1, __float_as_int(1.f), 0);
   }
-  if (!plan_tiles) {
-    if (tid == 0) { pk.rows[2] = 0; pk.rows[3] = 0; pk.tile_row0[0] = M; }
-    return;
-  }
-  const int NB = (int)B + (M - Tp);
-  int* nxt = sm + B + 1;
-  for (int i = tid; i < NB; i += SCAN_THREADS) {
-    const int lim = pack_bound(first, (int)B, Tp, i) + PACK_TILE;
-    int lo = i + 1, hi = NB;
-    while (lo < hi) {
-      const int mid = (lo + hi + 1) >> 1;
-      if (pack_bound(first, (int)B, Tp, mid) <= lim) lo = mid; else hi = mid - 1;
-    }
-    nxt[i] = lo;
-  }
-  __syncthreads();
+}
+
+template <bool EMBED, int LPR, int CH, int MODE, bool DROP>
+__global__ void __launch_bounds__(PACK_THREADS, 4) pack_fill_kernel(const int64_t* seq, const int64_t* keep, int64_t B, int L,
+                                                                    srfrd_pack_t pk, EmbedParams p) {
+  pdl_prologue_done();
+  const int lane = threadIdx.x & 31, warp = threadIdx.x >> 5;
+  const int64_t b0 = (int64_t)blockIdx.x * PACK_SEQS, b = b0 + warp;
+  const int off = __ldcg(pk.seq_first + b0);
+  const int c = (lane < PACK_SEQS && b0 + lane < B) ? __ldg(pk.cnt + b0 + lane) + 1 : 0;
+  int incl = c;
+#pragma unroll
+  for (int o = 1; o < PACK_SEQS; o <<= 1) { const int v = __shfl_up_sync(0xffffffffu, incl, o); if (lane >= o) incl += v; }
+  const int row0 = off + __shfl_sync(0xffffffffu, incl - c, warp);
+  const int end = row0 + __shfl_sync(0xffffffffu, c, warp);
+  const int blk_end = off + __shfl_sync(0xffffffffu, incl, PACK_SEQS - 1);
+  if (b < B) {
+    int4* info = reinterpret_cast<int4*>(pk.row_info);
+    if (lane == 0) {
+      pk.seq_first[b] = row0;
+      pk.row_tok[row0] = -1;
+      pk.row_ids[row0] = 0;
+      info[row0] = make_int4(row0, end, __float_as_int(1.f), 0);
+    }
+    int base = 0;
+    int last = row0;
+    for (int l0 = 0; l0 < L; l0 += 32) {
+      const int l = l0 + lane;
+      int64_t id = 0;
+      bool k = false;
+      if (l < L) {
+        id = __ldg(seq + b * L + l);
+        k = (id != 0) || (keep && __ldg(keep + b * L + l) != 0);
+      }
+      const unsigned m = __ballot_sync(0xffffffffu, k);
+      const int before = base + __popc(m & ((1u << lane) - 1u));
+      const int row = row0 + 1 + before;
+      if (l < L) {
+        pk.tok_row[b * L + l] = k ? row : -1;
+        if (k) {
+          pk.row_tok[row] = (int)(b * L + l);
+          pk.row_ids[row] = id;
+          info[row] = make_int4(row0, end, __float_as_int((float)(l - before)), l);
+          if (l == L - 1) last = row;
+        }
+      }
+      base += __popc(m);
+    }
+    last = __shfl_sync(0xffffffffu, last, (L - 1) & 31);
+    if (lane == 0) pk.last_row[b] = last;
+  }
+  if constexpr (EMBED) {
+    const int hi = b0 + PACK_SEQS >= B ? __ldcg(pk.rows) : blk_end;
+    __syncthreads();
+    if (DROP) p.drop_seed = mix_seed(p.drop_seed, p.drop_step);
+    constexpr int RPW = 32 / LPR;
+    const int sub = lane % LPR, grp = lane / LPR;
+    for (int t0 = off + warp * RPW; t0 < hi; t0 += PACK_SEQS * RPW) {
+      const int t = t0 + grp;
+      const bool row_ok = t < hi;
+      const int src = row_ok ? __ldcg(pk.row_tok + t) : -1;
+      int64_t id = 0, aid = 0;
+      int l = 0;
+      if (src >= 0) {
+        l = src % L;
+        id = __ldg(seq + src);
+        if (MODE == 1) aid = p.aux_ids ? __ldg(p.aux_ids + src) : 0;
+        if (MODE == 2) aid = __ldg(p.aux_ids + src / L);
+      }
+      embed_ln_row<LPR, CH, MODE, DROP>(p, t, row_ok, id, aid, l, sub);
+    }
+  }
+}
+
+__device__ __forceinline__ int pack_size(const uint8_t* s_size, int B, int i) { return i < B ? s_size[i] : 1; }
+
+__device__ __forceinline__ int tile_block_scan(int v, int* s_w, int* total) {
+  const int lane = threadIdx.x & 31, warp = threadIdx.x >> 5;
+  int incl = v;
+#pragma unroll
+  for (int o = 1; o < 32; o <<= 1) { const int u = __shfl_up_sync(0xffffffffu, incl, o); if (lane >= o) incl += u; }
+  __syncthreads();
+  if (lane == 31) s_w[warp] = incl;
+  __syncthreads();
+  int ex = incl - v;
+  *total = 0;
+  for (int w = 0; w < TILE_THREADS / 32; ++w) { if (w < warp) ex += s_w[w]; *total += s_w[w]; }
+  return ex;
+}
+
+__global__ void __launch_bounds__(TILE_THREADS, 16) pack_tiles_kernel(srfrd_pack_t pk, int B) {
+  extern __shared__ uint8_t sm_tiles[];
+  uint8_t* s_size = sm_tiles;
+  uint8_t* s_step = sm_tiles + B;
+  __shared__ int s_w[TILE_THREADS / 32];
   __shared__ int s_ntiles;
-  if (tid == 0) {
-    int k = 0;
-    for (int i = 0; i < NB;) { const int j = nxt[i]; nxt[k++] = i; i = j; }
-    s_ntiles = k;
-    pk.rows[2] = k;
-    pk.rows[3] = 0;
-  }
-  __syncthreads();
-  const int nt = s_ntiles;
-  for (int k = tid; k < nt; k += SCAN_THREADS) pk.tile_row0[k] = pack_bound(first, (int)B, Tp, nxt[k]);
-  if (tid == 0) pk.tile_row0[nt] = M;
-}
-
-__global__ void __launch_bounds__(256) pack_fill_kernel(const int64_t* seq, const int64_t* keep, int64_t B, int L, srfrd_pack_t pk) {
-  const int lane = threadIdx.x & 31;
-  const int64_t b = (int64_t)blockIdx.x * (blockDim.x >> 5) + (threadIdx.x >> 5);
-  if (b >= B) return;
-  const int row0 = pk.seq_first[b], end = pk.seq_first[b + 1];
-  int4* info = reinterpret_cast<int4*>(pk.row_info);
-  if (lane == 0) {
-    pk.row_tok[row0] = -1;
-    pk.row_ids[row0] = 0;
-    info[row0] = make_int4(row0, end, __float_as_int(1.f), 0);
-  }
-  int base = 0;
-  int last = row0;
-  for (int l0 = 0; l0 < L; l0 += 32) {
-    const int l = l0 + lane;
-    int64_t id = 0;
-    bool k = false;
-    if (l < L) {
-      id = __ldg(seq + b * L + l);
-      k = (id != 0) || (keep && __ldg(keep + b * L + l) != 0);
-    }
-    const unsigned m = __ballot_sync(0xffffffffu, k);
-    const int before = base + __popc(m & ((1u << lane) - 1u));
-    const int row = row0 + 1 + before;
-    if (l < L) {
-      pk.tok_row[b * L + l] = k ? row : -1;
-      if (k) {
-        pk.row_tok[row] = (int)(b * L + l);
-        pk.row_ids[row] = id;
-        info[row] = make_int4(row0, end, __float_as_int((float)(l - before)), l);
-        if (l == L - 1) last = row;
-      }
-    }
-    base += __popc(m);
-  }
-  last = __shfl_sync(0xffffffffu, last, (L - 1) & 31);
-  if (lane == 0) pk.last_row[b] = last;
+  pdl_prologue_done();
+#pragma unroll 8
+  for (int i = threadIdx.x; i < B; i += TILE_THREADS) s_size[i] = (uint8_t)(__ldg(pk.cnt + i) + 1);
+  __syncthreads();
+  const int per = (B + PACK_TILE - 1 + TILE_THREADS - 1) / TILE_THREADS;
+  const int i0 = threadIdx.x * per, i1 = i0 + per;
+  int local = 0;
+  for (int i = i0; i < min(i1, B); ++i) local += s_size[i];
+  int Tp;
+  int bnd = tile_block_scan(local, s_w, &Tp) + max(0, i0 - B);
+  const int M = (Tp + PACK_TILE - 1) / PACK_TILE * PACK_TILE;
+  const int NB = B + (M - Tp), iend = min(i1, NB);
+  for (int i = i0, k = i0, span = 0; i < iend; ++i) {
+    for (; k < NB; ++k) {
+      const int sz = pack_size(s_size, B, k);
+      if (span + sz > PACK_TILE) break;
+      span += sz;
+    }
+    s_step[i] = (uint8_t)(k - i - 1);
+    span -= pack_size(s_size, B, i);
+  }
+  __syncthreads();
+  if (threadIdx.x == 0) {
+    int n = 0;
+    for (int i = 0; i < NB; ++n) {
+      const int d = s_step[i];
+      s_step[i] = (uint8_t)(d | 0x80);
+      i += d + 1;
+    }
+    s_ntiles = n;
+    pk.rows[2] = n;
+  }
+  __syncthreads();
+  int mine = 0;
+  for (int i = i0; i < iend; ++i) mine += s_step[i] >> 7;
+  int unused;
+  int k = tile_block_scan(mine, s_w, &unused);
+  for (int i = i0; i < iend; ++i) {
+    if (s_step[i] & 0x80) pk.tile_row0[k++] = bnd;
+    bnd += pack_size(s_size, B, i);
+  }
+  if (threadIdx.x == 0) pk.tile_row0[s_ntiles] = M;
 }
 
 }
 
 using namespace srfrd;
 
-extern "C" int srfrd_pack_plan(const int64_t* seq, const int64_t* keep, int64_t B, int L, const srfrd_pack_t* pk_host,
-                               void* stream_) {
-  cudaStream_t stream = (cudaStream_t)stream_;
+static int pack_check(const int64_t* seq, int64_t B, int L, const srfrd_pack_t* pk_host) {
   SRFRD_REQUIRE(seq && pk_host, "pack_plan: null pointer");
-  const srfrd_pack_t pk = *pk_host;
+  const srfrd_pack_t& pk = *pk_host;
   SRFRD_REQUIRE(pk.rows && pk.cnt && pk.seq_first && pk.tok_row && pk.row_tok && pk.row_ids && pk.row_info && pk.tile_row0 &&
                 pk.last_row, "pack_plan: null output");
   SRFRD_REQUIRE(B >= 1 && L >= 1 && L <= 4096, "pack_plan: bad shape (B=%lld L=%d)", (long long)B, L);
@@ -141,17 +228,75 @@
   const int64_t need = (B * (L + 1) + PACK_TILE - 1) / PACK_TILE * PACK_TILE;
   SRFRD_REQUIRE(pk.cap >= need, "pack_plan: capacity %lld rows < %lld", (long long)pk.cap, (long long)need);
   SRFRD_REQUIRE(((uintptr_t)pk.row_info & 15) == 0, "pack_plan: row_info must be 16-byte aligned");
-  pack_count_kernel<<<(unsigned)((B + 7) / 8), 256, 0, stream>>>(seq, keep, B, L, pk.cnt);
-  SRFRD_LAUNCH_CHECK();
-  const size_t smem = (size_t)(2 * B + 2 + PACK_TILE + 2) * sizeof(int);
-  static bool attr = false;
-  if (!attr) {
-    SRFRD_CUDA(cudaFuncSetAttribute(pack_scan_kernel, cudaFuncAttributeMaxDynamicSharedMemorySize, 160 * 1024));
-    attr = true;
-  }
-  pack_scan_kernel<<<1, SCAN_THREADS, smem, stream>>>(pk, B, L + 1 <= PACK_TILE ? 1 : 0);
-  SRFRD_LAUNCH_CHECK();
-  pack_fill_kernel<<<(unsigned)((B + 7) / 8), 256, 0, stream>>>(seq, keep, B, L, pk);
+  return 0;
+}
+
+static unsigned pack_blocks(int64_t B) { return (unsigned)((B + PACK_SEQS - 1) / PACK_SEQS); }
+
+extern "C" int srfrd_pack_offsets(const int64_t* seq, const int64_t* keep, int64_t B, int L, const srfrd_pack_t* pk,
+                                  void* stream) {
+  if (int rc = pack_check(seq, B, L, pk)) return rc;
+  SRFRD_CUDA(launch_pdl(pack_offsets_kernel, dim3(pack_blocks(B)), dim3(PACK_THREADS), 0, (cudaStream_t)stream, seq, keep,
+                        B, L, L + 1 <= PACK_TILE ? 1 : 0, *pk));
   SRFRD_LAUNCH_CHECK();
   return 0;
 }
+
+extern "C" int srfrd_pack_tiles(int64_t B, int L, const srfrd_pack_t* pk, void* stream) {
+  SRFRD_REQUIRE(pk && pk->rows && pk->cnt && pk->tile_row0, "pack_tiles: null pointer");
+  SRFRD_REQUIRE(B >= 1 && B <= 16384, "pack_tiles: bad batch (B=%lld)", (long long)B);
+  SRFRD_REQUIRE(L >= 1 && L + 1 <= PACK_TILE, "pack_tiles: sequences of %d rows do not fit a %d-row tile", L + 1, PACK_TILE);
+  const size_t smem = 2 * (size_t)B + PACK_TILE;
+  SRFRD_CUDA(launch_pdl(pack_tiles_kernel, dim3(1), dim3(TILE_THREADS), smem, (cudaStream_t)stream, *pk, (int)B));
+  SRFRD_LAUNCH_CHECK();
+  return 0;
+}
+
+extern "C" int srfrd_pack_embed_ln_fwd(const int64_t* seq, const int64_t* keep, int64_t B, int L, const srfrd_pack_t* pk,
+                                       const float* item_table, int64_t n_rows, int D, const float* pos_table,
+                                       const float* aux_table, int64_t n_aux, int F, int mode, const int64_t* aux_ids,
+                                       float item_scale, const float* ln_w, const float* ln_b, float eps, void* x0_bf16,
+                                       void* q_bf16, float* stats, int ldx, float drop_p, uint64_t drop_seed,
+                                       uint32_t drop_stream, const float* drop_step, void* stream) {
+  if (int rc = pack_check(seq, B, L, pk)) return rc;
+  EmbedParams p;
+  bool vec = false;
+  if (int rc = embed_params(p, vec, item_table, D, pos_table, aux_table, F, mode, seq, aux_ids, B, L, item_scale, ln_w, ln_b,
+                            eps, x0_bf16, nullptr, q_bf16, stats, ldx, drop_p, drop_seed, drop_stream, drop_step, pk->row_tok,
+                            pk->rows, pk->cap))
+    return rc;
+  if (L + 1 > PACK_TILE) {
+    SRFRD_CUDA(launch_pdl(pack_fill_kernel<false, 32, 1, 0, false>, dim3(pack_blocks(B)), dim3(PACK_THREADS), 0,
+                          (cudaStream_t)stream, seq, keep, B, L, *pk, p));
+    SRFRD_LAUNCH_CHECK();
+    return srfrd_embed_ln_fwd_packed(item_table, n_rows, D, pos_table, aux_table, n_aux, F, mode, seq, aux_ids, B, L,
+                                     item_scale, ln_w, ln_b, eps, x0_bf16, q_bf16, stats, ldx, drop_p, drop_seed, drop_stream,
+                                     drop_step, pk->row_tok, pk->rows, pk->cap, stream);
+  }
+  const int H = D + (mode == 1 ? F : 0);
+#define CALL(LPR, CH)                                                                                                \
+  do {                                                                                                               \
+    auto* kern = !p.drop_thresh ? (mode == 0 ? pack_fill_kernel<true, LPR, CH, 0, false>                             \
+                                  : mode == 1 ? pack_fill_kernel<true, LPR, CH, 1, false>                            \
+                                              : pack_fill_kernel<true, LPR, CH, 2, false>)                           \
+                                : (mode == 0 ? pack_fill_kernel<true, LPR, CH, 0, true>                              \
+                                  : mode == 1 ? pack_fill_kernel<true, LPR, CH, 1, true>                             \
+                                              : pack_fill_kernel<true, LPR, CH, 2, true>);                           \
+    SRFRD_CUDA(launch_pdl(kern, dim3(pack_blocks(B)), dim3(PACK_THREADS), 0, (cudaStream_t)stream, seq, keep, B, L, *pk, \
+                          p));                                                                                       \
+  } while (0)
+  SRFRD_ROW_DISPATCH(H, CALL);
+#undef CALL
+  SRFRD_LAUNCH_CHECK();
+  return 0;
+}
+
+extern "C" int srfrd_pack_plan(const int64_t* seq, const int64_t* keep, int64_t B, int L, const srfrd_pack_t* pk_host,
+                               void* stream) {
+  if (int rc = srfrd_pack_offsets(seq, keep, B, L, pk_host, stream)) return rc;
+  EmbedParams none = {};
+  SRFRD_CUDA(launch_pdl(pack_fill_kernel<false, 32, 1, 0, false>, dim3(pack_blocks(B)), dim3(PACK_THREADS), 0,
+                        (cudaStream_t)stream, seq, keep, B, L, *pk_host, none));
+  SRFRD_LAUNCH_CHECK();
+  return L + 1 <= PACK_TILE ? srfrd_pack_tiles(B, L, pk_host, stream) : 0;
+}
diff --git a/srfrd_b200/csrc/rowwise.cu b/srfrd_b200/csrc/rowwise.cu
--- a/srfrd_b200/csrc/rowwise.cu
+++ b/srfrd_b200/csrc/rowwise.cu
@@ -1,68 +1,10 @@
 #include <stdlib.h>
 
 #include "common.cuh"
+#include "embed_row.cuh"
 #include "srfrd_b200.h"
 
 namespace srfrd {
-
-static constexpr int MAXW = 512;
-
-template <int LPR>
-__device__ __forceinline__ float group_sum(float v) {
-#pragma unroll
-  for (int o = LPR / 2; o > 0; o >>= 1) v += __shfl_xor_sync(0xffffffffu, v, o);
-  return v;
-}
-
-__device__ __forceinline__ void unpack8(const uint4& u, float* f) {
-  const uint32_t w[4] = {u.x, u.y, u.z, u.w};
-#pragma unroll
-  for (int i = 0; i < 4; ++i) {
-    const float2 t = __bfloat1622float2(*reinterpret_cast<const __nv_bfloat162*>(&w[i]));
-    f[2 * i] = t.x; f[2 * i + 1] = t.y;
-  }
-}
-__device__ __forceinline__ uint4 pack8(const float* f) {
-  return make_uint4(pack_bf16x2(f[0], f[1]), pack_bf16x2(f[2], f[3]), pack_bf16x2(f[4], f[5]), pack_bf16x2(f[6], f[7]));
-}
-__device__ __forceinline__ void load8_f32(const float* p, float* f) {
-  const float4 a = __ldg(reinterpret_cast<const float4*>(p)), b = __ldg(reinterpret_cast<const float4*>(p) + 1);
-  f[0] = a.x; f[1] = a.y; f[2] = a.z; f[3] = a.w; f[4] = b.x; f[5] = b.y; f[6] = b.z; f[7] = b.w;
-}
-__device__ __forceinline__ void load8_f32_stream(const float* p, float* f) {
-  float4 a, b;
-  asm volatile("ld.global.nc.L1::no_allocate.L2::256B.v4.f32 {%0,%1,%2,%3}, [%4];"
-               : "=f"(a.x), "=f"(a.y), "=f"(a.z), "=f"(a.w) : "l"(p));
-  asm volatile("ld.global.nc.L1::no_allocate.L2::256B.v4.f32 {%0,%1,%2,%3}, [%4];"
-               : "=f"(b.x), "=f"(b.y), "=f"(b.z), "=f"(b.w) : "l"(p + 4));
-  f[0] = a.x; f[1] = a.y; f[2] = a.z; f[3] = a.w; f[4] = b.x; f[5] = b.y; f[6] = b.z; f[7] = b.w;
-}
-__device__ __forceinline__ void store8_f32(float* p, const float* f) {
-  reinterpret_cast<float4*>(p)[0] = make_float4(f[0], f[1], f[2], f[3]);
-  reinterpret_cast<float4*>(p)[1] = make_float4(f[4], f[5], f[6], f[7]);
-}
-
-struct EmbedParams {
-  const float* item_table;
-  const float* pos_table;
-  const float* aux_table;
-  const int64_t* seq;
-  const int64_t* aux_ids;
-  const int* row_tok;
-  const int* rows_dev;
-  int64_t T;
-  int L, D, F, mode;
-  float item_scale;
-  const float* ln_w;
-  const float* ln_b;
-  float eps;
-  bf16* x0;
-  float* x0_f32;
-  bf16* q;
-  float* stats;
-  int ldx;
-  uint64_t drop_seed; uint32_t drop_thresh, drop_stream; float drop_scale; const float* drop_step;
-};
 
 template <int LPR, int CH, bool VEC>
 __global__ void __launch_bounds__(256, 4) embed_ln_kernel(EmbedParams p) {
@@ -191,14 +133,11 @@
   if (DROP) p.drop_seed = mix_seed(p.drop_seed, p.drop_step);
   constexpr int RPW = 32 / LPR;
   const int lane = threadIdx.x & 31, sub = lane % LPR, grp = lane / LPR;
-  const int H = p.D + (MODE == 1 ? p.F : 0);
-  const float invH = 1.f / (float)H;
   const int64_t warp = (int64_t)blockIdx.x * (blockDim.x >> 5) + (threadIdx.x >> 5);
   const int64_t stride = (int64_t)gridDim.x * (blockDim.x >> 5) * RPW;
   const int lstep = (int)(stride % p.L);
   int64_t t = warp * RPW + grp;
   int l = (int)(t % p.L);
-  const bool has_ln = p.ln_w != nullptr;
   if (p.rows_dev) p.T = min(p.T, (int64_t)__ldg(p.rows_dev));
   for (; t - grp < p.T; t += stride, l = (l + lstep >= p.L) ? l + lstep - p.L : l + lstep) {
     const bool row_ok = t < p.T;
@@ -216,87 +155,7 @@
       if (MODE == 1) aid = p.aux_ids ? __ldg(p.aux_ids + t) : 0;
       if (MODE == 2) aid = __ldg(p.aux_ids + t / p.L);
     }
-    const bool valid = row_ok && id != 0;
-    const float* erow = p.item_table + id * p.D;
-    const float* prow = p.pos_table + (int64_t)l * p.D;
-    const float* arow = p.aux_table + aid * (MODE == 1 ? p.F : p.D);
-    float v[CH][8];
-    float e[CH][8];
-#pragma unroll
-    for (int ch = 0; ch < CH; ++ch) {
-      const int c = (ch * LPR + sub) * 8;
-#pragma unroll
-      for (int j = 0; j < 8; ++j) e[ch][j] = 0.f;
-      if (valid && c < H) {
-        if (MODE != 1 || c < p.D) load8_f32_stream(erow + c, e[ch]);
-        else load8_f32(arow + (c - p.D), e[ch]);
-      }
-    }
-    float sum = 0.f;
-#pragma unroll
-    for (int ch = 0; ch < CH; ++ch) {
-      const int c = (ch * LPR + sub) * 8;
-#pragma unroll
-      for (int j = 0; j < 8; ++j) v[ch][j] = e[ch][j];
-      if (valid && c < p.D) {
-        float pp[8];
-        load8_f32(prow + c, pp);
-#pragma unroll
-        for (int j = 0; j < 8; ++j) {
-          float x = e[ch][j];
-          if (p.item_scale != 1.f) x = __fmul_rn(x, p.item_scale);
-          v[ch][j] = __fadd_rn(x, pp[j]);
-        }
-        if (MODE == 2) {
-          float u[8];
-          load8_f32(arow + c, u);
-#pragma unroll
-          for (int j = 0; j < 8; ++j) v[ch][j] = __fadd_rn(v[ch][j], u[j]);
-        }
-      }
-      if (DROP) {
-        if (valid && c < H) {
-#pragma unroll
-          for (int j = 0; j < 8; ++j)
-            v[ch][j] = dropout_keep(p.drop_seed, p.drop_stream, (uint64_t)t * H + c + j, p.drop_thresh)
-                           ? v[ch][j] * p.drop_scale : 0.f;
-        }
-      }
-      sum += ((v[ch][0] + v[ch][1]) + (v[ch][2] + v[ch][3])) + ((v[ch][4] + v[ch][5]) + (v[ch][6] + v[ch][7]));
-    }
-    float a = 0.f, nb = 0.f, mean = 0.f;
-    if (has_ln) {
-      mean = group_sum<LPR>(sum) * invH;
-      float sq = 0.f;
-#pragma unroll
-      for (int ch = 0; ch < CH; ++ch) {
-        if ((ch * LPR + sub) * 8 < H) {
-          float d[8];
-#pragma unroll
-          for (int j = 0; j < 8; ++j) d[j] = v[ch][j] - mean;
-          sq += ((d[0] * d[0] + d[1] * d[1]) + (d[2] * d[2] + d[3] * d[3])) + ((d[4] * d[4] + d[5] * d[5]) + (d[6] * d[6] + d[7] * d[7]));
-        }
-      }
-      a = rsqrtf(group_sum<LPR>(sq) * invH + p.eps);
-      nb = -mean * a;
-    }
-    if (!row_ok) continue;
-#pragma unroll
-    for (int ch = 0; ch < CH; ++ch) {
-      const int c = (ch * LPR + sub) * 8;
-      if (c >= H) continue;
-      if (p.x0_f32) store8_f32(p.x0_f32 + t * H + c, v[ch]);
-      if (p.x0) *reinterpret_cast<uint4*>(p.x0 + t * p.ldx + c) = pack8(v[ch]);
-      if (has_ln) {
-        float w[8], b[8], y[8];
-        load8_f32(p.ln_w + c, w);
-        load8_f32(p.ln_b + c, b);
-#pragma unroll
-        for (int j = 0; j < 8; ++j) y[j] = fmaf(fmaf(v[ch][j], a, nb), w[j], b[j]);
-        *reinterpret_cast<uint4*>(p.q + t * p.ldx + c) = pack8(y);
-      }
-    }
-    if (has_ln && p.stats && sub == 0) *reinterpret_cast<float2*>(p.stats + 2 * t) = make_float2(mean, a);
+    embed_ln_row<LPR, CH, MODE, DROP>(p, t, row_ok, id, aid, l, sub);
   }
 }
 
@@ -687,18 +546,6 @@
     else if ((H) <= 256) { CALL(32, 1); }                \
     else { CALL(32, 2); }                                \
   } while (0)
-#define SRFRD_ROW_DISPATCH(H, CALL)                      \
-  do {                                                   \
-    if ((H) <= 32) { CALL(4, 1); }                       \
-    else if ((H) <= 64) { CALL(8, 1); }                  \
-    else if ((H) <= 96) { CALL(4, 3); }                  \
-    else if ((H) <= 128) { CALL(16, 1); }                \
-    else if ((H) <= 192) { CALL(8, 3); }                 \
-    else if ((H) <= 256) { CALL(32, 1); }                \
-    else if ((H) <= 384) { CALL(16, 3); }                \
-    else { CALL(32, 2); }                                \
-  } while (0)
-
 __global__ void __launch_bounds__(256) colsum_kernel(const bf16* X, int64_t M, int N, int64_t ld, float* out,
                                                      int rows_per_block) {
   extern __shared__ float sm[];
@@ -806,13 +653,11 @@
 
 using namespace srfrd;
 
-static int embed_ln_fwd_impl(const float* item_table, int64_t n_rows, int D, const float* pos_table,
-                             const float* aux_table, int64_t n_aux, int F, int mode, const int64_t* seq,
-                             const int64_t* aux_ids, int64_t B, int L, float item_scale, const float* ln_w,
-                             const float* ln_b, float eps, void* x0_bf16, float* x0_f32, void* q_bf16,
-                             float* stats, int ldx, float drop_p, uint64_t drop_seed, uint32_t drop_stream,
-                             const float* drop_step, const int* row_tok, const int* rows_dev, int64_t cap_rows,
-                             void* stream) {
+int srfrd::embed_params(EmbedParams& p, bool& vec, const float* item_table, int D, const float* pos_table,
+                        const float* aux_table, int F, int mode, const int64_t* seq, const int64_t* aux_ids, int64_t B, int L,
+                        float item_scale, const float* ln_w, const float* ln_b, float eps, void* x0_bf16, float* x0_f32,
+                        void* q_bf16, float* stats, int ldx, float drop_p, uint64_t drop_seed, uint32_t drop_stream,
+                        const float* drop_step, const int* row_tok, const int* rows_dev, int64_t cap_rows) {
   SRFRD_REQUIRE(item_table && pos_table && seq, "embed_ln_fwd: null input");
   SRFRD_REQUIRE(drop_p >= 0.f && drop_p < 1.f, "embed_ln_fwd: dropout p must be in [0, 1)");
   SRFRD_REQUIRE(mode >= 0 && mode <= 2, "embed_ln_fwd: mode must be 0 (none), 1 (concat fake) or 2 (add user label)");
@@ -820,14 +665,11 @@
   SRFRD_REQUIRE(mode != 2 || aux_ids, "embed_ln_fwd: per-sequence labels required for mode 2");
   const int H = D + (mode == 1 ? F : 0);
   SRFRD_REQUIRE(H <= MAXW, "embed_ln_fwd: width %d > %d unsupported", H, MAXW);
-  const bool vec = D % 8 == 0 && H % 8 == 0;
+  vec = D % 8 == 0 && H % 8 == 0;
   SRFRD_REQUIRE(!ln_w || (ln_b && q_bf16), "embed_ln_fwd: LN needs weight, bias and an output");
   SRFRD_REQUIRE((!x0_bf16 && !q_bf16) || (ldx >= ((H + 7) & ~7) && ldx % 8 == 0), "embed_ln_fwd: bad ldx %d", ldx);
-  (void)n_rows; (void)n_aux;
-  if (B * L == 0) return 0;
   SRFRD_REQUIRE(!row_tok || (vec && rows_dev && cap_rows > 0 && !x0_f32),
                 "embed_ln_fwd_packed: needs widths that are multiples of 8, the device row count and a capacity");
-  EmbedParams p;
   p.item_table = item_table; p.pos_table = pos_table; p.aux_table = aux_table; p.seq = seq; p.aux_ids = aux_ids;
   p.row_tok = row_tok; p.rows_dev = rows_dev;
   p.T = row_tok ? cap_rows : B * L; p.L = L; p.D = D; p.F = F; p.mode = mode; p.item_scale = item_scale;
@@ -836,6 +678,25 @@
   p.drop_seed = drop_seed; p.drop_stream = drop_stream; p.drop_step = drop_step;
   p.drop_thresh = drop_p > 0.f ? (uint32_t)((double)drop_p * 4294967296.0) : 0;
   p.drop_scale = drop_p > 0.f ? 1.f / (1.f - drop_p) : 1.f;
+  return 0;
+}
+
+static int embed_ln_fwd_impl(const float* item_table, int64_t n_rows, int D, const float* pos_table,
+                             const float* aux_table, int64_t n_aux, int F, int mode, const int64_t* seq,
+                             const int64_t* aux_ids, int64_t B, int L, float item_scale, const float* ln_w,
+                             const float* ln_b, float eps, void* x0_bf16, float* x0_f32, void* q_bf16,
+                             float* stats, int ldx, float drop_p, uint64_t drop_seed, uint32_t drop_stream,
+                             const float* drop_step, const int* row_tok, const int* rows_dev, int64_t cap_rows,
+                             void* stream) {
+  (void)n_rows; (void)n_aux;
+  EmbedParams p;
+  bool vec = false;
+  if (int rc = embed_params(p, vec, item_table, D, pos_table, aux_table, F, mode, seq, aux_ids, B, L, item_scale, ln_w, ln_b,
+                            eps, x0_bf16, x0_f32, q_bf16, stats, ldx, drop_p, drop_seed, drop_stream, drop_step, row_tok,
+                            rows_dev, cap_rows))
+    return rc;
+  if (B * L == 0) return 0;
+  const int H = p.D + (mode == 1 ? F : 0);
 #define CALL(LPR, CH)                                                                                       \
   do {                                                                                                      \
     const int grid = grid_for_rows(p.T, 8 * (32 / LPR), 8);                                                 \
diff --git a/srfrd_b200/engine.py b/srfrd_b200/engine.py
--- a/srfrd_b200/engine.py
+++ b/srfrd_b200/engine.py
@@ -390,8 +390,18 @@
         seq = seq.contiguous()
         aux_ids = self._aux_ids(fake_ids, B, L)
         hyb = live = None
+        x = [ws[f"x{i}"][:T] for i in range(nb + 1)]
+        emb = (P.view(s.item_key), P.view(s.pos_key), P.view(s.aux_key) if s.aux_key else None, s.mode, seq, aux_ids,
+               s.item_scale, P.view("attention_layernorms.0.weight"), P.view("attention_layernorms.0.bias"), LN_EPS)
+        emb_drop = dict(drop_p=p_drop if s.kind == "SASRec" else 0.0, drop_seed=seed, drop_stream=1, drop_step=step)
+        tiles = packed and self.packed_mode(B, L) == "tile"
         if packed:
-            plan.build(seq, None if keep is None else keep.contiguous())
+            keep = None if keep is None else keep.contiguous()
+            plan.offsets(seq, keep)
+            if tiles:
+                with self._branch(second=True):
+                    plan.tiles()
+            plan.embed_ln_fwd(*emb, x[0], ws["Q0"][:T], ws["st1_0"][:T], keep=keep, **emb_drop)
             if self.packed_mode(B, L) == "hybrid":
                 hyb = self._hybrid_ws(B * L)
                 if self.live_tiles:
@@ -404,14 +414,8 @@
         sv = _Saved(seq=seq, aux_ids=aux_ids, B=B, L=L, T=T, row_ids=plan.row_ids if packed else seq.view(-1), plan=plan,
                     hyb=hyb, live=live, p_drop=p_drop, seed=seed, step=step, fuse_ln=fuse_ln, oproj=oproj,
                     mlp2=packed and self.fuse_ffn and Hp <= 128, version=self.fwd_version)
-        x = [ws[f"x{i}"][:T] for i in range(nb + 1)]
         with ops.row_limit(plan.rows) if packed else nullcontext():
-            emb = (P.view(s.item_key), P.view(s.pos_key), P.view(s.aux_key) if s.aux_key else None, s.mode, seq, aux_ids,
-                   s.item_scale, P.view("attention_layernorms.0.weight"), P.view("attention_layernorms.0.bias"), LN_EPS)
-            emb_drop = dict(drop_p=p_drop if s.kind == "SASRec" else 0.0, drop_seed=seed, drop_stream=1, drop_step=step)
-            if packed:
-                ops.embed_ln_fwd_packed(*emb, x[0], ws["Q0"][:T], ws["st1_0"][:T], plan, **emb_drop)
-            else:
+            if not packed:
                 ops.embed_ln_fwd(*emb, x0_bf16=x[0], q_bf16=ws["Q0"][:T], stats=ws["st1_0"][:T], **emb_drop)
             for i in range(nb):
                 Q, q, kv, o, r, y, h1 = (ws[f"{n}{i}"][:T] for n in ("Q", "q", "kv", "o", "r", "y", "h1"))
@@ -425,6 +429,8 @@
                 ln2 = dict(ln_w=P.view(f"forward_layernorms.{i}.weight"), ln_b=P.view(f"forward_layernorms.{i}.bias"),
                            ln_eps=LN_EPS, ln_stats=ws[f"st2_{i}"][:T])
                 fold = dict(wo=self.sh[f"wo{i}"], bias=self.bias("bo", i), residual=Q, r=r, y=y, **ln2) if oproj & 1 else {}
+                if tiles and i == 0:
+                    self._join(second=True)
                 self._attention_fwd(sv, i, q, kv, o, ws.get(f"ast{i}"), fold)
                 if oproj & 1:
                     pass
diff --git a/srfrd_b200/ops.py b/srfrd_b200/ops.py
--- a/srfrd_b200/ops.py
+++ b/srfrd_b200/ops.py
@@ -323,6 +323,27 @@
         _chk(seq, torch.int64, "seq")
         call("srfrd_pack_plan", _p(seq), _p(keep), B, L, C.byref(self.desc), _stream())
 
+    def offsets(self, seq, keep=None):
+        _lib.require_device()
+        assert tuple(seq.shape) == (self.B, self.L)
+        _chk(seq, torch.int64, "seq")
+        call("srfrd_pack_offsets", _p(seq), _p(keep), self.B, self.L, C.byref(self.desc), _stream())
+
+    def embed_ln_fwd(self, item_table, pos_table, aux_table, mode, seq, aux_ids, item_scale, ln_w, ln_b, eps, x0_bf16, q_bf16,
+                     stats, keep=None, drop_p=0.0, drop_seed=0, drop_stream=0, drop_step=None):
+        _lib.require_device()
+        assert tuple(seq.shape) == (self.B, self.L)
+        D = item_table.shape[1]
+        F = aux_table.shape[1] if (aux_table is not None and mode == 1) else 0
+        call("srfrd_pack_embed_ln_fwd", _p(seq), _p(keep), self.B, self.L, C.byref(self.desc), _p(item_table),
+             item_table.shape[0], D, _p(pos_table), _p(aux_table), 0 if aux_table is None else aux_table.shape[0], F, mode,
+             _p(aux_ids), float(item_scale), _p(ln_w), _p(ln_b), float(eps), _p(x0_bf16), _p(q_bf16), _p(stats),
+             x0_bf16.stride(0), float(drop_p), int(drop_seed), int(drop_stream), _p(drop_step), _stream())
+
+    def tiles(self):
+        _lib.require_device()
+        call("srfrd_pack_tiles", self.B, self.L, C.byref(self.desc), _stream())
+
 
 @contextmanager
 def row_limit(rows_dev):
```

After: 10.07 million (median of 6 runs). +2.4%, better.
